# KadAMRN/Data_Free_Quantization

Hardware: AMD Instinct MI355X
Metric: weight-GB/s quantized (per-ch INT8 DFQ sweep) + top-1 delta, MobileNetV2 (higher is better)
Workload: dtype f32

## Files before the change

### data_free_quantization_amd/_lib.py

```python
from __future__ import annotations

import ctypes as C
import os
from pathlib import Path
from typing import Optional

import torch

PKG = Path(__file__).resolve().parent
LIB_PATH = PKG / "libdfq_hip.so"

DFQ_TENSOR_ASYM, DFQ_TENSOR_SYM, DFQ_CHANNEL_ASYM, DFQ_CHANNEL_SYM = 0, 1, 2, 3
DFQ_CLIP, DFQ_GIVEN_RANGE, DFQ_SCALE_F32, DFQ_PACK_INT4, DFQ_DEVICE_RANGE = 0x1, 0x2, 0x4, 0x8, 0x10
DFQ_OK, DFQ_ERR_INVALID, DFQ_ERR_HIP, DFQ_ERR_UNSUPPORTED = 0, -1, -2, -3
DFQ_ERR_NOMEM, DFQ_ERR_SHAPE, DFQ_ERR_WORKSPACE = -4, -5, -6

EXPORTS = [
    "dfq_abi_version", "dfq_preload", "dfq_error_string", "dfq_last_hip_error",
    "dfq_quantize_ws_bytes", "dfq_quantize_tensor", "dfq_chunk_range", "dfq_range", "dfq_fake_quant_given",
    "dfq_fake_quant_tensor",
    "dfq_act_observe",
    "dfq_sweep_plan_create", "dfq_sweep_plan_ws_bytes", "dfq_sweep_plan_create_ws", "dfq_sweep_plan_execute",
    "dfq_sweep_plan_stats", "dfq_sweep_plan_destroy",
    "dfq_bn_fold", "dfq_bn_fold_ws_bytes", "dfq_bn_fold_batch", "dfq_clamp", "dfq_clamp_batch",
    "dfq_cle_ws_bytes", "dfq_cle_relation",
    "dfq_diff_plan_create", "dfq_diff_plan_snapshot", "dfq_diff_plan_execute", "dfq_diff_plan_destroy",
    "dfq_cle_plan_ws_bytes", "dfq_cle_plan_create", "dfq_cle_plan_run", "dfq_cle_plan_launch", "dfq_cle_plan_join",
    "dfq_cle_plan_info", "dfq_cle_plan_set_timing", "dfq_cle_plan_stats", "dfq_cle_plan_destroy",
    "dfq_bias_absorb", "dfq_bias_absorb_ws_bytes", "dfq_bias_absorb_batch", "dfq_bc_expect", "dfq_bc_apply", "dfq_bc_propagate", "dfq_bc_chain",
    "dfq_act_moments", "dfq_act_minmax", "dfq_act_affine",
    "dfq_pair_stats_ws_bytes", "dfq_pair_stats_batch",
    "dfq_clip_search_ws_bytes", "dfq_clip_search_batch",
    "dfq_mx_quantize_ws_bytes", "dfq_mx_quantize_batch", "dfq_mx_quantize_search_batch", "dfq_mx_gemm",
    "dfq_mx_linear", "dfq_mx_conv2d",
    "dfq_int_gemm", "dfq_int_linear", "dfq_int_conv2d", "dfq_int_dwconv2d",
]
DIAG_EXPORTS = ["dfq_probe_stream", "dfq_probe_lds", "dfq_debug_timeline", "dfq_debug_ablate",
                "dfq_diag_cle_check_structure"]
DIAG_LIB_PATH = PKG / "libdfq_diag.so"


class TensorDesc(C.Structure):
    _fields_ = [
        ("src", C.c_void_p), ("dst", C.c_void_p), ("codes", C.c_void_p), ("scale", C.c_void_p),
        ("zero", C.c_void_p), ("esum", C.c_void_p), ("rows", C.c_int64), ("row_len", C.c_int64),
        ("khw", C.c_int32), ("bits", C.c_int32), ("mode", C.c_int32), ("flags", C.c_int32),
        ("clip_lo", C.c_float), ("clip_hi", C.c_float), ("given_min", C.c_double), ("given_max", C.c_double),
        ("range_enc", C.c_void_p),
    ]


class SweepStats(C.Structure):
    _fields_ = [
        ("n_tensors", C.c_int64), ("n_elems", C.c_int64), ("n_tasks_reduce", C.c_int64),
        ("n_tasks_main", C.c_int64), ("algo_bytes", C.c_int64), ("launches", C.c_int32),
        ("grid_blocks", C.c_int32), ("variant", C.c_int32), ("reserved", C.c_int32),
    ]


class BnFoldDesc(C.Structure):
    _fields_ = [
        ("w", C.c_void_p), ("bias", C.c_void_p), ("bn_w", C.c_void_p), ("bn_b", C.c_void_p),
        ("bn_mean", C.c_void_p), ("bn_var", C.c_void_p), ("fake_w", C.c_void_p), ("fake_b", C.c_void_p),
        ("eps", C.c_float), ("flags", C.c_int32), ("rows", C.c_int64), ("row_len", C.c_int64),
        ("range_enc", C.c_void_p),
    ]


class CleRel(C.Structure):
    _fields_ = [
        ("w1", C.c_void_p), ("w2", C.c_void_p), ("b1", C.c_void_p), ("bn_w", C.c_void_p), ("bn_b", C.c_void_p),
        ("s_acc", C.c_void_p), ("c1", C.c_int64), ("len1", C.c_int64), ("o2", C.c_int64), ("i2", C.c_int64),
        ("khw2", C.c_int64), ("s_acc_init", C.c_int32), ("reserved", C.c_int32),
    ]


class AbsorbDesc(C.Structure):
    _fields_ = [
        ("w2", C.c_void_p), ("b1", C.c_void_p), ("b2", C.c_void_p), ("bn_w", C.c_void_p), ("bn_b", C.c_void_p),
        ("c1", C.c_int64), ("o2", C.c_int64), ("i2", C.c_int64), ("khw2", C.c_int64),
    ]


class BcOp(C.Structure):
    _fields_ = [
        ("kind", C.c_int32), ("flag", C.c_int32), ("a", C.c_void_p), ("b", C.c_void_p), ("out", C.c_void_p),
        ("out2", C.c_void_p), ("n", C.c_int64), ("i2", C.c_int64), ("f", C.c_int64),
    ]


class PairDesc(C.Structure):
    _fields_ = [
        ("x", C.c_void_p), ("y", C.c_void_p), ("rows_out", C.c_void_p), ("total_out", C.c_void_p),
        ("rows", C.c_int64), ("row_len", C.c_int64),
    ]


class ClipSearchDesc(C.Structure):
    _fields_ = [
        ("w", C.c_void_p), ("rows", C.c_int64), ("row_len", C.c_int64), ("bits", C.c_int32), ("mode", C.c_int32),
        ("candidates", C.c_int32), ("flags", C.c_int32), ("min_frac", C.c_float), ("reserved", C.c_int32),
        ("choice", C.c_void_p), ("range", C.c_void_p), ("noise", C.c_void_p), ("range_enc", C.c_void_p),
    ]


class MxDesc(C.Structure):
    _fields_ = [
        ("src", C.c_void_p), ("dst", C.c_void_p), ("codes", C.c_void_p), ("scales", C.c_void_p), ("esum", C.c_void_p),
        ("rows", C.c_int64), ("row_len", C.c_int64), ("khw", C.c_int32), ("format", C.c_int32), ("flags", C.c_int32),
        ("reserved", C.c_int32),
    ]


class MxGemmDesc(C.Structure):
    _fields_ = [
        ("a_codes", C.c_void_p), ("a_scales", C.c_void_p), ("b_codes", C.c_void_p), ("b_scales", C.c_void_p),
        ("bias", C.c_void_p), ("out", C.c_void_p), ("ldo", C.c_int64), ("M", C.c_int64), ("N", C.c_int64),
        ("K", C.c_int64), ("a_format", C.c_int32), ("b_format", C.c_int32), ("flags", C.c_int32),
        ("reserved", C.c_int32),
    ]


class MxLinearDesc(C.Structure):
    _fields_ = [
        ("x", C.c_void_p), ("b_codes", C.c_void_p), ("b_scales", C.c_void_p), ("bias", C.c_void_p), ("out", C.c_void_p),
        ("ldx", C.c_int64), ("ldo", C.c_int64), ("M", C.c_int64), ("N", C.c_int64), ("K", C.c_int64),
        ("x_format", C.c_int32), ("b_format", C.c_int32), ("flags", C.c_int32), ("reserved", C.c_int32),
    ]


class MxConv2dDesc(C.Structure):
    _fields_ = [
        ("x", C.c_void_p), ("b_codes", C.c_void_p), ("b_scales", C.c_void_p), ("bias", C.c_void_p), ("out", C.c_void_p),
        ("B", C.c_int64), ("C", C.c_int64), ("H", C.c_int64), ("W", C.c_int64), ("N", C.c_int64), ("KH", C.c_int64),
        ("KW", C.c_int64), ("stride_h", C.c_int64), ("stride_w", C.c_int64), ("pad_h", C.c_int64), ("pad_w", C.c_int64),
        ("dil_h", C.c_int64), ("dil_w", C.c_int64),
        ("x_format", C.c_int32), ("b_format", C.c_int32), ("flags", C.c_int32), ("reserved", C.c_int32),
    ]


class IntGemmDesc(C.Structure):
    _fields_ = [
        ("a_codes", C.c_void_p), ("a_scale", C.c_void_p), ("a_zero", C.c_void_p), ("b_codes", C.c_void_p),
        ("b_scale", C.c_void_p), ("b_zero", C.c_void_p), ("bias", C.c_void_p), ("out", C.c_void_p),
        ("ldo", C.c_int64), ("M", C.c_int64), ("N", C.c_int64), ("K", C.c_int64),
        ("a_signed", C.c_int32), ("b_signed", C.c_int32), ("flags", C.c_int32), ("reserved", C.c_int32),
    ]


class IntLinearDesc(C.Structure):
    _fields_ = [
        ("x", C.c_void_p), ("min_dev", C.c_void_p), ("max_dev", C.c_void_p), ("b_codes", C.c_void_p),
        ("b_scale", C.c_void_p), ("b_zero", C.c_void_p), ("bias", C.c_void_p), ("out", C.c_void_p),
        ("given_min", C.c_double), ("given_max", C.c_double),
        ("ldx", C.c_int64), ("ldo", C.c_int64), ("M", C.c_int64), ("N", C.c_int64), ("K", C.c_int64),
        ("x_bits", C.c_int32), ("x_symmetric", C.c_int32), ("b_signed", C.c_int32), ("flags", C.c_int32),
        ("reserved", C.c_int32), ("reserved2", C.c_int32),
    ]


class IntConv2dDesc(C.Structure):
    _fields_ = [
        ("x", C.c_void_p), ("min_dev", C.c_void_p), ("max_dev", C.c_void_p), ("b_codes", C.c_void_p),
        ("b_scale", C.c_void_p), ("b_zero", C.c_void_p), ("bias", C.c_void_p), ("out", C.c_void_p),
        ("given_min", C.c_double), ("given_max", C.c_double),
        ("B", C.c_int64), ("C", C.c_int64), ("H", C.c_int64), ("W", C.c_int64), ("N", C.c_int64), ("KH", C.c_int64),
        ("KW", C.c_int64), ("stride_h", C.c_int64), ("stride_w", C.c_int64), ("pad_h", C.c_int64), ("pad_w", C.c_int64),
        ("dil_h", C.c_int64), ("dil_w", C.c_int64),
        ("x_bits", C.c_int32), ("x_symmetric", C.c_int32), ("b_signed", C.c_int32), ("flags", C.c_int32),
        ("reserved", C.c_int32), ("reserved2", C.c_int32),
    ]


class IntDwConv2dDesc(C.Structure):
    _fields_ = [(("mult", t) if f == "N" else (f, t)) for f, t in IntConv2dDesc._fields_]


DFQ_BC_OP_EXPECT, DFQ_BC_OP_APPLY, DFQ_BC_OP_PROPAGATE, DFQ_BC_OP_COPY = 0, 1, 2, 3
DFQ_BC_APPLY_VEC_SCRATCH = 1
DFQ_BN_FOLD_ZERO_BIAS = 1
DFQ_PAIR_PIECE_ELEMS = 8192
DFQ_CLIP_PIECE_ELEMS, DFQ_CLIP_MAX_CANDIDATES, DFQ_CLIP_SEARCH_DRY = 4096, 64, 1
DFQ_MX_BLOCK = 32
DFQ_MX_FP4_E2M1, DFQ_MX_FP8_E4M3 = 0, 1
DFQ_MX_FP6_E2M3, DFQ_MX_FP6_E3M2 = 0x23, 0x32
DFQ_MX_TASK_ELEMS, DFQ_MX_ESUM_TASK_ELEMS = 4096, 2048
DFQ_INT_B_PACK4, DFQ_INT_B_PER_ROW, DFQ_INT_MAX_K = 0x1, 0x2, 32768
DFQ_INT_DW_MAX_TAPS, DFQ_INT_DW_TILE_H, DFQ_INT_DW_TILE_W, DFQ_INT_DW_LDS_BYTES = 64, 32, 64, 16384

_LIB: Optional[C.CDLL] = None


class DFQLibraryError(RuntimeError):
    pass


def load(path: Optional[os.PathLike] = None) -> C.CDLL:
    global _LIB
    if _LIB is not None and path is None:
        return _LIB
    by_env = path is None and os.environ.get("DFQ_LIB") == "diag"
    if by_env:
        path = DIAG_LIB_PATH
    p = Path(path) if path else LIB_PATH
    if not p.exists():
        raise DFQLibraryError(
            f"{p} is missing: build it with `python -m data_free_quantization_amd.build` "
            "(or __graft_entry__.build()); there is no CPU fallback")
    L = C.CDLL(str(p))
    P, I32, I64, F32, F64, SZ = C.c_void_p, C.c_int32, C.c_int64, C.c_float, C.c_double, C.c_size_t
    sig = {
        "dfq_abi_version": ([], C.c_int),
        "dfq_preload": ([], C.c_int),
        "dfq_error_string": ([C.c_int], C.c_char_p),
        "dfq_last_hip_error": ([], C.c_char_p),
        "dfq_quantize_ws_bytes": ([C.POINTER(TensorDesc), C.POINTER(SZ)], C.c_int),
        "dfq_quantize_tensor": ([C.POINTER(TensorDesc), P, SZ, P], C.c_int),
        "dfq_chunk_range": ([P, I64, I64, P, P, P], C.c_int),
        "dfq_range": ([P, I64, P, P], C.c_int),
        "dfq_act_observe": ([P, I64, I64, P, P, P, I32, I32, F64, P, P], C.c_int),
        "dfq_fake_quant_given": ([P, P, I64, I32, I32, I32, P, P, P, F64, F64, P], C.c_int),
        "dfq_fake_quant_tensor": ([P, P, I64, I32, I32, I32, P, P], C.c_int),
        "dfq_sweep_plan_create": ([C.POINTER(TensorDesc), I32, C.POINTER(P)], C.c_int),
        "dfq_sweep_plan_ws_bytes": ([C.POINTER(TensorDesc), I32], C.c_int64),
        "dfq_sweep_plan_create_ws": ([C.POINTER(TensorDesc), I32, P, I64, P, C.POINTER(P)], C.c_int),
        "dfq_sweep_plan_execute": ([P, P], C.c_int),
        "dfq_sweep_plan_stats": ([P, C.POINTER(SweepStats)], C.c_int),
        "dfq_sweep_plan_destroy": ([P], C.c_int),
        "dfq_bn_fold": ([P, P, P, P, P, P, P, P, F32, I64, I64, P], C.c_int),
        "dfq_clamp": ([P, I64, F32, F32, P], C.c_int),
        "dfq_clamp_batch": ([C.POINTER(P), C.POINTER(I64), I32, F32, F32, P], C.c_int),
        "dfq_bn_fold_ws_bytes": ([C.POINTER(BnFoldDesc), I32], C.c_int64),
        "dfq_bn_fold_batch": ([C.POINTER(BnFoldDesc), I32, P, I64, P], C.c_int),
        "dfq_cle_ws_bytes": ([I64], SZ),
        "dfq_cle_relation": ([P, P, P, P, P, I64, I64, I64, I64, I64, F64, F64, I32, F32, P, P, I32, P, SZ, P],
                             C.c_int),
        "dfq_diff_plan_create": ([C.POINTER(P), C.POINTER(P), C.POINTER(I64), I32, C.POINTER(P)], C.c_int),
        "dfq_diff_plan_snapshot": ([P, P], C.c_int),
        "dfq_diff_plan_execute": ([P, C.POINTER(F64), P], C.c_int),
        "dfq_diff_plan_destroy": ([P], C.c_int),
        "dfq_cle_plan_ws_bytes": ([C.POINTER(I64), I32], C.c_int64),
        "dfq_cle_plan_create": ([C.POINTER(CleRel), I32, C.POINTER(P), C.POINTER(I64), I32, F64, F64, I32, F32, I32,
                                 P, I64, C.POINTER(P)], C.c_int),
        "dfq_cle_plan_run": ([P, F64, I32, I32, C.POINTER(I32), C.POINTER(F64), P], C.c_int),
        "dfq_cle_plan_launch": ([P, F64, I32, I32, P], C.c_int),
        "dfq_cle_plan_join": ([P, C.POINTER(I32), C.POINTER(F64)], C.c_int),
        "dfq_cle_plan_info": ([P, C.POINTER(I32), C.POINTER(I32), C.POINTER(I32)], C.c_int),
        "dfq_cle_plan_destroy": ([P], C.c_int),
        "dfq_cle_plan_set_timing": ([P, I32], C.c_int),
        "dfq_cle_plan_stats": ([P, C.POINTER(I64), C.POINTER(F64), C.POINTER(I32)], C.c_int),
        "dfq_bias_absorb": ([P, P, P, P, P, I64, I64, I64, I64, F32, P], C.c_int),
        "dfq_bias_absorb_ws_bytes": ([C.POINTER(AbsorbDesc), I32], C.c_int64),
        "dfq_bias_absorb_batch": ([C.POINTER(AbsorbDesc), I32, F32, P, I64, C.POINTER(I32), P], C.c_int),
        "dfq_bc_expect": ([P, P, I64, I32, I32, P, P], C.c_int),
        "dfq_bc_apply": ([P, I64, I64, P, I64, P, P, C.POINTER(I64), P], C.c_int),
        "dfq_bc_propagate": ([P, I64, P, I64, I32, P], C.c_int),
        "dfq_bc_chain": ([C.POINTER(BcOp), I32, C.POINTER(I32), P], C.c_int),
        "dfq_act_moments": ([P, P, I64, I32, I32, F32, I32, P, P, P], C.c_int),
        "dfq_act_minmax": ([P, P, I64, I32, F32, F32, P, P], C.c_int),
        "dfq_act_affine": ([P, P, P, I64, I64, I64, I64, P, P], C.c_int),
        "dfq_pair_stats_ws_bytes": ([C.POINTER(PairDesc), I32], C.c_int64),
        "dfq_pair_stats_batch": ([C.POINTER(PairDesc), I32, P, I64, P], C.c_int),
        "dfq_clip_search_ws_bytes": ([C.POINTER(ClipSearchDesc), I32], C.c_int64),
        "dfq_clip_search_batch": ([C.POINTER(ClipSearchDesc), I32, P, I64, P], C.c_int),
        "dfq_mx_quantize_ws_bytes": ([C.POINTER(MxDesc), I32], C.c_int64),
        "dfq_mx_quantize_batch": ([C.POINTER(MxDesc), I32, P, I64, P], C.c_int),
        "dfq_mx_quantize_search_batch": ([C.POINTER(MxDesc), I32, P, I64, P], C.c_int),
        "dfq_mx_gemm": ([C.POINTER(MxGemmDesc), P], C.c_int),
        "dfq_mx_linear": ([C.POINTER(MxLinearDesc), P], C.c_int),
        "dfq_mx_conv2d": ([C.POINTER(MxConv2dDesc), P], C.c_int),
        "dfq_int_gemm": ([C.POINTER(IntGemmDesc), P], C.c_int),
        "dfq_int_linear": ([C.POINTER(IntLinearDesc), P], C.c_int),
        "dfq_int_conv2d": ([C.POINTER(IntConv2dDesc), P], C.c_int),
        "dfq_int_dwconv2d": ([C.POINTER(IntDwConv2dDesc), P], C.c_int),
    }
    diag = {
        "dfq_probe_stream": ([P, P, P, P, I64, I32, P], C.c_int),
        "dfq_debug_timeline": ([P, I64], C.c_int),
        "dfq_debug_ablate": ([C.c_uint32], C.c_int),
        "dfq_probe_lds": ([P, P, P, P, I64, I32, I32, P], C.c_int),
        "dfq_diag_cle_check_structure": ([C.POINTER(CleRel), I32, C.POINTER(P), C.POINTER(I64), I32, I32,
                                          C.POINTER(I64), C.c_char_p, I32], C.c_int),
    }
    for name, (args, res) in sig.items():
        fn = getattr(L, name)
        fn.argtypes = args
        fn.restype = res
    for name, (args, res) in diag.items():
        if hasattr(L, name):
            fn = getattr(L, name)
            fn.argtypes = args
            fn.restype = res
    if L.dfq_abi_version() != 1:
        raise DFQLibraryError("libdfq_hip.so ABI version mismatch")
    if path is None or by_env:
        _LIB = L
    return L


_PRELOADED = False


def preload() -> C.CDLL:
    global _PRELOADED
    L = load()
    if not _PRELOADED:
        check(L.dfq_preload(), "dfq_preload")
        _PRELOADED = True
    return L


_DIAG: Optional[C.CDLL] = None


def load_diag() -> C.CDLL:
    global _DIAG
    if _DIAG is None:
        _DIAG = load(DIAG_LIB_PATH)
    return _DIAG


def check(rc: int, what: str, shape_error=RuntimeError):
    if rc == DFQ_OK:
        return
    L = load()
    msg = f"{what}: {L.dfq_error_string(rc).decode()}"
    if rc == DFQ_ERR_HIP:
        msg += f" ({L.dfq_last_hip_error().decode()})"
    if rc == DFQ_ERR_SHAPE:
        raise shape_error(msg)
    if rc == DFQ_ERR_UNSUPPORTED:
        raise NotImplementedError(msg)
    raise DFQLibraryError(msg)


_F32 = torch.float32


def require_device(*tensors: Optional[torch.Tensor]):
    for t in tensors:
        if t is None or (t.is_cuda and t.dtype is _F32 and t.is_contiguous()):
            continue
        if not t.is_cuda:
            raise RuntimeError(
                "data_free_quantization_amd runs the DFQ weight path on a ROCm GPU only; "
                f"got a tensor on {t.device} (move the model with .cuda() first)")
        if t.dtype != torch.float32:
            raise TypeError(f"expected float32 tensors, got {t.dtype}")
        raise ValueError("expected contiguous tensors")


def ptr(t: Optional[torch.Tensor]):
    return None if t is None else C.c_void_p(t.data_ptr())


WEIGHT_GENERATION = 0


def weights_changed() -> None:
    global WEIGHT_GENERATION
    WEIGHT_GENERATION += 1


REF_THREADS = int(os.environ.get("DFQ_REF_THREADS", "8"))


_RAW_STREAM = getattr(torch._C, "_cuda_getCurrentRawStream", None)


def raw_stream(device: torch.device) -> C.c_void_p:
    idx = device.index if device.index is not None else torch.cuda.current_device()
    if _RAW_STREAM is not None:
        return C.c_void_p(_RAW_STREAM(idx))
    return C.c_void_p(torch.cuda.current_stream(device).cuda_stream)


def stream_of(t: torch.Tensor):
    return raw_stream(t.device)
```

### data_free_quantization_amd/csrc/dfq_cle.hip

```cpp
#include "dfq_cle_kernels.h"

#include <algorithm>
#include <chrono>
#include <cstdio>
#include <cstdlib>
#include <cstring>
#include <condition_variable>
#include <functional>
#include <memory>
#include <mutex>
#include <thread>
#include <type_traits>
#include <new>
#include <vector>

using namespace dfq;

constexpr int32_t kCleHistCap = 1025;

struct CleTables {
    CleRel* rels = nullptr;
    CleTask *rtasks = nullptr, *atasks = nullptr;
    CleLayer* layers = nullptr;
    CleChunk* chunks = nullptr;
    CleUnit* units = nullptr;
    int64_t* b1off = nullptr;
    float* part = nullptr;
    float* b1 = nullptr;
    float* tail = nullptr;
    uint32_t* rng = nullptr;
    double* means = nullptr;
    CleState* state = nullptr;
    double* hist = nullptr;
    uint32_t* cnt = nullptr;
    float* vsave = nullptr;
    int32_t* vtag = nullptr;
    int64_t host_bytes = 0, total = 0;
    void bind(char* base, const CleStructure& S, int32_t slots) {
        constexpr bool kHost = true, kDevice = false;
        int64_t off = 0;
        auto table = [&](auto*& ptr, int64_t count, bool host_built) {
            using T = std::remove_reference_t<decltype(*ptr)>;
            ptr = base ? reinterpret_cast<T*>(base + off) : nullptr;
            off += round256((int64_t)sizeof(T) * std::max<int64_t>(count, 1));
            if (host_built) host_bytes = off;
        };
        const int64_t nl = (int64_t)S.layers.size(), nch = (int64_t)S.chunks.size();
        table(rels, (int64_t)S.R.size(), kHost);
        table(rtasks, (int64_t)S.rt.size(), kHost);
        table(atasks, (int64_t)S.at.size(), kHost);
        table(layers, nl, kHost);
        table(chunks, nch, kHost);
        table(units, (int64_t)S.units.size(), kHost);
        table(b1off, (int64_t)S.b1off.size(), kHost);
        table(part, (int64_t)(slots + 2) * nl, kHost);
        table(b1, 32 * S.nb1_total, kDevice);
        table(tail, kCleTailWords * nch, kDevice);
        table(rng, 4 * S.M, kDevice);
        table(means, nl, kDevice);
        table(state, 1, kDevice);
        table(hist, kCleHistCap, kDevice);
        table(cnt, nch + 1, kDevice);
        table(vsave, S.lagged ? 2 * S.M : 0, kDevice);
        table(vtag, S.lagged ? (int64_t)S.at.size() : 0, kDevice);
        if (!S.lagged) vsave = nullptr, vtag = nullptr;
        total = off;
    }
};

struct dfq_cle_plan {
    std::shared_ptr<const CleStructure> S;
    CleTables t;
    int32_t slots = 8;
    double* d_hist = nullptr;
    uint32_t* d_flag = nullptr;
    uint64_t* d_sig = nullptr;
    uint64_t gen = 0;
    double smin = 1e-8, smax = 1e8;
    int32_t is_signed = 0;
    float eps = 0.f;
    void* d_tables = nullptr;
    bool pooled = false;
    void* d_snap_owned = nullptr;
    int dev = 0;
    struct CleAsync* async = nullptr;
    bool abandoned = false;
    bool timed = false;
    float loop_ms = -1.f;
    int32_t launched = 0;
    int32_t nl() const { return (int32_t)S->layers.size(); }
    int64_t nchunks() const { return (int64_t)S->chunks.size(); }
    int64_t nunits() const { return (int64_t)S->units.size(); }
};

static bool cle_timing() {
    static const bool on = ab_env("DFQ_CLE_TIMING") != nullptr;
    return on;
}

struct CleDeviceCtx {
    std::mutex mu;
    hipStream_t st = nullptr;
    CleState* h_state = nullptr;
    uint32_t* h_flag = nullptr;
    uint32_t* d_flag = nullptr;
    char* d_pool = nullptr;
    size_t pool_cap = 0;
    char* h_pool = nullptr;
    size_t hpool_cap = 0;
    bool pool_busy = false;
    uint64_t pool_struct = 0;
    hipEvent_t pool_ev = nullptr;
    double* d_hist = nullptr;
    int64_t hist_cap = 0;
    double* h_hist = nullptr;
    int64_t h_hist_cap = 0;
    void* sig = nullptr;
    int sig_state = 0;
    uint64_t gen = 0;
    struct dfq_cle_plan* pending = nullptr;
    hipEvent_t in_ev = nullptr;
    struct CleWorker* worker = nullptr;
};
static CleDeviceCtx& cle_device_ctx(int dev) {
    static CleDeviceCtx ctx[64];
    return ctx[dev & 63];
}
static std::unique_lock<std::mutex> cle_ctx_acquire(CleDeviceCtx& ctx, bool join_pending);
static hipError_t cle_ctx_ready(CleDeviceCtx& ctx) {
    hipError_t e = hipSuccess;
    if (!ctx.st) {
        int least = 0, greatest = 0;
        e = hipDeviceGetStreamPriorityRange(&least, &greatest);
        if (e == hipSuccess) e = hipStreamCreateWithPriority(&ctx.st, hipStreamNonBlocking, greatest);
    }
    if (e == hipSuccess && !ctx.h_state) e = hipHostMalloc(&ctx.h_state, sizeof(CleState));
    if (e == hipSuccess && !ctx.h_flag) {
        e = hipHostMalloc(&ctx.h_flag, 64, hipHostMallocMapped | hipHostMallocCoherent);
        if (e == hipSuccess) e = hipHostGetDevicePointer(reinterpret_cast<void**>(&ctx.d_flag), ctx.h_flag, 0);
    }
    if (e == hipSuccess && !ctx.pool_ev) e = hipEventCreateWithFlags(&ctx.pool_ev, hipEventDisableTiming);
    if (e == hipSuccess && !ctx.in_ev) e = hipEventCreateWithFlags(&ctx.in_ev, hipEventDisableTiming);
    return e;
}

template <class T, class N>
static hipError_t cle_grow(T*& buf, N& have, N need, N cap, bool pinned) {
    if (have >= need) return hipSuccess;
    (void)(pinned ? hipHostFree(buf) : hipFree(buf));
    buf = nullptr;
    have = 0;
    const hipError_t e = pinned ? hipHostMalloc(&buf, sizeof(T) * cap, hipHostMallocDefault) : hipMalloc(&buf, sizeof(T) * cap);
    if (e == hipSuccess) have = cap;
    return e;
}
static hipError_t cle_pool_reserve(CleDeviceCtx& ctx, size_t dev_bytes, size_t host_bytes, bool headroom) {
    const auto cap = [&](size_t n) { return headroom ? n + n / 2 : n; };
    if (ctx.pool_cap < dev_bytes) ctx.pool_struct = 0;
    hipError_t e = cle_grow(ctx.d_pool, ctx.pool_cap, dev_bytes, cap(dev_bytes), false);
    if (e == hipSuccess) e = cle_grow(ctx.h_pool, ctx.hpool_cap, host_bytes, cap(host_bytes), true);
    return e;
}

static void cle_plan_free(dfq_cle_plan* p) {
    const double t0 = now_us();
    if (p->pooled) {
        CleDeviceCtx& ctx = cle_device_ctx(p->dev);
        const std::unique_lock<std::mutex> lock = cle_ctx_acquire(ctx, false);
        ctx.pool_busy = false;
    } else {
        (void)hipFree(p->d_tables);
    }
    (void)hipFree(p->d_snap_owned);
    if (cle_timing()) fprintf(stderr, "DFQ_CLE_TIMING free: %.1f us\n", now_us() - t0);
    delete p;
}

static int64_t snap_bytes(int64_t n) { return round256(n * (int64_t)sizeof(float)); }

extern "C" int64_t dfq_cle_plan_ws_bytes(const int64_t* target_n, int32_t n_targets) {
    if (n_targets < 0 || (n_targets > 0 && !target_n)) return -1;
    int64_t b = 0;
    for (int32_t l = 0; l < n_targets; ++l) {
        if (target_n[l] < 0) return -1;
        b += snap_bytes(target_n[l]);
    }
    return b;
}

extern "C" int dfq_cle_plan_create(const dfq_cle_rel* rels, int32_t n_rel, float* const* targets,
                                   const int64_t* target_n, int32_t n_targets, double s_min, double s_max,
                                   int32_t is_signed, float eps, int32_t ref_threads, void* ws, int64_t ws_bytes,
                                   dfq_cle_plan** out) {
    if (!out || n_rel < 0 || n_targets < 0 || (n_rel > 0 && !rels) || (n_targets > 0 && (!targets || !target_n)))
        return DFQ_ERR_INVALID;
    const double tc0 = now_us();
    const int64_t need_ws = dfq_cle_plan_ws_bytes(target_n, n_targets);
    if (need_ws < 0) return DFQ_ERR_INVALID;
    if (ws && (ws_bytes < need_ws || reinterpret_cast<uintptr_t>(ws) % 256 != 0)) return DFQ_ERR_INVALID;
    *out = nullptr;
    std::vector<CleRel> R;
    int64_t M = 0;
    if (const int rc = cle_rels_from_desc(rels, n_rel, R, M); rc != DFQ_OK) return rc;
    const double tp1 = now_us();
    bool cached = false;
    int rc = DFQ_OK;
    const std::shared_ptr<const CleStructure> S =
        cle_structure_cached(R, M, targets, target_n, n_targets, ref_threads, rc, cached);
    if (!S) return rc;
    const double tp5 = now_us();
    std::vector<CleRel> Rb = S->R;
    for (int32_t r = 0; r < n_rel; ++r) {
        Rb[r].w1 = R[r].w1; Rb[r].w2 = R[r].w2; Rb[r].b1 = R[r].b1;
        Rb[r].bnw = R[r].bnw; Rb[r].bnb = R[r].bnb; Rb[r].sacc = R[r].sacc;
    }
    dfq_cle_plan* p = new (std::nothrow) dfq_cle_plan();
    if (!p) return DFQ_ERR_NOMEM;
    p->S = S;
    std::vector<CleLayer> layers = S->layers;
    {
        char* snap_base = static_cast<char*>(ws);
        if (!snap_base && need_ws > 0) {
            hipError_t e = hipMalloc(&p->d_snap_owned, need_ws);
            if (e != hipSuccess) { set_last_hip_error(e); cle_plan_free(p); return DFQ_ERR_HIP; }
            snap_base = static_cast<char*>(p->d_snap_owned);
        }
        int64_t snap_off = 0;
        for (int32_t l = 0; l < n_targets; ++l) {
            layers[l].w = targets[l];
            layers[l].snap = reinterpret_cast<float*>(snap_base + snap_off);
            snap_off += snap_bytes(target_n[l]);
        }
    }
    if (cle_timing() && !cached) {
        fprintf(stderr, "DFQ_CLE_TIMING plan: steps %d nlaunch %d lagged %d stop %d; offsets (units/ranges):", S->steps,
                S->nlaunch, (int)S->lagged, S->stop_off);
        for (int32_t k = 0; k < 2 * S->nlaunch; ++k)
            fprintf(stderr, " %d:%lld/%lld", k, (long long)(S->uoffs[k + 1] - S->uoffs[k]),
                    (long long)(S->roffs[k + 1] - S->roffs[k]));
        fprintf(stderr, "; rescale tasks per step:");
        for (int32_t k = 0; k < S->steps; ++k) fprintf(stderr, " %lld", (long long)(S->astep[k + 1] - S->astep[k]));
        fprintf(stderr, "\n");
    }
    (void)hipGetDevice(&p->dev);
    p->smin = s_min; p->smax = s_max; p->is_signed = is_signed; p->eps = eps;
    p->slots = std::max<int32_t>(ref_threads, 1);
    hipError_t e;
    auto fail = [&](hipError_t err) { set_last_hip_error(err); cle_plan_free(p); return DFQ_ERR_HIP; };
    CleTables& T = p->t;
    T.bind(nullptr, *S, p->slots);
    const double tm0 = now_us();
    char* base = nullptr;
    char* hblob = nullptr;
    CleDeviceCtx& ctx = cle_device_ctx(p->dev);
    e = hipSuccess;
    {
        const std::unique_lock<std::mutex> lock = cle_ctx_acquire(ctx, false);
        if (!ctx.pool_busy && (e = cle_ctx_ready(ctx)) == hipSuccess &&
            (e = hipEventSynchronize(ctx.pool_ev)) == hipSuccess &&
            (e = cle_pool_reserve(ctx, (size_t)T.total, (size_t)T.host_bytes, true)) == hipSuccess) {
            ctx.pool_busy = true;
            p->pooled = true;
            base = ctx.d_pool;
            hblob = ctx.h_pool;
        }
        if (e != hipSuccess) return fail(e);
    }
    std::vector<char> blob;
    const bool resident = p->pooled && ctx.pool_struct == S->id;
    if (!p->pooled) {
        if ((e = hipMalloc(&p->d_tables, T.total)) != hipSuccess) return fail(e);
        base = static_cast<char*>(p->d_tables);
        blob.assign(T.host_bytes, 0);
        hblob = blob.data();
    } else if (!resident) {
        std::memset(hblob, 0, T.host_bytes);
    }
    T.bind(base, *S, p->slots);
    const double tm1 = now_us();
    auto mirror = [&](const auto* d) { return hblob + (reinterpret_cast<const char*>(d) - base); };
    auto put = [&](const auto* d, const auto& v) {
        if (!v.empty()) std::memcpy(mirror(d), v.data(), sizeof(v[0]) * v.size());
    };
    put(T.rels, Rb);
    put(T.layers, layers);
    if (!resident) {
        put(T.rtasks, S->rt); put(T.atasks, S->at); put(T.chunks, S->chunks); put(T.units, S->units); put(T.b1off, S->b1off);
        float* lm = reinterpret_cast<float*>(mirror(T.part)) + (int64_t)p->slots * n_targets;
        for (int64_t l = 0; l < n_targets; ++l) {
            lm[2 * l] = (float)layers[l].n;
            lm[2 * l + 1] = layers[l].nt == 1 ? 1.f : 0.f;
        }
    }
    if (p->pooled) {
        if (resident) {
            const size_t nr = sizeof(CleRel) * Rb.size(), nly = sizeof(CleLayer) * layers.size();
            if (nr && (e = hipMemcpyAsync(T.rels, mirror(T.rels), nr, hipMemcpyHostToDevice, ctx.st)) != hipSuccess)
                return fail(e);
            if (nly && (e = hipMemcpyAsync(T.layers, mirror(T.layers), nly, hipMemcpyHostToDevice, ctx.st)) != hipSuccess)
                return fail(e);
        } else if ((e = hipMemcpyAsync(base, hblob, T.host_bytes, hipMemcpyHostToDevice, ctx.st)) != hipSuccess) {
            return fail(e);
        }
        if ((e = hipEventRecord(ctx.pool_ev, ctx.st)) != hipSuccess) return fail(e);
        ctx.pool_struct = S->id;
    } else if ((e = hipMemcpy(base, hblob, T.host_bytes, hipMemcpyHostToDevice)) != hipSuccess) {
        return fail(e);
    }
    if (cle_timing())
        fprintf(stderr, "DFQ_CLE_TIMING create: plan %.1f us (relations %.1f, structure %s %.1f: chains %.1f, tasks %.1f, "
                "chunks %.1f, placement %.1f), tables %lld B %.1f us, copy %lld B %.1f us\n", tm0 - tc0, tp1 - tc0,
                cached ? "cached" : "built", tp5 - tp1, S->t_chains, S->t_tasks, S->t_chunks, S->t_place,
                (long long)T.total, tm1 - tm0, (long long)T.host_bytes, now_us() - tm1);
    *out = p;
    return DFQ_OK;
}

static int cle_enqueue_iteration(dfq_cle_plan* p, hipStream_t s, int32_t g, int32_t max_iters) {
    const int64_t kStepGrid = [] {
        const char* e = ab_env("DFQ_CLE_STEP_GRID");
        return e && *e ? std::max<int64_t>(1, atoll(e)) : int64_t(2048);
    }();
    const int64_t kTileGrid = [] {
        const char* e = ab_env("DFQ_CLE_TILE_GRID");
        return e && *e ? std::max<int64_t>(1, atoll(e)) : int64_t(4096);
    }();
    const CleStructure& S = *p->S;
    const CleTables& T = p->t;
    CleFin F{T.cnt, T.part, T.means, p->d_hist, p->nchunks(), S.nbig, p->slots, p->nl(), 0, p->d_flag,
             S.stop_off < 0 ? 1 : 0};
    const int32_t NL = S.nlaunch;
    const bool run_g = g < max_iters, prev = g >= 1;
    for (int32_t k = 0; k < NL; ++k) {
        const bool step = k < S.steps;
        const int64_t a0 = step ? S.astep[k] : 0, a1 = step ? S.astep[k + 1] : 0;
        if (step && run_g && !S.fused && S.rstep[k + 1] > S.rstep[k]) {
            hipLaunchKernelGGL(cle_loop_range_kernel, dim3((int)std::min<int64_t>(S.rstep[k + 1] - S.rstep[k], kStepGrid)),
                               dim3(kThreads), 0, s, T.rels, T.rtasks, S.rstep[k], S.rstep[k + 1], T.rng, S.M, T.state, 0);
            DFQ_LAUNCH_CHECK();
        }
        const int64_t nab = run_g ? std::min<int64_t>(a1 - a0, kStepGrid) : 0;
        const int64_t uo = S.uoffs[k], nuo = run_g ? S.uoffs[k + 1] - uo : 0;
        const int64_t up = S.uoffs[NL + k], nup = prev ? S.uoffs[NL + k + 1] - up : 0;
        const int64_t ro = S.roffs[k], nro_t = (g + 1 < max_iters) ? S.roffs[k + 1] - ro : 0;
        const int64_t rp = S.roffs[NL + k], nrp_t = (prev && run_g) ? S.roffs[NL + k + 1] - rp : 0;
        int64_t nto = std::min<int64_t>(nuo, kTileGrid);
        const int64_t ntp = std::min<int64_t>(nup, kTileGrid);
        F.last = (k == S.steps) ? 1 : 0;
        if (F.last && run_g && S.nbig == 0) nto = std::max<int64_t>(nto, 1);
        const int64_t nro = std::min<int64_t>(nro_t, kStepGrid), nrp = std::min<int64_t>(nrp_t, kStepGrid);
        int32_t stop_it = -1;
        if (S.stop_off == k && run_g) stop_it = g;
        else if (S.stop_off == NL + k && prev) stop_it = g - 1;
        const int64_t nblk = nab + (stop_it >= 0 ? cle_stop_blocks(p->nchunks()) : 0) + nto + ntp + nro + nrp;
        if (nblk == 0) continue;
        auto kern = (step && S.step_pos[k]) ? cle_loop_step_kernel<true> : cle_loop_step_kernel<false>;
        hipLaunchKernelGGL(kern, dim3((int)nblk), dim3(kThreads), 0, s, T.rels, T.atasks, a0, a1, nab, T.rng,
                           S.M, p->is_signed, p->eps, p->smin, p->smax, T.layers, T.chunks, T.b1off,
                           T.units, uo, nuo, nto, up, nup, ntp, T.b1, T.tail, T.rtasks, ro, nro_t, nro, rp,
                           nrp_t, nrp, F, T.state, g, T.vsave, T.vtag, stop_it);
        DFQ_LAUNCH_CHECK();
    }
    return DFQ_OK;
}

constexpr int32_t kCleAhead = 1;
constexpr double kClePollQuietUs = 1000.0;
static constexpr int kCleGateSeconds = 120;
static constexpr int kCleJoinSeconds = kCleGateSeconds + 30;
static constexpr double kCleLaunchDeadlineUs = 0.5e6 * kCleGateSeconds;
static hipError_t cle_hist_ready(CleDeviceCtx& ctx, int32_t max_iters) {
    const int64_t n = (int64_t)max_iters + 1;
    hipError_t e = cle_grow(ctx.h_hist, ctx.h_hist_cap, n, n, true);
    if (e == hipSuccess && n > kCleHistCap) e = cle_grow(ctx.d_hist, ctx.hist_cap, n, n, false);
    return e;
}

static hipError_t cle_copy_back(void* dst, const void* src, size_t bytes, hipStream_t s) {
    hipError_t e = hipMemcpyAsync(dst, src, bytes, hipMemcpyDeviceToHost, s);
    return e == hipSuccess ? hipStreamSynchronize(s) : e;
}

#ifdef DFQ_DIAGNOSTICS
#include "dfq_cle_timeline.h"
#else
struct CleTimeline {
    int begin(const dfq_cle_plan*, hipStream_t) { return DFQ_OK; }
    int report(const dfq_cle_plan*, hipStream_t) { return DFQ_OK; }
};
#endif

struct CleRun {
    double threshold;
    int32_t count, max_iters;
    double deadline_us;
    bool idle = false;
    double t_drive = 0;
    int32_t launched = 0;
    bool deadline_hit = false;
    hipEvent_t tev[2] = {nullptr, nullptr};
};

static int cle_run_setup(dfq_cle_plan* p, CleDeviceCtx& ctx, CleRun& run) {
    DFQ_HIP_CHECK(cle_ctx_ready(ctx));
    *ctx.h_flag = 0;
    p->d_flag = ctx.d_flag;
    hipStream_t s = ctx.st;
    const CleStructure& S = *p->S;
    const CleTables& T = p->t;
    p->d_hist = T.hist;
    DFQ_HIP_CHECK(cle_hist_ready(ctx, run.max_iters));
    if (run.max_iters + 1 > kCleHistCap) p->d_hist = ctx.d_hist;
    CleState init{};
    init.diff = 1e8;
    init.thr = run.threshold;
    init.count = run.count;
    init.max_iters = run.max_iters;
    init.done = !((init.diff > run.threshold) && (0 < run.count)) || run.max_iters == 0;
    run.idle = init.done != 0;
    {
        const int64_t npart = (int64_t)p->slots * std::max(p->nl(), 1), ncnt = p->nchunks() + 1;
        const int64_t nvtag = T.vtag ? (int64_t)S.at.size() : 0;
        const int64_t words = std::max({4 * S.M, npart, ncnt, nvtag});
        const int64_t grid = std::min<int64_t>(std::max<int64_t>({p->nunits(), ceil_div(words, (int64_t)kThreads), 1}), 4096);
        hipLaunchKernelGGL(cle_loop_init_kernel, dim3((int)grid), dim3(kThreads), 0, s, T.layers, T.chunks,
                           p->nchunks(), T.units, p->nunits(), T.rng, S.M, T.part, npart, T.cnt, ncnt,
                           T.vtag, nvtag, T.state, init);
        DFQ_LAUNCH_CHECK();
    }
    if (S.fused && S.rstep[1] > S.rstep[0]) {
        hipLaunchKernelGGL(cle_loop_range_kernel, dim3((int)std::min<int64_t>(S.rstep[1] - S.rstep[0], 2048)),
                           dim3(kThreads), 0, s, T.rels, T.rtasks, S.rstep[0], S.rstep[1], T.rng, S.M, T.state, 0);
        DFQ_LAUNCH_CHECK();
    }
    return DFQ_OK;
}

static int cle_run_drive(dfq_cle_plan* p, CleDeviceCtx& ctx, CleRun& run) {
    hipStream_t s = ctx.st;
    const int32_t max_iters = run.max_iters;
    run.t_drive = now_us();
    p->loop_ms = -1.f;
    if (p->timed) {
        DFQ_HIP_CHECK(hipEventCreate(&run.tev[0]));
        DFQ_HIP_CHECK(hipEventCreate(&run.tev[1]));
        DFQ_HIP_CHECK(hipEventRecord(run.tev[0], s));
    }
    if (run.idle) return DFQ_OK;
    const char* pd = ab_env("DFQ_CLE_TEST_POLL_DELAY_US");
    const int poll_delay_us = pd ? atoi(pd) : 0;
    const double quiet_us = pd ? 0.0 : kClePollQuietUs;
    uint32_t last_f = ~0u;
    double t_moved = run.t_drive;
    for (;;) {
        const uint32_t f = __atomic_load_n(ctx.h_flag, __ATOMIC_ACQUIRE);
        if (f & 1u) break;
        const int32_t ran = (int32_t)(f >> 1);
        if (run.launched <= max_iters && !run.deadline_hit && run.launched - ran <= kCleAhead) {
            const int rc = cle_enqueue_iteration(p, s, run.launched, max_iters);
            if (rc != DFQ_OK) return rc;
            ++run.launched;
            continue;
        }
        if (poll_delay_us > 0) std::this_thread::sleep_for(std::chrono::microseconds(poll_delay_us));
        const double t = now_us();
        if (f != last_f) {
            last_f = f;
            t_moved = t;
        } else if (t - t_moved >= quiet_us) {
            const hipError_t q = hipStreamQuery(s);
            if (q != hipErrorNotReady) {
                if (q != hipSuccess) break;
                const uint32_t f2 = __atomic_load_n(ctx.h_flag, __ATOMIC_ACQUIRE);
                if ((f2 & 1u) || run.launched > max_iters || run.deadline_hit || (int32_t)(f2 >> 1) + 1 < run.launched)
                    break;
            }
            t_moved = t;
        }
        if (run.deadline_us > 0 && t - run.t_drive > run.deadline_us) run.deadline_hit = true;
        __builtin_ia32_pause();
    }
    return DFQ_OK;
}

static int cle_run_drain(dfq_cle_plan* p, CleDeviceCtx& ctx, CleRun& run, CleTimeline& timeline, int32_t* iterations,
                         std::vector<double>* hist) {
    hipStream_t s = ctx.st;
    const CleTables& T = p->t;
    if (!run.idle && p->S->lagged) {
        hipLaunchKernelGGL(cle_loop_rollback_kernel, dim3(1024), dim3(kThreads), 0, s, T.layers, p->nl(), T.rels,
                           T.atasks, (int64_t)p->S->at.size(), T.vsave, T.vtag, T.state);
        DFQ_LAUNCH_CHECK();
    }
    if (run.tev[1]) DFQ_HIP_CHECK(hipEventRecord(run.tev[1], s));
    if (p->d_sig) DFQ_HIP_CHECK(hipStreamWriteValue64(s, p->d_sig, p->gen, 0));
    DFQ_HIP_CHECK(hipMemcpyAsync(ctx.h_state, T.state, sizeof(CleState), hipMemcpyDeviceToHost, s));
    const int32_t hn = std::min(run.launched, run.max_iters);
    if (hist && hn > 0) DFQ_HIP_CHECK(hipMemcpyAsync(ctx.h_hist, p->d_hist, sizeof(double) * hn, hipMemcpyDeviceToHost, s));
    DFQ_HIP_CHECK(hipStreamSynchronize(s));
    p->launched = run.launched;
    if (run.tev[0]) {
        float ms = -1.f;
        if (hipEventElapsedTime(&ms, run.tev[0], run.tev[1]) == hipSuccess) p->loop_ms = ms;
        (void)hipEventDestroy(run.tev[0]);
        (void)hipEventDestroy(run.tev[1]);
    }
    if (cle_timing())
        fprintf(stderr, "DFQ_CLE_TIMING run: loop %.1f us (%d iterations launched)\n", now_us() - run.t_drive, run.launched);
    if (const int rc = timeline.report(p, s); rc != DFQ_OK) return rc;
    const CleState fin = *ctx.h_state;
    if (fin.error) {
        set_last_hip_error(hipErrorLaunchTimeOut);
        return DFQ_ERR_HIP;
    }
    if (!fin.done) {
        set_last_hip_error_text(run.deadline_hit ? "the launched CLE loop reached its time limit before converging"
                                                 : "the CLE loop stopped before its stop rule said done");
        return DFQ_ERR_HIP;
    }
    if (ab_env("DFQ_CLE_DEBUG")) {
        std::vector<float> part((size_t)p->slots * std::max(p->nl(), 1));
        DFQ_HIP_CHECK(cle_copy_back(part.data(), T.part, sizeof(float) * part.size(), s));
        for (int32_t l = 0; l < p->nl(); ++l) {
            fprintf(stderr, "DFQ_CLE_DEBUG layer %d:", l);
            for (int t = 0; t < p->slots; ++t) fprintf(stderr, " %.9g", part[(size_t)p->slots * l + t]);
            fprintf(stderr, "\n");
        }
    }
    if (iterations) *iterations = fin.iters;
    if (hist) {
        hist->assign((size_t)std::max(fin.iters, 0), 0.0);
        if (fin.iters > 0) std::memcpy(hist->data(), ctx.h_hist, sizeof(double) * std::min(fin.iters, hn));
    }
    return DFQ_OK;
}

static int cle_run_locked(dfq_cle_plan* p, CleDeviceCtx& ctx, double threshold, int32_t count, int32_t max_iters,
                          int32_t* iterations, std::vector<double>* hist, double deadline_us = -1.0) {
    CleRun run{threshold, count, max_iters, deadline_us};
    CleTimeline timeline;
    int rc = cle_run_setup(p, ctx, run);
    if (rc == DFQ_OK) rc = timeline.begin(p, ctx.st);
    if (rc == DFQ_OK) rc = cle_run_drive(p, ctx, run);
    if (rc == DFQ_OK) rc = cle_run_drain(p, ctx, run, timeline, iterations, hist);
    return rc;
}


struct CleAsync {
    std::mutex m;
    std::condition_variable cv;
    bool done = false;
    int rc = DFQ_OK;
    int32_t iters = 0;
    std::vector<double> hist;
    char err[128] = {0};
};

struct CleWorker {
    std::mutex m;
    std::condition_variable cv;
    std::function<void()> job;
    bool has_job = false;
};
static void cle_worker_loop(CleWorker* w) {
    for (;;) {
        std::function<void()> j;
        {
            std::unique_lock<std::mutex> l(w->m);
            w->cv.wait(l, [w] { return w->has_job; });
            j = std::move(w->job);
            w->has_job = false;
        }
        j();
    }
}
static void cle_worker_ready(CleDeviceCtx& ctx) {
    if (ctx.worker) return;
    CleWorker* w = new CleWorker();
    std::thread(cle_worker_loop, w).detach();
    ctx.worker = w;
}

static hipError_t cle_signal_ready(CleDeviceCtx& ctx) {
    if (ctx.sig) return hipSuccess;
    if (ctx.sig_state < 0) return hipErrorNotSupported;
    hipError_t e = hipSuccess;
    void* sig = nullptr;
    if ((e = hipExtMallocWithFlags(&sig, sizeof(uint64_t), hipMallocSignalMemory)) != hipSuccess) {
        ctx.sig_state = -1;
        return e;
    }
    if ((e = hipStreamWriteValue64(ctx.st, sig, 0, 0)) != hipSuccess || (e = hipStreamSynchronize(ctx.st)) != hipSuccess) {
        (void)hipFree(sig);
        ctx.sig_state = -1;
        return e;
    }
    ctx.sig = sig;
    ctx.gen = 0;
    return hipSuccess;
}

static bool cle_async_join(dfq_cle_plan* p, double seconds = -1.0) {
    if (!p || !p->async) return true;
    CleAsync* a = p->async;
    std::unique_lock<std::mutex> l(a->m);
    if (seconds < 0) {
        a->cv.wait(l, [a] { return a->done; });
        return true;
    }
    return a->cv.wait_for(l, std::chrono::duration<double>(seconds), [a] { return a->done; });
}

static std::unique_lock<std::mutex> cle_ctx_acquire(CleDeviceCtx& ctx, bool join_pending) {
    std::unique_lock<std::mutex> lock(ctx.mu);
    while (dfq_cle_plan* q = join_pending ? ctx.pending : nullptr) {
        lock.unlock();
        cle_async_join(q);
        lock.lock();
        if (ctx.pending == q) ctx.pending = nullptr;
    }
    return lock;
}
static void cle_pending_clear(CleDeviceCtx& ctx, dfq_cle_plan* p) {
    const std::unique_lock<std::mutex> lock = cle_ctx_acquire(ctx, false);
    if (ctx.pending == p) ctx.pending = nullptr;
}

extern "C" int dfq_cle_plan_run(dfq_cle_plan* p, double threshold, int32_t count, int32_t max_iters,
                                int32_t* iterations, double* diffs, void* stream) {
    if (!p || max_iters < 0 || p->async) return DFQ_ERR_INVALID;
    const double ts0 = now_us();
    DFQ_HIP_CHECK(hipStreamSynchronize(static_cast<hipStream_t>(stream)));
    const double ts1 = now_us();
    int dev = 0;
    DFQ_HIP_CHECK(hipGetDevice(&dev));
    CleDeviceCtx& ctx = cle_device_ctx(dev);
    const std::unique_lock<std::mutex> lock = cle_ctx_acquire(ctx, true);
    if (cle_timing()) fprintf(stderr, "DFQ_CLE_TIMING run: caller sync %.1f us, context %.1f us\n", ts1 - ts0,
                              now_us() - ts1);
    std::vector<double> h;
    const int rc = cle_run_locked(p, ctx, threshold, count, max_iters, iterations, diffs ? &h : nullptr);
    if (rc == DFQ_OK && diffs && !h.empty()) std::memcpy(diffs, h.data(), sizeof(double) * h.size());
    return rc;
}

extern "C" int dfq_cle_plan_launch(dfq_cle_plan* p, double threshold, int32_t count, int32_t max_iters,
                                   void* stream) {
    if (!p || max_iters < 0 || p->async) return DFQ_ERR_INVALID;
    if (ab_env("DFQ_CLE_TL")) return DFQ_ERR_UNSUPPORTED;
    hipStream_t caller = static_cast<hipStream_t>(stream);
    CleDeviceCtx& ctx = cle_device_ctx(p->dev);
    const double tl0 = now_us();
    std::unique_ptr<CleAsync> rec(new (std::nothrow) CleAsync());
    uint64_t gen = 0;
    {
        const std::unique_lock<std::mutex> lock = cle_ctx_acquire(ctx, true);
        DFQ_HIP_CHECK(hipSetDevice(p->dev));
        DFQ_HIP_CHECK(cle_ctx_ready(ctx));
        const hipError_t es = cle_signal_ready(ctx);
        if (es == hipErrorNotSupported) return DFQ_ERR_UNSUPPORTED;
        DFQ_HIP_CHECK(es);
        DFQ_HIP_CHECK(cle_hist_ready(ctx, max_iters));
        DFQ_HIP_CHECK(hipEventRecord(ctx.in_ev, caller));
        DFQ_HIP_CHECK(hipStreamWaitEvent(ctx.st, ctx.in_ev, 0));
        gen = ctx.gen + 1;
        hipLaunchKernelGGL(cle_caller_gate_kernel, dim3(1), dim3(64), 0, caller,
                           static_cast<const uint64_t*>(ctx.sig), gen, (uint64_t)kCleGateSeconds * 100000000ull);
        DFQ_LAUNCH_CHECK();
        ctx.gen = gen;
        if (rec) p->async = rec.get(), ctx.pending = p;
    }
    if (cle_timing()) fprintf(stderr, "DFQ_CLE_TIMING launch: gate and order %.1f us\n", now_us() - tl0);
    CleAsync* a = rec.release();
    const double t_launch = now_us();
    auto body = [p, &ctx, threshold, count, max_iters, gen, t_launch](CleAsync* a) {
        std::lock_guard<std::mutex> lock(ctx.mu);
        int rc = DFQ_OK;
        if (hipSetDevice(p->dev) != hipSuccess) {
            rc = DFQ_ERR_HIP;
        } else {
            rc = cle_run_locked(p, ctx, threshold, count, max_iters, &a->iters, &a->hist, kCleLaunchDeadlineUs);
        }
        if (rc == DFQ_ERR_HIP) copy_error_text(a->err, sizeof(a->err), dfq_last_hip_error());
        if (const char* d = ab_env("DFQ_CLE_TEST_RELEASE_DELAY_MS"))
            std::this_thread::sleep_for(std::chrono::milliseconds(atoi(d)));
        hipError_t e = hipStreamWriteValue64(ctx.st, ctx.sig, gen, 0);
        if (e == hipSuccess) e = hipStreamSynchronize(ctx.st);
        if (e != hipSuccess) {
            fprintf(stderr, "dfq_cle_plan_launch: releasing the caller's stream failed (%s)\n", hipGetErrorString(e));
            if (rc == DFQ_OK) rc = DFQ_ERR_HIP;
        }
        if (rc == DFQ_OK && now_us() - t_launch > 0.9e6 * kCleGateSeconds) {
            set_last_hip_error(hipErrorLaunchTimeOut);
            copy_error_text(a->err, sizeof(a->err), "CLE loop outlived the caller's stream gate");
            rc = DFQ_ERR_HIP;
        }
        {
            std::lock_guard<std::mutex> l(a->m);
            a->rc = rc;
            a->done = true;
        }
        a->cv.notify_all();
    };
    if (!a) {
        CleAsync tmp;
        body(&tmp);
        return tmp.rc;
    }
    p->d_sig = static_cast<uint64_t*>(ctx.sig);
    if (ab_env("DFQ_CLE_HOST_RELEASE")) p->d_sig = nullptr;
    p->gen = gen;
    bool posted = false;
    try {
        const std::unique_lock<std::mutex> lock = cle_ctx_acquire(ctx, false);
        cle_worker_ready(ctx);
        {
            std::lock_guard<std::mutex> l(ctx.worker->m);
            ctx.worker->job = [body, a] { body(a); };
            ctx.worker->has_job = true;
        }
        ctx.worker->cv.notify_one();
        posted = true;
    } catch (...) {}
    if (!posted) body(a);
    if (cle_timing()) fprintf(stderr, "DFQ_CLE_TIMING launch: total %.1f us\n", now_us() - tl0);
    return DFQ_OK;
}

extern "C" int dfq_cle_plan_join(dfq_cle_plan* p, int32_t* iterations, double* diffs) {
    if (!p || !p->async) return DFQ_ERR_INVALID;
    if (p->abandoned) return DFQ_ERR_HIP;
    double limit = kCleJoinSeconds;
    if (const char* j = ab_env("DFQ_CLE_TEST_JOIN_LIMIT_MS")) limit = atoi(j) * 1e-3;
    if (!cle_async_join(p, limit)) {
        p->abandoned = true;
        set_last_hip_error_text("the launched CLE loop did not finish in time; the caller's stream stays held");
        return DFQ_ERR_HIP;
    }
    cle_pending_clear(cle_device_ctx(p->dev), p);
    const CleAsync& a = *p->async;
    if (a.rc == DFQ_ERR_HIP && a.err[0]) set_last_hip_error_text(a.err);
    if (a.rc != DFQ_OK) return a.rc;
    if (iterations) *iterations = a.iters;
    if (diffs && !a.hist.empty()) std::memcpy(diffs, a.hist.data(), sizeof(double) * a.hist.size());
    return DFQ_OK;
}

extern "C" int dfq_cle_plan_info(const dfq_cle_plan* p, int32_t* chains, int32_t* steps, int32_t* launches) {
    if (!p) return DFQ_ERR_INVALID;
    if (chains) *chains = p->S->chains;
    if (steps) *steps = p->S->steps;
    if (launches) *launches = p->S->fused ? p->S->nlaunch : 2 * p->S->steps + 1;
    return DFQ_OK;
}

extern "C" int dfq_cle_plan_set_timing(dfq_cle_plan* p, int32_t on) {
    if (!p || p->async) return DFQ_ERR_INVALID;
    p->timed = on != 0;
    return DFQ_OK;
}

extern "C" int dfq_cle_plan_stats(const dfq_cle_plan* p, int64_t* bytes, double* loop_ms, int32_t* launched) {
    if (!p) return DFQ_ERR_INVALID;
    if (bytes) {
        bytes[0] = p->S->bytes_rescale;
        bytes[1] = p->S->bytes_metric;
        bytes[2] = p->S->bytes_range;
    }
    if (loop_ms) *loop_ms = p->loop_ms;
    if (launched) *launched = p->launched;
    return DFQ_OK;
}

extern "C" int dfq_cle_plan_destroy(dfq_cle_plan* p) {
    if (!p) return DFQ_OK;
    if (p->abandoned) return DFQ_OK;
    if (p->async) {
        cle_async_join(p);
        cle_pending_clear(cle_device_ctx(p->dev), p);
        delete p->async;
        p->async = nullptr;
    }
    cle_plan_free(p);
    return DFQ_OK;
}

namespace dfq {
constexpr size_t kClePreloadPool = size_t(4) << 20, kClePreloadHostPool = size_t(2) << 20;
constexpr int32_t kClePreloadHistIters = 100000;
hipError_t preload_cle() {
    int dev = 0;
    hipError_t e0 = hipGetDevice(&dev);
    if (e0 != hipSuccess) return e0;
    {
        CleDeviceCtx& ctx = cle_device_ctx(dev);
        const std::unique_lock<std::mutex> lock = cle_ctx_acquire(ctx, false);
        if ((e0 = cle_ctx_ready(ctx)) != hipSuccess) return e0;
        if (!ctx.pool_busy && (e0 = cle_pool_reserve(ctx, kClePreloadPool, kClePreloadHostPool, false)) != hipSuccess)
            return e0;
        if ((e0 = cle_hist_ready(ctx, kClePreloadHistIters)) != hipSuccess) return e0;
        (void)cle_signal_ready(ctx);
        try { cle_worker_ready(ctx); } catch (...) {}
    }
    hipFuncAttributes a;
    hipError_t e = hipFuncGetAttributes(&a, reinterpret_cast<const void*>(cle_loop_step_kernel<true>));
    if (e == hipSuccess) e = hipFuncGetAttributes(&a, reinterpret_cast<const void*>(cle_loop_step_kernel<false>));
    return e;
}
}
```

### data_free_quantization_amd/csrc/dfq_cle_kernels.h

```cpp
#pragma once
#include "dfq_cle_common.h"
namespace dfq {

struct CleState {
    double diff;
    double thr;
    int32_t iter_count;
    int32_t iters;
    int32_t done;
    int32_t count;
    int32_t max_iters;
    int32_t error;
};

constexpr int kCleW1RowsPerTask = 4;
constexpr int kCleW2ChansPerTask = 4;

__device__ __forceinline__ float group_min(float v, int g) {
    for (int off = g >> 1; off >= 1; off >>= 1) v = fminf(v, __shfl_xor(v, off, 64));
    return v;
}
__device__ __forceinline__ float group_max(float v, int g) {
    for (int off = g >> 1; off >= 1; off >>= 1) v = fmaxf(v, __shfl_xor(v, off, 64));
    return v;
}
template <class F>
__device__ __forceinline__ void for_short_rows(int64_t a, int64_t b, int64_t len, F&& f) {
    const int lane = threadIdx.x & 63, wv = threadIdx.x >> 6;
    const int G = row_group_lanes(len), rpw = 64 / G;
    const int sub = lane / G, sl = lane % G;
    for (int64_t base = a + (int64_t)wv * rpw; base < b; base += (int64_t)(kThreads / 64) * rpw) {
        const int64_t c = base + sub;
        f(c, c < b, sl, G);
    }
}
__device__ __forceinline__ void wave_range(const float* __restrict__ p_, int64_t n, bool vec, int lane, float& vmin,
                                           float& vmax) {
    const DFQ_GLOBAL float* __restrict__ p = (const DFQ_GLOBAL float*)p_;
    vmin = INFINITY;
    vmax = -INFINITY;
    if (vec) {
        const DFQ_GLOBAL f32x4* p4 = (const DFQ_GLOBAL f32x4*)p;
        const int64_t n4 = n >> 2;
        for (int64_t i = lane; i < n4; i += 4 * 64) {
            f32x4 v[4];
#pragma unroll
            for (int u = 0; u < 4; ++u)
                if (i + 64 * u < n4) v[u] = p4[i + 64 * u];
#pragma unroll
            for (int u = 0; u < 4; ++u)
                if (i + 64 * u < n4) {
                    vmin = fminf(vmin, fminf(fminf(v[u].x, v[u].y), fminf(v[u].z, v[u].w)));
                    vmax = fmaxf(vmax, fmaxf(fmaxf(v[u].x, v[u].y), fmaxf(v[u].z, v[u].w)));
                }
        }
    } else {
        for (int64_t i = lane; i < n; i += 4 * 64) {
            float v[4];
#pragma unroll
            for (int u = 0; u < 4; ++u)
                if (i + 64 * u < n) v[u] = p[i + 64 * u];
#pragma unroll
            for (int u = 0; u < 4; ++u)
                if (i + 64 * u < n) {
                    vmin = fminf(vmin, v[u]);
                    vmax = fmaxf(vmax, v[u]);
                }
        }
    }
    cle_wave_minmax(vmin, vmax);
}

template <class F>
__device__ __forceinline__ void wave_scale(float* __restrict__ p_, int64_t n, bool vec, int lane, F&& factor) {
    DFQ_GLOBAL float* __restrict__ p = (DFQ_GLOBAL float*)p_;
    float f = 0.f;
    bool have = false;
    if (vec) {
        DFQ_GLOBAL f32x4* p4 = (DFQ_GLOBAL f32x4*)p;
        const int64_t n4 = n >> 2;
        for (int64_t i = lane; i < n4; i += 4 * 64) {
            f32x4 v[4];
#pragma unroll
            for (int u = 0; u < 4; ++u)
                if (i + 64 * u < n4) v[u] = p4[i + 64 * u];
            if (!have) {
                f = factor();
                have = true;
            }
#pragma unroll
            for (int u = 0; u < 4; ++u)
                if (i + 64 * u < n4) {
                    v[u].x = v[u].x * f;
                    v[u].y = v[u].y * f;
                    v[u].z = v[u].z * f;
                    v[u].w = v[u].w * f;
                    p4[i + 64 * u] = v[u];
                }
        }
    } else {
        for (int64_t i = lane; i < n; i += 4 * 64) {
            float v[4];
#pragma unroll
            for (int u = 0; u < 4; ++u)
                if (i + 64 * u < n) v[u] = p[i + 64 * u];
            if (!have) {
                f = factor();
                have = true;
            }
#pragma unroll
            for (int u = 0; u < 4; ++u)
                if (i + 64 * u < n) p[i + 64 * u] = v[u] * f;
        }
    }
}

template <class F>
__device__ __forceinline__ void wave_scale_mm(float* __restrict__ p_, int64_t n, bool vec, int lane, float& vmin,
                                              float& vmax, F&& factor) {
    DFQ_GLOBAL float* __restrict__ p = (DFQ_GLOBAL float*)p_;
    vmin = INFINITY;
    vmax = -INFINITY;
    float f = 0.f;
    bool have = false;
    if (vec) {
        DFQ_GLOBAL f32x4* p4 = (DFQ_GLOBAL f32x4*)p;
        const int64_t n4 = n >> 2;
        for (int64_t i = lane; i < n4; i += 4 * 64) {
            f32x4 v[4];
#pragma unroll
            for (int u = 0; u < 4; ++u)
                if (i + 64 * u < n4) v[u] = p4[i + 64 * u];
            if (!have) {
                f = factor();
                have = true;
            }
#pragma unroll
            for (int u = 0; u < 4; ++u)
                if (i + 64 * u < n4) {
                    v[u].x = v[u].x * f;
                    v[u].y = v[u].y * f;
                    v[u].z = v[u].z * f;
                    v[u].w = v[u].w * f;
                    p4[i + 64 * u] = v[u];
                    vmin = fminf(vmin, fminf(fminf(v[u].x, v[u].y), fminf(v[u].z, v[u].w)));
                    vmax = fmaxf(vmax, fmaxf(fmaxf(v[u].x, v[u].y), fmaxf(v[u].z, v[u].w)));
                }
        }
    } else {
        for (int64_t i = lane; i < n; i += 4 * 64) {
            float v[4];
#pragma unroll
            for (int u = 0; u < 4; ++u)
                if (i + 64 * u < n) v[u] = p[i + 64 * u];
            if (!have) {
                f = factor();
                have = true;
            }
#pragma unroll
            for (int u = 0; u < 4; ++u)
                if (i + 64 * u < n) {
                    const float y = v[u] * f;
                    p[i + 64 * u] = y;
                    vmin = fminf(vmin, y);
                    vmax = fmaxf(vmax, y);
                }
        }
    }
    cle_wave_minmax(vmin, vmax);
}

template <class F>
__device__ __forceinline__ void wave_scale_range(float* __restrict__ p_, int64_t n, int lane, float& vmin, float& vmax,
                                                 F&& factor) {
    DFQ_GLOBAL float* __restrict__ p = (DFQ_GLOBAL float*)p_;
    vmin = INFINITY;
    vmax = -INFINITY;
    float f = 0.f;
    bool have = false;
    for (int64_t i = lane; i < n; i += 64) {
        const float x = p[i];
        if (!have) {
            f = factor();
            have = true;
        }
        const float y = x * f;
        p[i] = y;
        vmin = fminf(vmin, y);
        vmax = fmaxf(vmax, y);
    }
    cle_wave_minmax(vmin, vmax);
}

__device__ __forceinline__ bool tile_by_position(const CleRel& R, const CleTask& tk) {
    return R.khw2 > 1 && R.khw2 <= kTileMaxKhw && (tk.a / R.o2g) == ((tk.b - 1) / R.o2g);
}

__device__ void tile_range_by_position(const CleRel& R, const CleTask& tk, uint32_t* __restrict__ mn,
                                       uint32_t* __restrict__ mx, float* __restrict__ tl) {
    const int t = threadIdx.x;
    const int khw = (int)R.khw2;
    const int64_t rowlen = R.i2 * R.khw2;
    const int ncol = (int)(tk.c1 - tk.c0);
    const int npos = ncol * khw;
    const DFQ_GLOBAL float* base = (const DFQ_GLOBAL float*)(R.w2 + tk.c0 * R.khw2);
    float vmn[kTileMaxKhw], vmx[kTileMaxKhw];
#pragma unroll
    for (int m = 0; m < kTileMaxKhw; ++m) {
        vmn[m] = INFINITY;
        vmx[m] = -INFINITY;
    }
    for (int64_t o = tk.a; o < tk.b; ++o) {
        const DFQ_GLOBAL float* rp = base + o * rowlen;
        float v[kTileMaxKhw];
#pragma unroll
        for (int m = 0; m < kTileMaxKhw; ++m)
            if (m < khw && t + kThreads * m < npos) v[m] = rp[t + kThreads * m];
#pragma unroll
        for (int m = 0; m < kTileMaxKhw; ++m)
            if (m < khw && t + kThreads * m < npos) {
                vmn[m] = fminf(vmn[m], v[m]);
                vmx[m] = fmaxf(vmx[m], v[m]);
            }
    }
#pragma unroll
    for (int m = 0; m < kTileMaxKhw; ++m)
        if (m < khw && t + kThreads * m < npos) {
            tl[t + kThreads * m] = vmn[m];
            tl[kThreads * kTileMaxKhw + t + kThreads * m] = vmx[m];
        }
    __syncthreads();
    if (t < ncol) {
        float a = INFINITY, b = -INFINITY;
        for (int k = 0; k < khw; ++k) {
            a = fminf(a, tl[t * khw + k]);
            b = fmaxf(b, tl[kThreads * kTileMaxKhw + t * khw + k]);
        }
        const int64_t c = R.c1 + (tk.a / R.o2g) * R.i2 + tk.c0 + t;
        atomicMin(&mn[c], enc_ord(a));
        atomicMax(&mx[c], enc_ord(b));
    }
    __syncthreads();
}

__device__ __forceinline__ void cle_range_body(const CleRel* __restrict__ rels, const CleTask* __restrict__ tasks,
                                               int64_t t0, int64_t t1, uint32_t* __restrict__ rng, int64_t M, int par,
                                               int64_t blk, int64_t nblk, float* tl) {
    uint32_t* mins = rng + (int64_t)par * 2 * M;
    uint32_t* maxs = mins + M;
    uint32_t* omins = rng + (int64_t)(par ^ 1) * 2 * M;
    uint32_t* omaxs = omins + M;
    const int lane = threadIdx.x & 63;
    const int wv = threadIdx.x >> 6;
    for (int64_t t = t0 + blk; t < t1; t += nblk) {
        const CleTask tk = tasks[t];
        const CleRel& R = rels[tk.rel];
        uint32_t* mn = mins + R.moff;
        uint32_t* mx = maxs + R.moff;
        if (tk.kind == kRangeW1 && R.len1 < 64) {
            for_short_rows(tk.a, tk.b, R.len1, [&](int64_t c, bool act, int sl, int G) {
                float vmin = INFINITY, vmax = -INFINITY;
                if (act)
                    for (int64_t i = sl; i < R.len1; i += G) {
                        const float x = ((DFQ_GLOBAL float*)R.w1)[c * R.len1 + i];
                        vmin = fminf(vmin, x);
                        vmax = fmaxf(vmax, x);
                    }
                vmin = group_min(vmin, G);
                vmax = group_max(vmax, G);
                if (act && sl == 0) {
                    mn[c] = enc_ord(vmin);
                    mx[c] = enc_ord(vmax);
                }
            });
        } else if (tk.kind == kRangeW2Contig && R.o2g * R.khw2 < 64) {
            const int64_t seg = R.o2g * R.khw2;
            for_short_rows(tk.a, tk.b, seg, [&](int64_t c, bool act, int sl, int G) {
                float vmin = INFINITY, vmax = -INFINITY;
                if (act)
                    for (int64_t i = sl; i < seg; i += G) {
                        const float x = ((DFQ_GLOBAL float*)R.w2)[c * seg + i];
                        vmin = fminf(vmin, x);
                        vmax = fmaxf(vmax, x);
                    }
                vmin = group_min(vmin, G);
                vmax = group_max(vmax, G);
                if (act && sl == 0) {
                    mn[R.c1 + c] = enc_ord(vmin);
                    mx[R.c1 + c] = enc_ord(vmax);
                }
            });
        } else if (tk.kind == kRangeW1) {
            for (int64_t c = tk.a + wv; c < tk.b; c += kThreads / 64) {
                float vmin, vmax;
                wave_range(R.w1 + c * R.len1, R.len1, R.vec1, lane, vmin, vmax);
                if (lane == 0) {
                    mn[c] = enc_ord(vmin);
                    mx[c] = enc_ord(vmax);
                }
            }
        } else if (tk.kind == kRangeW2Contig) {
            const int64_t seg = R.o2g * R.khw2;
            for (int64_t c = tk.a + wv; c < tk.b; c += kThreads / 64) {
                float vmin, vmax;
                wave_range(R.w2 + c * seg, seg, R.vec2, lane, vmin, vmax);
                if (lane == 0) {
                    mn[R.c1 + c] = enc_ord(vmin);
                    mx[R.c1 + c] = enc_ord(vmax);
                }
            }
        } else if (tk.kind == kRangeW2Tile) {
            if (tile_by_position(R, tk)) {
                tile_range_by_position(R, tk, mn, mx, tl);
                continue;
            }
            const int64_t rowlen = R.i2 * R.khw2;
            const bool one_group = (tk.a / R.o2g) == ((tk.b - 1) / R.o2g);
            for (int64_t i = tk.c0 + threadIdx.x; i < tk.c1; i += kThreads) {
                float vmin = INFINITY, vmax = -INFINITY;
                if (one_group && R.khw2 == 1) {
                    float v[kColTileRows];
#pragma unroll
                    for (int j = 0; j < kColTileRows; ++j)
                        if (tk.a + j < tk.b) v[j] = ((DFQ_GLOBAL float*)R.w2)[(tk.a + j) * rowlen + i];
#pragma unroll
                    for (int j = 0; j < kColTileRows; ++j)
                        if (tk.a + j < tk.b) {
                            vmin = fminf(vmin, v[j]);
                            vmax = fmaxf(vmax, v[j]);
                        }
                    const int64_t c = R.c1 + (tk.a / R.o2g) * R.i2 + i;
                    atomicMin(&mn[c], enc_ord(vmin));
                    atomicMax(&mx[c], enc_ord(vmax));
                    continue;
                }
                int64_t g_prev = -1;
                for (int64_t o = tk.a; o < tk.b; ++o) {
                    const int64_t g = o / R.o2g;
                    if (g != g_prev && g_prev >= 0) {
                        atomicMin(&mn[R.c1 + g_prev * R.i2 + i], enc_ord(vmin));
                        atomicMax(&mx[R.c1 + g_prev * R.i2 + i], enc_ord(vmax));
                        vmin = INFINITY;
                        vmax = -INFINITY;
                    }
                    g_prev = g;
                    const DFQ_GLOBAL float* p = (const DFQ_GLOBAL float*)(R.w2 + o * rowlen + i * R.khw2);
                    for (int64_t k = 0; k < R.khw2; ++k) {
                        vmin = fminf(vmin, p[k]);
                        vmax = fmaxf(vmax, p[k]);
                    }
                }
                if (g_prev >= 0) {
                    atomicMin(&mn[R.c1 + g_prev * R.i2 + i], enc_ord(vmin));
                    atomicMax(&mx[R.c1 + g_prev * R.i2 + i], enc_ord(vmax));
                }
            }
        } else {
            const int64_t off = R.moff + (tk.kind == kRangeReset ? R.c1 : 0);
            for (int64_t c = tk.a + threadIdx.x; c < tk.b; c += kThreads) {
                omins[off + c] = 0xFFFFFFFFu;
                omaxs[off + c] = 0u;
            }
        }
    }
}

__global__ void __launch_bounds__(kThreads)
cle_loop_range_kernel(const CleRel* __restrict__ rels, const CleTask* __restrict__ tasks, int64_t t0, int64_t t1,
                      uint32_t* __restrict__ rng, int64_t M, const CleState* __restrict__ st, int next) {
    __shared__ float tl[2 * kThreads * kTileMaxKhw];
    if (st->done) return;
    cle_range_body(rels, tasks, t0, t1, rng, M, (st->iters + next) & 1, blockIdx.x, gridDim.x, tl);
}

__device__ __forceinline__ CleScale cle_rel_scale(const CleRel* __restrict__ rels, const CleRel& R,
                                                  const uint32_t* __restrict__ mins, const uint32_t* __restrict__ maxs,
                                                  int64_t c, int is_signed, float eps, double smin, double smax) {
    if (R.dw_prev < 0) return cle_scale(mins + R.moff, maxs + R.moff, R.c1, c, is_signed, eps, smin, smax);
    const CleRel& Q = rels[R.dw_prev];
    const CleScale q = cle_scale(mins + Q.moff, maxs + Q.moff, Q.c1, c, is_signed, eps, smin, smax);
    const float mn1 = dec_ord(mins[Q.moff + Q.c1 + c]) * q.inv;
    const float mx1 = dec_ord(maxs[Q.moff + Q.c1 + c]) * q.inv;
    return cle_scale_from(mn1, mx1, dec_ord(mins[R.moff + R.c1 + c]), dec_ord(maxs[R.moff + R.c1 + c]), is_signed, eps,
                          smin, smax);
}

struct CleApplyLds {
    float red[2][kThreads / 64][kColTileRows];
    float inv_s[kThreads];
    float inv_pos[kThreads * kTileMaxKhw];
    float rows[kColTileRows * kThreads];
};

#ifdef DFQ_DIAGNOSTICS
__device__ uint64_t* g_cle_tl = nullptr;
__device__ uint64_t* g_cle_tl2 = nullptr;
__device__ int64_t g_cle_tl2_a0 = -1;
constexpr int kCleTl2Fin = 8192;
#endif

template <bool POS = true>
__device__ __forceinline__ void cle_apply_body(const CleRel* __restrict__ rels, const CleTask* __restrict__ tasks,
                                               int64_t t0, int64_t t1, uint32_t* __restrict__ rng, int64_t M,
                                               int par, bool first_iter, int is_signed, float eps, double smin,
                                               double smax, int64_t blk, int64_t nblk, CleApplyLds& A,
                                               float* __restrict__ vsave = nullptr, int32_t* __restrict__ vtag = nullptr,
                                               int32_t iter = 0) {
    auto& red = A.red;
    float* rows = A.rows;
    float* inv_s = A.inv_s;
    float* inv_pos = A.inv_pos;
    uint32_t* mins = rng + (int64_t)par * 2 * M;
    uint32_t* maxs = mins + M;
    uint32_t* nmins = rng + (int64_t)(par ^ 1) * 2 * M;
    uint32_t* nmaxs = nmins + M;
    const int lane = threadIdx.x & 63;
    const int wv = threadIdx.x >> 6;
    for (int64_t t = t0 + blk; t < t1; t += nblk) {
#ifdef DFQ_DIAGNOSTICS
        const bool tl_on = g_cle_tl != nullptr;
        const uint64_t tl_start = tl_on ? __builtin_amdgcn_s_memrealtime() : 0;
        uint64_t tl_sub = 0;
#define DFQ_CLE_TL_MARK(k) \
        if (tl_on) tl_sub |= (1ull << 63) | (((__builtin_amdgcn_s_memrealtime() - tl_start) & 0xffffull) << (16 * (k)));
#else
#define DFQ_CLE_TL_MARK(k)
#endif
        const CleTask tk = tasks[t];
        const CleRel& R = rels[tk.rel];
        const uint32_t* mn = mins + R.moff;
        const uint32_t* mx = maxs + R.moff;
        if (tk.kind == kApplyW1 && R.len1 < 64) {
            for_short_rows(tk.a, tk.b, R.len1, [&](int64_t c, bool act, int sl, int G) {
                float y0 = INFINITY, y1 = -INFINITY;
                if (act && sl < R.len1) {
                    DFQ_GLOBAL float* p = (DFQ_GLOBAL float*)(R.w1 + c * R.len1 + sl);
                    const float x = *p;
                    const float y = x * cle_rel_scale(rels, R, mins, maxs, c, is_signed, eps, smin, smax).s;
                    *p = y;
                    y0 = y1 = y;
                }
                if (R.w1_self) {
                    y0 = group_min(y0, G);
                    y1 = group_max(y1, G);
                    if (act && sl == 0) {
                        nmins[R.moff + c] = enc_ord(y0);
                        nmaxs[R.moff + c] = enc_ord(y1);
                    }
                }
            });
        } else if (tk.kind == kApplyDwBoth && R.o2g * R.khw2 < 64) {
            const CleRel& N = rels[tk.c0];
            const int64_t seg = R.o2g * R.khw2;
            for_short_rows(tk.a, tk.b, seg, [&](int64_t c, bool act, int sl, int G) {
                float z0 = INFINITY, z1 = -INFINITY;
                if (act && sl < seg) {
                    DFQ_GLOBAL float* p = (DFQ_GLOBAL float*)(R.w2 + c * seg + sl);
                    const float x = *p;
                    const float inv = cle_rel_scale(rels, R, mins, maxs, c, is_signed, eps, smin, smax).inv;
                    const float sn = cle_rel_scale(rels, N, mins, maxs, c, is_signed, eps, smin, smax).s;
                    const float y = x * inv;
                    const float z = y * sn;
                    *p = z;
                    z0 = z1 = z;
                }
                if (R.w2_self) {
                    z0 = group_min(z0, G);
                    z1 = group_max(z1, G);
                    if (act && sl == 0) {
                        nmins[R.moff + R.c1 + c] = enc_ord(z0);
                        nmaxs[R.moff + R.c1 + c] = enc_ord(z1);
                    }
                }
            });
        } else if (tk.kind == kApplyW2Contig && R.o2g * R.khw2 < 64) {
            const int64_t seg = R.o2g * R.khw2;
            const bool fuse = R.fuse_next >= 0;
            for_short_rows(tk.a, tk.b, seg, [&](int64_t c, bool act, int sl, int G) {
                float vmin = INFINITY, vmax = -INFINITY;
                if (act && sl < seg) {
                    DFQ_GLOBAL float* p = (DFQ_GLOBAL float*)(R.w2 + c * seg + sl);
                    const float x = *p;
                    const float y = x * cle_rel_scale(rels, R, mins, maxs, c, is_signed, eps, smin, smax).inv;
                    *p = y;
                    vmin = vmax = y;
                }
                if (fuse) {
                    vmin = group_min(vmin, G);
                    vmax = group_max(vmax, G);
                    if (act && sl == 0) {
                        const int64_t off = rels[R.fuse_next].moff;
                        mins[off + c] = enc_ord(vmin);
                        maxs[off + c] = enc_ord(vmax);
                    }
                }
            });
        } else if (tk.kind == kApplyW1) {
            for (int64_t c = tk.a + wv; c < tk.b; c += kThreads / 64) {
                auto sc = [&] { return cle_rel_scale(rels, R, mins, maxs, c, is_signed, eps, smin, smax).s; };
                if (R.w1_self) {
                    float y0, y1;
                    wave_scale_mm(R.w1 + c * R.len1, R.len1, R.vec1, lane, y0, y1, sc);
                    if (lane == 0) {
                        nmins[R.moff + c] = enc_ord(y0);
                        nmaxs[R.moff + c] = enc_ord(y1);
                    }
                } else {
                    wave_scale(R.w1 + c * R.len1, R.len1, R.vec1, lane, sc);
                }
            }
        } else if (tk.kind == kApplyDwBoth) {
            const CleRel& N = rels[tk.c0];
            const int64_t seg = R.o2g * R.khw2;
            for (int64_t c = tk.a + wv; c < tk.b; c += kThreads / 64) {
                const float inv = cle_rel_scale(rels, R, mins, maxs, c, is_signed, eps, smin, smax).inv;
                const float sn = cle_rel_scale(rels, N, mins, maxs, c, is_signed, eps, smin, smax).s;
                DFQ_GLOBAL float* p = (DFQ_GLOBAL float*)(R.w2 + c * seg);
                float z0 = INFINITY, z1 = -INFINITY;
                for (int64_t i = lane; i < seg; i += 64) {
                    const float y = p[i] * inv;
                    const float z = y * sn;
                    p[i] = z;
                    z0 = fminf(z0, z);
                    z1 = fmaxf(z1, z);
                }
                if (R.w2_self) {
                    cle_wave_minmax(z0, z1);
                    if (lane == 0) {
                        nmins[R.moff + R.c1 + c] = enc_ord(z0);
                        nmaxs[R.moff + R.c1 + c] = enc_ord(z1);
                    }
                }
            }
        } else if (tk.kind == kApplyW2Contig) {
            const int64_t seg = R.o2g * R.khw2;
            for (int64_t c = tk.a + wv; c < tk.b; c += kThreads / 64) {
                auto inv = [&] { return cle_rel_scale(rels, R, mins, maxs, c, is_signed, eps, smin, smax).inv; };
                if (R.fuse_next >= 0) {
                    float vmin, vmax;
                    wave_scale_range(R.w2 + c * seg, seg, lane, vmin, vmax, inv);
                    if (lane == 0) {
                        const int64_t off = rels[R.fuse_next].moff;
                        mins[off + c] = enc_ord(vmin);
                        maxs[off + c] = enc_ord(vmax);
                    }
                } else {
                    wave_scale(R.w2 + c * seg, seg, R.vec2, lane, inv);
                }
            }
        } else if (POS && tk.kind == kApplyW2Tile && tile_by_position(R, tk) && tk.b - tk.a <= kPosTileMaxRows) {
            const int t = threadIdx.x;
            const int khw = (int)R.khw2;
            const int64_t rowlen = R.i2 * R.khw2;
            const int ncol = (int)(tk.c1 - tk.c0);
            const int npos = ncol * khw;
            DFQ_GLOBAL float* base = (DFQ_GLOBAL float*)(R.w2 + tk.c0 * R.khw2);
            const bool fuse = R.fuse_next >= 0;
            if (t < ncol)
                inv_s[t] = cle_rel_scale(rels, R, mins, maxs, (tk.a / R.o2g) * R.i2 + tk.c0 + t, is_signed, eps, smin, smax).inv;
            __syncthreads();
            DFQ_CLE_TL_MARK(0)
            for (int q = t; q < npos; q += kThreads) inv_pos[q] = inv_s[q / khw];
            __syncthreads();
            DFQ_CLE_TL_MARK(1)
            float v[kPosTileMaxRows][kTileMaxKhw];
#pragma unroll
            for (int r = 0; r < kPosTileMaxRows; ++r) {
                const DFQ_GLOBAL float* rb = base + (tk.a + r) * rowlen;
#pragma unroll
                for (int m = 0; m < kTileMaxKhw; ++m)
                    if (tk.a + r < tk.b && m < khw && t + kThreads * m < npos) v[r][m] = rb[t + kThreads * m];
            }
#pragma unroll
            for (int r = 0; r < kPosTileMaxRows; ++r) {
                if (tk.a + r >= tk.b) break;
                DFQ_GLOBAL float* rp = base + (tk.a + r) * rowlen;
                float lo = INFINITY, hi = -INFINITY;
#pragma unroll
                for (int m = 0; m < kTileMaxKhw; ++m)
                    if (m < khw && t + kThreads * m < npos) {
                        const float y = v[r][m] * inv_pos[t + kThreads * m];
                        rp[t + kThreads * m] = y;
                        lo = fminf(lo, y);
                        hi = fmaxf(hi, y);
                    }
                if (fuse) {
                    cle_wave_minmax(lo, hi);
                    if (lane == 0) {
                        red[0][wv][r] = lo;
                        red[1][wv][r] = hi;
                    }
                }
            }
            __syncthreads();
            DFQ_CLE_TL_MARK(2)
            if (fuse && t < tk.b - tk.a) {
                float a = red[0][0][t], b = red[1][0][t];
                for (int w = 1; w < kThreads / 64; ++w) {
                    a = fminf(a, red[0][w][t]);
                    b = fmaxf(b, red[1][w][t]);
                }
                const int64_t off = rels[R.fuse_next].moff + tk.a + t;
                atomicMin(&mins[off], enc_ord(a));
                atomicMax(&maxs[off], enc_ord(b));
            }
            __syncthreads();
        } else if (tk.kind == kApplyW2Tile && R.fuse_next >= 0) {
            const int64_t rowlen = R.i2 * R.khw2;
            const int64_t i = tk.c0 + threadIdx.x;
            const bool act = i < tk.c1;
            const bool one_group = (tk.a / R.o2g) == ((tk.b - 1) / R.o2g);
            const int nr = (int)(tk.b - tk.a);
            if (one_group && R.khw2 == 1) {
                float v[kColTileRows];
#pragma unroll
                for (int j = 0; j < kColTileRows; ++j)
                    if (act && j < nr) v[j] = ((DFQ_GLOBAL float*)R.w2)[(tk.a + j) * rowlen + i];
                const float inv =
                    act ? cle_rel_scale(rels, R, mins, maxs, (tk.a / R.o2g) * R.i2 + i, is_signed, eps, smin, smax).inv : 0.f;
#pragma unroll
                for (int j = 0; j < kColTileRows; ++j) {
                    if (j < nr) {
                        float y = __builtin_nanf("");
                        if (act) {
                            y = v[j] * inv;
                            ((DFQ_GLOBAL float*)R.w2)[(tk.a + j) * rowlen + i] = y;
                        }
                        rows[j * kThreads + threadIdx.x] = y;
                    }
                    if (j == 0) {
                        DFQ_CLE_TL_MARK(0)
                    }
                }
                DFQ_CLE_TL_MARK(1)
                block_lds_sync();
                const int r = threadIdx.x >> 4, sg = threadIdx.x & 15;
                float lo = INFINITY, hi = -INFINITY;
                if (r < nr) {
                    const float4* q = reinterpret_cast<const float4*>(rows + r * kThreads + sg * 16);
#pragma unroll
                    for (int u = 0; u < 4; ++u) {
                        const float4 x = q[u];
                        lo = fminf(lo, fminf(fminf(x.x, x.y), fminf(x.z, x.w)));
                        hi = fmaxf(hi, fmaxf(fmaxf(x.x, x.y), fmaxf(x.z, x.w)));
                    }
                }
                lo = fminf(lo, dpp_f(lo, 0xB1));
                hi = fmaxf(hi, dpp_f(hi, 0xB1));
                lo = fminf(lo, dpp_f(lo, 0x4E));
                hi = fmaxf(hi, dpp_f(hi, 0x4E));
                lo = fminf(lo, dpp_f(lo, 0x141));
                hi = fmaxf(hi, dpp_f(hi, 0x141));
                lo = fminf(lo, dpp_f(lo, 0x140));
                hi = fmaxf(hi, dpp_f(hi, 0x140));
                DFQ_CLE_TL_MARK(2)
                if (sg == 0 && r < nr) {
                    const int64_t off = rels[R.fuse_next].moff + tk.a + r;
                    atomicMin(&mins[off], enc_ord(lo));
                    atomicMax(&maxs[off], enc_ord(hi));
                }
            } else {
                int64_t g_prev = -1;
                float inv = 0.f;
                for (int j = 0; j < nr; ++j) {
                    const int64_t o = tk.a + j;
                    float lo = INFINITY, hi = -INFINITY;
                    if (act) {
                        const int64_t g = o / R.o2g;
                        if (g != g_prev) {
                            inv = cle_rel_scale(rels, R, mins, maxs, g * R.i2 + i, is_signed, eps, smin, smax).inv;
                            g_prev = g;
                        }
                        DFQ_GLOBAL float* p = (DFQ_GLOBAL float*)(R.w2 + o * rowlen + i * R.khw2);
                        for (int64_t k = 0; k < R.khw2; ++k) {
                            const float y = p[k] * inv;
                            p[k] = y;
                            lo = fminf(lo, y);
                            hi = fmaxf(hi, y);
                        }
                    }
                    float a = lo, b = hi;
                    cle_wave_minmax(a, b);
                    if (lane == 0) {
                        red[0][wv][j] = a;
                        red[1][wv][j] = b;
                    }
                }
                __syncthreads();
                if (threadIdx.x < tk.b - tk.a) {
                    const int j = threadIdx.x;
                    float a = red[0][0][j], b = red[1][0][j];
                    for (int w = 1; w < kThreads / 64; ++w) {
                        a = fminf(a, red[0][w][j]);
                        b = fmaxf(b, red[1][w][j]);
                    }
                    const int64_t off = rels[R.fuse_next].moff + tk.a + j;
                    atomicMin(&mins[off], enc_ord(a));
                    atomicMax(&maxs[off], enc_ord(b));
                }
            }
            __syncthreads();
        } else if (tk.kind == kApplyW2Tile) {
            const int64_t rowlen = R.i2 * R.khw2;
            const bool one_group = (tk.a / R.o2g) == ((tk.b - 1) / R.o2g);
            for (int64_t i = tk.c0 + threadIdx.x; i < tk.c1; i += kThreads) {
                if (one_group && R.khw2 == 1) {
                    float v[kColTileRows];
#pragma unroll
                    for (int j = 0; j < kColTileRows; ++j)
                        if (tk.a + j < tk.b) v[j] = ((DFQ_GLOBAL float*)R.w2)[(tk.a + j) * rowlen + i];
                    const float inv = cle_rel_scale(rels, R, mins, maxs, (tk.a / R.o2g) * R.i2 + i, is_signed, eps, smin,
                                                smax).inv;
                    ((DFQ_GLOBAL float*)R.w2)[tk.a * rowlen + i] = v[0] * inv;
                    DFQ_CLE_TL_MARK(0)
#pragma unroll
                    for (int j = 1; j < kColTileRows; ++j)
                        if (tk.a + j < tk.b) ((DFQ_GLOBAL float*)R.w2)[(tk.a + j) * rowlen + i] = v[j] * inv;
                    DFQ_CLE_TL_MARK(1)
                    continue;
                }
                int64_t g_prev = -1;
                float inv = 0.f;
                for (int64_t o = tk.a; o < tk.b; ++o) {
                    const int64_t g = o / R.o2g;
                    if (g != g_prev) {
                        inv = cle_rel_scale(rels, R, mins, maxs, g * R.i2 + i, is_signed, eps, smin, smax).inv;
                        g_prev = g;
                    }
                    DFQ_GLOBAL float* p = (DFQ_GLOBAL float*)(R.w2 + o * rowlen + i * R.khw2);
                    for (int64_t k = 0; k < R.khw2; ++k) p[k] = p[k] * inv;
                }
            }
        } else {
            if (vtag && threadIdx.x == 0) vtag[t] = iter;
            for (int64_t c = tk.a + threadIdx.x; c < tk.b; c += kThreads) {
                const CleScale cs = cle_rel_scale(rels, R, mins, maxs, c, is_signed, eps, smin, smax);
                if (vsave) {
                    float* v = vsave + 2 * R.moff;
                    if (R.b1) v[c] = R.b1[c];
                    if (R.bnw) v[R.c1 + c] = R.bnw[c];
                    if (R.bnb) v[2 * R.c1 + c] = R.bnb[c];
                    if (R.sacc) v[3 * R.c1 + c] = R.sacc[c];
                }
                if (R.b1) R.b1[c] = R.b1[c] * cs.s;
                if (R.bnw) R.bnw[c] = R.bnw[c] * cs.s;
                if (R.bnb) R.bnb[c] = R.bnb[c] * cs.s;
                if (R.sacc) R.sacc[c] = (R.sacc_init && first_iter) ? cs.s : R.sacc[c] * cs.s;
            }
        }
#ifdef DFQ_DIAGNOSTICS
        if (tl_on) {
            __syncthreads();
            if (threadIdx.x == 0) {
                uint32_t hw, xcc;
                asm volatile("s_getreg_b32 %0, hwreg(HW_REG_HW_ID)" : "=s"(hw));
                asm volatile("s_getreg_b32 %0, hwreg(HW_REG_XCC_ID)" : "=s"(xcc));
                uint64_t* r = g_cle_tl + 4 * t;
                r[0] = tl_start;
                r[1] = __builtin_amdgcn_s_memrealtime();
                r[2] = tl_sub ? tl_sub : (((uint64_t)xcc << 32) | hw);
                r[3] = (uint64_t)tk.kind | ((uint64_t)tk.rel << 8) | ((uint64_t)(tk.b - tk.a) << 24);
            }
        }
#endif
    }
}


__global__ void __launch_bounds__(kThreads)
cle_loop_init_kernel(const CleLayer* __restrict__ layers, const CleChunk* __restrict__ chunks, int64_t nchunks,
                     const CleUnit* __restrict__ units, int64_t nunits, uint32_t* __restrict__ rng, int64_t M,
                     float* __restrict__ part, int64_t npart, uint32_t* __restrict__ cnt, int64_t ncnt,
                     int32_t* __restrict__ vtag, int64_t nvtag, CleState* __restrict__ st, CleState init) {
    const int64_t gt = (int64_t)blockIdx.x * kThreads + threadIdx.x, gs = (int64_t)gridDim.x * kThreads;
    for (int64_t i = gt; i < 4 * M; i += gs) rng[i] = ((i / M) & 1) ? 0u : 0xFFFFFFFFu;
    for (int64_t i = gt; i < npart; i += gs) part[i] = 0.f;
    for (int64_t i = gt; i < ncnt; i += gs) cnt[i] = 0u;
    for (int64_t i = gt; i < nvtag; i += gs) vtag[i] = -1;
    if (gt == 0) *st = init;
    for (int64_t u = blockIdx.x; u < nunits; u += gridDim.x) {
        const CleUnit un = units[u];
        const CleChunk ch = chunks[un.chunk];
        const CleLayer Ly = layers[ch.layer];
        const int64_t nb1 = (ch.len / 32) / 256;
        const int64_t e0 = (int64_t)un.tile * 8192;
        const int64_t e1 = un.tile < nb1 ? e0 + 8192 : ch.len;
        for (int64_t i = e0 + threadIdx.x; i < e1; i += kThreads) Ly.snap[ch.c0 + i] = Ly.w[ch.c0 + i];
    }
    if (blockIdx.x == 0)
        for (int64_t k = 0; k < nchunks; ++k) {
            const CleChunk ch = chunks[k];
            if (ch.len >= 8) continue;
            const CleLayer Ly = layers[ch.layer];
            for (int64_t i = threadIdx.x; i < ch.len; i += kThreads) Ly.snap[ch.c0 + i] = Ly.w[ch.c0 + i];
        }
}


struct CleNoUnitHook {
    __device__ void operator()(const CleUnit&, const CleChunk&, int64_t) const {}
};

template <class Hook = CleNoUnitHook>
__device__ __forceinline__ void cle_tiles_body(const CleLayer* __restrict__ layers, const CleChunk* __restrict__ chunks,
                                               const int64_t* __restrict__ b1off, const CleUnit* __restrict__ units,
                                               int64_t nunits, float* __restrict__ b1buf, float* __restrict__ tailbuf,
                                               int64_t blk, int64_t nblk, float* d, float* b0, Hook hook = Hook()) {
    const int tid = threadIdx.x;
    for (int64_t u = blk; u < nunits; u += nblk) {
        const CleUnit un = units[u];
        const CleChunk ch = chunks[un.chunk];
        const CleLayer Ly = layers[ch.layer];
        const DFQ_GLOBAL float* __restrict__ w = (const DFQ_GLOBAL float*)(Ly.w + ch.c0);
        DFQ_GLOBAL float* __restrict__ sn = (DFQ_GLOBAL float*)(Ly.snap + ch.c0);
        const int64_t len = ch.len, sz = len / 32, vs = len / 8;
        const int64_t nb1 = sz / 256;
        const bool full = un.tile < nb1;
        const int64_t e0 = (int64_t)un.tile * kCleTile;
        const int64_t cnt = full ? kCleTile : len - e0;
        if (full) {
            float xs[2][16], ys[2][16];
#pragma unroll
            for (int h = 0; h < 2; ++h) {
                const int q = tid + h * kThreads;
                const int64_t base = e0 + 32 * (16 * (q >> 5)) + (q & 31);
#pragma unroll
                for (int j = 0; j < 16; ++j) {
                    xs[h][j] = w[base + 32 * j];
                    ys[h][j] = sn[base + 32 * j];
                }
            }
#pragma unroll
            for (int h = 0; h < 2; ++h) {
                const int q = tid + h * kThreads;
                const int64_t base = e0 + 32 * (16 * (q >> 5)) + (q & 31);
                float a = 0.f;
#pragma unroll
                for (int j = 0; j < 16; ++j) {
                    a += fabsf(xs[h][j] - ys[h][j]);
                    sn[base + 32 * j] = xs[h][j];
                }
                b0[q] = a;
            }
            __syncthreads();
            if (tid < 32) {
                float a = 0.f;
#pragma unroll
                for (int m = 0; m < 16; ++m) a += b0[m * 32 + tid];
                st_coh(b1buf + b1off[un.chunk] + (int64_t)un.tile * 32 + tid, a);
            }
        } else {
            for (int64_t e = tid; e < cnt; e += 8 * kThreads) {
                float x[8], y[8];
#pragma unroll
                for (int u = 0; u < 8; ++u)
                    if (e + u * kThreads < cnt) {
                        x[u] = w[e0 + e + u * kThreads];
                        y[u] = sn[e0 + e + u * kThreads];
                    }
#pragma unroll
                for (int u = 0; u < 8; ++u)
                    if (e + u * kThreads < cnt) {
                        d[e + u * kThreads] = fabsf(x[u] - y[u]);
                        sn[e0 + e + u * kThreads] = x[u];
                    }
            }
            __syncthreads();
            const int64_t ni = sz - nb1 * 256;
            const int64_t rem_b0 = ni / 16, tail0 = ni % 16;
            float* tb = tailbuf + (int64_t)un.chunk * kCleTailWords;
            if (tid < 32) {
                float a1p = 0.f;
                for (int64_t m = 0; m < rem_b0; ++m) {
                    float a = 0.f;
                    for (int j = 0; j < 16; ++j) a += d[32 * (16 * m + j) + tid];
                    a1p += a;
                }
                float a0t = 0.f;
                for (int64_t j = 0; j < tail0; ++j) a0t += d[32 * (16 * rem_b0 + j) + tid];
                float p = a0t;
                p += a1p;
                st_coh(tb + tid, p);
            } else if (tid < 64) {
                const int t = tid - 32;
                const int64_t nv = vs - 4 * sz;
                if (t < 24 && t < nv * 8) st_coh(tb + 32 + t, d[8 * (4 * sz) + t - e0]);
                if (t < 8 && t < len - 8 * vs) st_coh(tb + 56 + t, d[8 * vs + t - e0]);
            }
        }
        __syncthreads();
        hook(un, ch, nb1);
    }
}

constexpr int kCleTilesLds = kCleTile + kCleTailWords + 512;
constexpr int kCleRangeLds = 2 * kThreads * kTileMaxKhw;

template <class LdB1, class LdTb>
__device__ __forceinline__ float cle_chunk_sum_with(const CleChunk& ch, LdB1&& b1, LdTb&& tb, int lane) {
    const int64_t len = ch.len;
    const int64_t sz = len / 32, vs = len / 8;
    const int64_t nb1 = sz / 256, nb2 = nb1 / 16, rem_b1 = nb1 % 16;
    float fa = 0.f;
    float p = 0.f;
    if (lane < 32) {
        float a3 = 0.f;
        for (int64_t r = 0; r < nb2; ++r) {
            float b2 = 0.f;
            for (int q = 0; q < 16; ++q) b2 += b1((r * 16 + q) * 32 + lane);
            a3 += b2;
        }
        float a2p = 0.f;
        for (int64_t q = 0; q < rem_b1; ++q) a2p += b1((nb2 * 16 + q) * 32 + lane);
        p = tb(lane);
        p += a2p;
        p += a3;
    }
    auto ps = [&](int s) { return rl_f(p, s); };
    for (int64_t e = 0; e < len - 8 * vs; ++e) fa += tb(56 + e);
    const int64_t nv = vs - 4 * sz;
    for (int l = 0; l < 8; ++l) {
        float p0 = ps(l);
        for (int64_t v = 0; v < nv; ++v) p0 += tb(32 + v * 8 + l);
        p0 += ps(l + 8);
        p0 += ps(l + 16);
        p0 += ps(l + 24);
        fa += p0;
    }
    return fa;
}

__device__ __forceinline__ float cle_chunk_sum(const CleChunk& ch, const float* b1, const float* tb, int lane) {
    const DFQ_GLOBAL float* g1 = (const DFQ_GLOBAL float*)b1;
    const DFQ_GLOBAL float* gt = (const DFQ_GLOBAL float*)tb;
    return cle_chunk_sum_with(ch, [g1](int64_t i) { return ld_coh(g1 + i); }, [gt](int64_t i) { return ld_coh(gt + i); },
                              lane);
}

__device__ __forceinline__ float cle_tiny_chunk_sum(const CleLayer* __restrict__ layers, const CleChunk& ch) {
    const CleLayer Ly = layers[ch.layer];
    float* w = Ly.w + ch.c0;
    float* sn = Ly.snap + ch.c0;
    return aten_inner_sum([&](int64_t e) {
        const float x = w[e];
        const float dd = fabsf(x - sn[e]);
        sn[e] = x;
        return dd;
    }, ch.len);
}

template <class P>
__device__ __forceinline__ double np_pairwise_leaf(P x, int64_t n) {
    if (n < 8) {
        double res = 0.;
        for (int64_t i = 0; i < n; ++i) res += x[i];
        return res;
    }
    double r[8];
#pragma unroll
    for (int j = 0; j < 8; ++j) r[j] = x[j];
    int64_t i;
    for (i = 8; i < n - (n % 8); i += 8)
#pragma unroll
        for (int j = 0; j < 8; ++j) r[j] += x[i + j];
    double res = ((r[0] + r[1]) + (r[2] + r[3])) + ((r[4] + r[5]) + (r[6] + r[7]));
    for (; i < n; ++i) res += x[i];
    return res;
}

struct NpFrame {
    int64_t o, n;
    int64_t state;
};
constexpr int kNpFrames = 48;
constexpr int kNpStackFloats = kNpFrames * (int)(sizeof(NpFrame) + sizeof(double)) / 4;
template <class P>
__device__ double np_pairwise(P a, int64_t n, float* stack) {
    if (n <= 128) return 0. + np_pairwise_leaf(a, n);
    NpFrame* fr = reinterpret_cast<NpFrame*>(stack);
    double* acc = reinterpret_cast<double*>(fr + kNpFrames);
    int fp = 0, ap = 0;
    fr[fp++] = {0, n, 0};
    while (fp > 0) {
        NpFrame& f = fr[fp - 1];
        if (f.n <= 128) {
            acc[ap++] = np_pairwise_leaf(a + f.o, f.n);
            --fp;
        } else if (f.state == 0) {
            int64_t n2 = f.n / 2;
            n2 -= n2 % 8;
            f.state = 1;
            const NpFrame left{f.o, n2, 0}, right{f.o + n2, f.n - n2, 0};
            fr[fp++] = right;
            fr[fp++] = left;
        } else {
            const double right = acc[--ap];
            const double left = acc[--ap];
            acc[ap++] = left + right;
            --fp;
        }
    }
    return 0. + acc[0];
}

template <bool kLeafOnly = false, bool kCoherent = false>
__device__ __forceinline__ void cle_final_body(const CleLayer* __restrict__ layers, int32_t nl,
                                               const float* __restrict__ part, int32_t S, double* __restrict__ means,
                                               double* __restrict__ hist, CleState* __restrict__ st, double* sm,
                                               float* part_lds = nullptr, float* np_stack = nullptr,
                                               uint32_t* hflag = nullptr) {
#ifdef DFQ_DIAGNOSTICS
    uint64_t* tlm = (kCoherent && threadIdx.x == 0 && g_cle_tl2) ? g_cle_tl2 + 4 * kCleTl2Fin : nullptr;
#endif
    constexpr int kStateWords = (int)(sizeof(CleState) / 4);
    static_assert(sizeof(CleState) % 4 == 0, "CleState: whole 4-B words");
    const int64_t nps = (int64_t)nl * (S + 2);
    DFQ_LDS float* pls = (DFQ_LDS float*)part_lds;
    if (part_lds) {
        for (int64_t i = threadIdx.x; i < nps + kStateWords; i += blockDim.x) {
            const DFQ_GLOBAL float* src = (const DFQ_GLOBAL float*)(i < nps ? part + i
                                                                           : reinterpret_cast<const float*>(st) + (i - nps));
            pls[i] = kCoherent ? ld_coh(src) : *src;
        }
        __syncthreads();
    }
#ifdef DFQ_DIAGNOSTICS
    if (tlm) tlm[2] = __builtin_amdgcn_s_memrealtime();
#endif
    DFQ_LDS double* ms = (DFQ_LDS double*)sm;
    DFQ_GLOBAL double* mg = (DFQ_GLOBAL double*)means;
    const bool m_lds = nl <= 1024;
    double* m = m_lds ? sm : means;
    for (int l = threadIdx.x; l < nl; l += blockDim.x) {
        const float* pl = (part_lds ? part_lds : part) + (int64_t)l * S;
        auto ld = [&](int64_t e) { return (part_lds || !kCoherent) ? pl[e] : ld_coh(pl + e); };
        const float* lm = part_lds ? part_lds + (int64_t)nl * S + 2 * l : nullptr;
        const bool serial = lm ? lm[1] != 0.f : layers[l].nt == 1;
        const float sum = serial ? 0.f + (0.f + ld(0)) : 0.f + aten_inner_sum([&](int64_t e) { return ld(e); }, S);
        m[l] = (double)(sum / (lm ? lm[0] : (float)layers[l].n));
    }
    __syncthreads();
#ifdef DFQ_DIAGNOSTICS
    if (tlm) tlm[3] = __builtin_amdgcn_s_memrealtime();
#endif
    if (threadIdx.x == 0) {
        CleState s0;
        if (part_lds) {
            __builtin_memcpy(&s0, part_lds + nps, sizeof(CleState));
        } else {
            s0 = *st;
        }
        double dt = 0.0;
        if constexpr (kLeafOnly) {
            dt = nl > 0 ? 0. + (m_lds ? np_pairwise_leaf(ms, nl) : np_pairwise_leaf(mg, nl)) : 0.0;
        } else {
            dt = nl > 0 ? (m_lds ? np_pairwise(ms, nl, np_stack) : np_pairwise(mg, nl, np_stack)) : 0.0;
        }
        const int it = s0.iters;
        hist[it] = dt;
        int ic = s0.iter_count;
        double diff = s0.diff;
        if (fabs(diff - dt) > 1e-9) {
            ic = 0;
            diff = dt;
        } else {
            ic += 1;
        }
        const bool cont = (diff > s0.thr) && (ic < s0.count);
        const int done = (!cont || it + 1 >= s0.max_iters) ? 1 : 0;
        st->iters = it + 1;
        st->iter_count = ic;
        st->diff = diff;
        st->done = done;
        if (hflag)
            __hip_atomic_store(hflag, ((uint32_t)(it + 1) << 1) | (uint32_t)done, __ATOMIC_RELAXED,
                               __HIP_MEMORY_SCOPE_SYSTEM);
    }
}

__device__ __forceinline__ bool handoff_arrive(uint32_t* c, uint32_t target) {
    return __hip_atomic_fetch_add(c, 1u, __ATOMIC_RELAXED, __HIP_MEMORY_SCOPE_AGENT) == target;
}

__host__ __device__ inline int64_t cle_stop_blocks(int64_t nchunks) {
    return nchunks > 0 ? (nchunks + kThreads / 64 - 1) / (kThreads / 64) : 1;
}

struct CleFin {
    uint32_t* cnt;
    float* part;
    double* means;
    double* hist;
    int64_t nchunks, nbig;
    int32_t S, nl;
    int32_t last;
    uint32_t* hflag;
    int32_t stop_arrival;
};

static_assert(kCleTilesLds - kCleTile >= kNpStackFloats, "np_pairwise's frame stack after the tile area");
union CleStepLds {
    CleApplyLds apply;
    float tiles[kCleTilesLds > kCleRangeLds ? kCleTilesLds : kCleRangeLds];
};

constexpr bool kCleTilesFirst = true;
#ifdef DFQ_DIAGNOSTICS
__device__ int g_cle_tiles_first = kCleTilesFirst ? 1 : 0;
#endif

template <bool POS>
#ifndef DFQ_CLE_POS_WAVES
#define DFQ_CLE_POS_WAVES 1
#endif
__global__ void __launch_bounds__(kThreads) __attribute__((amdgpu_waves_per_eu(POS ? DFQ_CLE_POS_WAVES : 4)))
cle_loop_step_kernel(const CleRel* __restrict__ rels, const CleTask* __restrict__ atasks, int64_t a0, int64_t a1,
                     int64_t nab, uint32_t* __restrict__ rng, int64_t M, int is_signed, float eps, double smin,
                     double smax, const CleLayer* __restrict__ layers, const CleChunk* __restrict__ chunks,
                     const int64_t* __restrict__ b1off, const CleUnit* __restrict__ units, int64_t uo, int64_t nuo,
                     int64_t nto, int64_t up, int64_t nup, int64_t ntp, float* __restrict__ b1buf,
                     float* __restrict__ tailbuf, const CleTask* __restrict__ rtasks, int64_t ro, int64_t nro_t,
                     int64_t nro, int64_t rp, int64_t nrp_t, int64_t nrp, CleFin F, CleState* __restrict__ st,
                     int32_t g, float* __restrict__ vsave, int32_t* __restrict__ vtag, int32_t stop_it) {
    __shared__ CleStepLds L;
    __shared__ int flag;
    if (st->done) return;
    int64_t blk = blockIdx.x;
#ifdef DFQ_DIAGNOSTICS
    const bool tiles_first = g_cle_tiles_first != 0;
#else
    constexpr bool tiles_first = kCleTilesFirst;
#endif
    const int64_t nstop = stop_it >= 0 ? cle_stop_blocks(F.nchunks) : 0;
    if (tiles_first) {
        const int64_t ns = nab + nstop, ntl = nto + ntp;
        if (blk < ntl) blk += ns;
        else if (blk < ntl + ns) blk -= ntl;
    }
    if (blk < nab) {
        cle_apply_body<POS>(rels, atasks, a0, a1, rng, M, g & 1, g == 0, is_signed, eps, smin, smax, blk, nab, L.apply,
                            vsave, vtag, g);
        return;
    }
    blk -= nab;
#ifdef DFQ_DIAGNOSTICS
    const bool tl2 = g_cle_tl2 != nullptr && blk < kCleTl2Fin && (g_cle_tl2_a0 < 0 || (a0 == g_cle_tl2_a0 && nab > 0));
    const uint64_t tl2_start = tl2 ? __builtin_amdgcn_s_memrealtime() : 0;
    auto tl2_rec = [&](int role) {
        if (tl2 && threadIdx.x == 0) {
            uint64_t* r = g_cle_tl2 + 4 * blk;
            r[0] = tl2_start;
            r[1] = __builtin_amdgcn_s_memrealtime();
            r[2] = (uint64_t)role;
        }
    };
#else
    auto tl2_rec = [](int) {};
#endif
    float* lds = L.tiles;
    auto finish = [&]() {
#ifdef DFQ_DIAGNOSTICS
        const uint64_t tf0 = __builtin_amdgcn_s_memrealtime();
#endif
        if (threadIdx.x == 0 && F.nchunks > F.nbig)
            for (int64_t k = 0; k < F.nchunks; ++k) {
                const CleChunk c2 = chunks[k];
                if (c2.len < 8) st_coh(F.part + (int64_t)c2.layer * F.S + c2.t, 0.f + cle_tiny_chunk_sum(layers, c2));
            }
        asm volatile("s_waitcnt vmcnt(0)" ::: "memory");
        __syncthreads();
        const bool stage_part = (int64_t)F.nl * (F.S + 2) + (int64_t)(sizeof(CleState) / 4) + 2048 <= kCleTile;
        if (F.nl <= 128)
            cle_final_body<true, true>(layers, F.nl, F.part, F.S, F.means, F.hist, st, reinterpret_cast<double*>(lds),
                                       stage_part ? lds + 2048 : nullptr, nullptr, F.hflag);
        else
            cle_final_body<false, true>(layers, F.nl, F.part, F.S, F.means, F.hist, st,
                                        reinterpret_cast<double*>(lds), stage_part ? lds + 2048 : nullptr,
                                        lds + kCleTile, F.hflag);
#ifdef DFQ_DIAGNOSTICS
        if (tl2 && threadIdx.x == 0) {
            uint64_t* r = g_cle_tl2 + 4 * kCleTl2Fin;
            r[0] = tf0;
            r[1] = __builtin_amdgcn_s_memrealtime();
        }
#endif
    };
    if (stop_it >= 0) {
        if (blk < nstop) {
            const int64_t c = blk * (kThreads / 64) + (threadIdx.x >> 6);
            if (c < F.nchunks) {
                const CleChunk ch = chunks[c];
                if (ch.len >= 8) {
                    const float fa = cle_chunk_sum(ch, b1buf + b1off[c], tailbuf + c * kCleTailWords, threadIdx.x & 63);
                    if ((threadIdx.x & 63) == 0) st_coh(F.part + (int64_t)ch.layer * F.S + ch.t, 0.f + fa);
                }
            }
            asm volatile("s_waitcnt vmcnt(0)" ::: "memory");
            __syncthreads();
            if (threadIdx.x == 0)
                flag = handoff_arrive(F.cnt + F.nchunks, ((uint32_t)stop_it + 1u) * (uint32_t)nstop - 1u);
            __syncthreads();
            if (flag) finish();
            return;
        }
        blk -= nstop;
    }
    const int64_t ntiles = nto + ntp;
    if (blk >= ntiles) {
        blk -= ntiles;
        const bool own = blk < nro;
        const int64_t b = own ? blk : blk - nro;
        cle_range_body(rels, rtasks, own ? ro : rp, (own ? ro : rp) + (own ? nro_t : nrp_t), rng, M,
                       own ? (g + 1) & 1 : g & 1, b, own ? nro : nrp, L.tiles);
        tl2_rec(2);
        return;
    }
    const bool own = blk < nto;
    const int32_t it = own ? g : g - 1;
    const int64_t tb = own ? blk : blk - nto;
    const int64_t tnb = own ? nto : ntp;
    const uint32_t round = (uint32_t)it + 1u;
    auto arrive = [&](uint32_t* c, uint32_t members) -> bool {
        asm volatile("s_waitcnt vmcnt(0)" ::: "memory");
        __syncthreads();
        if (threadIdx.x == 0) flag = handoff_arrive(c, round * members - 1u);
        __syncthreads();
        return flag != 0;
    };
    if (F.nbig == 0) {
        if (own && tb == 0 && F.last) finish();
        return;
    }
    const uint32_t fin_members = (uint32_t)F.nbig;
    auto hook = [&](const CleUnit& un, const CleChunk& ch, int64_t nb1) {
        if (!arrive(F.cnt + un.chunk, (uint32_t)(nb1 + 1))) return;
        {
            const float* gb1 = b1buf + b1off[un.chunk];
            const float* gtb = tailbuf + (int64_t)un.chunk * kCleTailWords;
            const int64_t nw = 32 * nb1;
            const bool staged = nw + kCleTailWords <= kCleTile;
            if (staged) {
                DFQ_LDS float* ll = (DFQ_LDS float*)lds;
                const DFQ_GLOBAL float* g1 = (const DFQ_GLOBAL float*)gb1;
                for (int64_t i = threadIdx.x; i < nw; i += kThreads) ll[i] = ld_coh(g1 + i);
                if (threadIdx.x < kCleTailWords) ll[nw + threadIdx.x] = ld_coh((const DFQ_GLOBAL float*)gtb + threadIdx.x);
            }
            __syncthreads();
            if (threadIdx.x < 64) {
                const float fa = staged ? cle_chunk_sum_with(ch, [&](int64_t i) { return lds[i]; },
                                                             [&](int64_t i) { return lds[nw + i]; }, threadIdx.x)
                                        : cle_chunk_sum(ch, gb1, gtb, threadIdx.x);
                if (threadIdx.x == 0) st_coh(F.part + (int64_t)ch.layer * F.S + ch.t, 0.f + fa);
            }
        }
        if (F.stop_arrival && arrive(F.cnt + F.nchunks, fin_members)) finish();
    };
    if (F.stop_arrival)
        cle_tiles_body<decltype(hook)>(layers, chunks, b1off, units + (own ? uo : up), own ? nuo : nup, b1buf, tailbuf,
                                       tb, tnb, lds, lds + kCleTile + kCleTailWords, hook);
    else
        cle_tiles_body(layers, chunks, b1off, units + (own ? uo : up), own ? nuo : nup, b1buf, tailbuf, tb, tnb, lds,
                       lds + kCleTile + kCleTailWords);
#ifdef DFQ_DIAGNOSTICS
    if (tl2) {
        const CleUnit un0 = units[(own ? uo : up) + tb];
        tl2_rec(un0.tile >= (chunks[un0.chunk].len / 32) / 256 ? 3 : 1);
    }
#else
    tl2_rec(1);
#endif
}

__global__ void __launch_bounds__(kThreads)
cle_loop_rollback_kernel(const CleLayer* __restrict__ layers, int32_t nl, const CleRel* __restrict__ rels,
                         const CleTask* __restrict__ atasks, int64_t n_at, const float* __restrict__ vsave,
                         const int32_t* __restrict__ vtag, const CleState* __restrict__ st) {
    const int32_t A = st->iters;
    const int64_t gt = (int64_t)blockIdx.x * kThreads + threadIdx.x, gs = (int64_t)gridDim.x * kThreads;
    for (int32_t l = 0; l < nl; ++l) {
        const CleLayer Ly = layers[l];
        for (int64_t i = gt; i < Ly.n; i += gs) Ly.w[i] = Ly.snap[i];
    }
    for (int64_t t = blockIdx.x; t < n_at; t += gridDim.x) {
        const CleTask tk = atasks[t];
        if (tk.kind != kApplyChannels || vtag[t] != A) continue;
        const CleRel& R = rels[tk.rel];
        const float* v = vsave + 2 * R.moff;
        for (int64_t c = tk.a + threadIdx.x; c < tk.b; c += kThreads) {
            if (R.b1) R.b1[c] = v[c];
            if (R.bnw) R.bnw[c] = v[R.c1 + c];
            if (R.bnb) R.bnb[c] = v[2 * R.c1 + c];
            if (R.sacc) R.sacc[c] = v[3 * R.c1 + c];
        }
    }
}


__global__ void __launch_bounds__(64) cle_caller_gate_kernel(const uint64_t* sig, uint64_t gen, uint64_t limit) {
    if (threadIdx.x != 0) return;
    const uint64_t t0 = __builtin_amdgcn_s_memrealtime();
    while (__hip_atomic_load(sig, __ATOMIC_RELAXED, __HIP_MEMORY_SCOPE_SYSTEM) < gen) {
        if (__builtin_amdgcn_s_memrealtime() - t0 > limit) __builtin_trap();
        __builtin_amdgcn_s_sleep(32);
    }
    __atomic_thread_fence(__ATOMIC_ACQUIRE);
}
}
```

### data_free_quantization_amd/csrc/dfq_cle_plan.cpp

```cpp
#include "dfq_cle_plan.h"

#include <algorithm>
#include <atomic>
#include <climits>
#include <cstdio>
#include <cstring>
#include <list>
#include <mutex>
#include <numeric>
#include <utility>

namespace dfq {

CleSwitches CleSwitches::from_env() {
    CleSwitches sw;
    auto rows = [](const char* name, int64_t dflt) {
        const char* e = ab_env(name);
        return e && *e ? std::max<int64_t>(1, atoll(e)) : dflt;
    };
    if (const char* e = ab_env("DFQ_CLE_FUSED")) sw.fused = e[0] != '0';
    sw.w1_mult = rows("DFQ_CLE_W1_ROWS", 0);
    sw.dw_mult = rows("DFQ_CLE_DW_ROWS", kCleDwRowsMult);
    if (const char* e = ab_env("DFQ_CLE_LAG")) sw.lag = e[0] != '0';
    if (const char* e = ab_env("DFQ_CLE_STOP")) sw.stop_arrival = e[0] == 'a';
    if (const char* e = ab_env("DFQ_CLE_BAND")) sw.band = atoi(e);
    return sw;
}
void CleSwitches::append_to(std::vector<int64_t>& key) const {
    key.insert(key.end(), {(int64_t)fused, w1_mult, dw_mult, (int64_t)lag, (int64_t)stop_arrival, (int64_t)band});
}

int cle_rels_from_desc(const dfq_cle_rel* rels, int32_t n_rel, std::vector<CleRel>& R, int64_t& M) {
    R.assign(n_rel, CleRel{});
    M = 0;
    for (int32_t r = 0; r < n_rel; ++r) {
        const dfq_cle_rel& d = rels[r];
        if (!d.w1 || !d.w2 || !d.b1 || d.c1 <= 0 || d.len1 <= 0 || d.o2 <= 0 || d.i2 <= 0 || d.khw2 <= 0)
            return DFQ_ERR_INVALID;
        int64_t groups = 1;
        if (d.c1 != d.i2) {
            groups = d.c1 / d.i2;
            if (groups <= 0 || groups * d.i2 != d.c1) return DFQ_ERR_SHAPE;
        }
        if (d.o2 % groups != 0) return DFQ_ERR_SHAPE;
        CleRel c{};
        c.w1 = d.w1; c.w2 = d.w2; c.b1 = d.b1; c.bnw = d.bn_w; c.bnb = d.bn_b; c.sacc = d.s_acc;
        c.c1 = d.c1; c.len1 = d.len1; c.o2 = d.o2; c.i2 = d.i2; c.khw2 = d.khw2; c.o2g = d.o2 / groups;
        c.moff = M;
        c.sacc_init = d.s_acc_init;
        c.vec1 = (d.len1 % 4 == 0 && reinterpret_cast<uintptr_t>(d.w1) % 16 == 0) ? 1 : 0;
        c.vec2 = (d.i2 == 1 && (c.o2g * d.khw2) % 4 == 0 && reinterpret_cast<uintptr_t>(d.w2) % 16 == 0) ? 1 : 0;
        c.fuse_next = -1;
        c.dw_prev = -1;
        c.w1_self = 0;
        c.w2_self = 0;
        M += 2 * d.c1;
        R[r] = c;
    }
    return DFQ_OK;
}

static int64_t cle_apply_elems(const CleTask& tk, const CleRel& q) {
    const int64_t n = tk.b - tk.a;
    switch (tk.kind) {
        case kApplyW1: return n * q.len1;
        case kApplyW2Tile: return n * (tk.c1 - tk.c0) * q.khw2;
        case kApplyChannels: return 0;
        default: return n * q.o2g * q.khw2;
    }
}
static int64_t cle_range_elems(const CleTask& tk, const CleRel& q) {
    const int64_t n = tk.b - tk.a;
    switch (tk.kind) {
        case kRangeW1: return n * q.len1;
        case kRangeW2Contig: return n * q.o2g * q.khw2;
        case kRangeW2Tile: return n * (tk.c1 - tk.c0) * q.khw2;
        default: return 0;
    }
}

struct CleChains {
    int32_t chains = 0, steps = 0;
    bool fused = true;
    std::vector<int32_t> step_of;
    std::vector<int32_t> w1_src;
    std::vector<int32_t> dw_next;
};

static CleChains cle_chains(std::vector<CleRel>& R, const CleSwitches& sw) {
    const int32_t n_rel = (int32_t)R.size();
    CleChains C;
    std::vector<int32_t> parent(n_rel);
    std::iota(parent.begin(), parent.end(), 0);
    auto find = [&](int32_t x) {
        while (parent[x] != x) x = parent[x] = parent[parent[x]];
        return x;
    };
    for (int32_t a = 0; a < n_rel; ++a) {
        const void* pa[5] = {R[a].w1, R[a].w2, R[a].b1, R[a].bnw, R[a].bnb};
        for (int32_t b = 0; b < a; ++b) {
            const void* pb[5] = {R[b].w1, R[b].w2, R[b].b1, R[b].bnw, R[b].bnb};
            bool share = false;
            for (int i = 0; i < 5 && !share; ++i)
                for (int j = 0; j < 5 && !share; ++j) share = pa[i] && pa[i] == pb[j];
            if (share) parent[find(a)] = find(b);
        }
    }
    std::vector<int32_t> comp_len(n_rel, 0);
    C.step_of.resize(n_rel);
    for (int32_t r = 0; r < n_rel; ++r) {
        const int32_t c = find(r);
        if (comp_len[c] == 0) ++C.chains;
        C.step_of[r] = comp_len[c]++;
        C.steps = std::max(C.steps, C.step_of[r] + 1);
    }
    C.w1_src.assign(n_rel, -1);
    C.fused = sw.fused;
    std::vector<std::vector<int32_t>> chain_of(n_rel);
    for (int32_t r = 0; r < n_rel; ++r) chain_of[find(r)].push_back(r);
    for (const auto& L : chain_of) {
        for (size_t j = 0; j < L.size() && C.fused; ++j) {
            const CleRel& cr = R[L[j]];
            for (size_t i = 0; i < j && C.fused; ++i) {
                const CleRel& cq = R[L[i]];
                if (cq.w1 == cr.w2 || cq.w2 == cr.w2) C.fused = false;
                if (cq.w1 == cr.w1 || cq.w2 == cr.w1) {
                    const bool ok = i + 1 == j && cq.w2 == cr.w1 && cq.w1 != cr.w1 && C.w1_src[L[j]] < 0 &&
                                    (cq.i2 > 1 || cq.o2g == 1) && cr.c1 == cq.o2 && cr.len1 == cq.i2 * cq.khw2;
                    if (ok) C.w1_src[L[j]] = L[i];
                    else C.fused = false;
                }
            }
        }
    }
    if (C.fused)
        for (int32_t r = 0; r < n_rel; ++r)
            if (C.w1_src[r] >= 0) R[C.w1_src[r]].fuse_next = r;
    C.dw_next.assign(n_rel, -1);
    if (C.fused) {
        for (int32_t r = 0; r < n_rel; ++r) {
            const int32_t q = C.w1_src[r];
            if (q < 0 || R[q].dw_prev >= 0 || C.dw_next[q] >= 0) continue;
            const CleRel& cq = R[q];
            const CleRel& cr = R[r];
            const bool dw = cq.i2 == 1 && cq.o2g == 1 && cq.o2 == cq.c1 && cr.c1 == cq.o2 && cr.len1 == cq.khw2;
            if (!dw) continue;
            R[r].dw_prev = q;
            R[q].fuse_next = -1;
            C.dw_next[q] = r;
        }
        std::vector<int32_t> cur(n_rel, 0);
        C.steps = 0;
        for (int32_t r = 0; r < n_rel; ++r) {
            const int32_t c = find(r);
            C.step_of[r] = R[r].dw_prev >= 0 ? C.step_of[R[r].dw_prev] : cur[c]++;
            C.steps = std::max(C.steps, C.step_of[r] + 1);
        }
    }
    return C;
}

struct CleTaskTables {
    std::vector<CleTask> rt, at;
    std::vector<int64_t> rstep{0}, astep{0};
    int64_t ri0 = 0, ri1 = 0;
};

static void cle_w2_range_tasks(const CleRel& c, int32_t r, std::vector<CleTask>& out) {
    if (c.i2 == 1) {
        const int64_t k = rows_per_task(c.o2g * c.khw2);
        for (int64_t a = 0; a < c.c1; a += k) out.push_back({r, kRangeW2Contig, a, std::min<int64_t>(a + k, c.c1), 0, 0});
    } else {
        for (int64_t a = 0; a < c.o2; a += kColTileRows)
            for (int64_t i0 = 0; i0 < c.i2; i0 += kThreads)
                out.push_back({r, kRangeW2Tile, a, std::min<int64_t>(a + kColTileRows, c.o2), i0,
                               std::min<int64_t>(i0 + kThreads, c.i2)});
        for (int64_t a = 0; a < c.c1; a += kCleChansPerTask)
            out.push_back({r, kRangeReset, a, std::min<int64_t>(a + kCleChansPerTask, c.c1), 0, 0});
    }
}
static void cle_w1_range_tasks(const CleRel& c, int32_t r, bool produced, std::vector<CleTask>& out) {
    if (c.dw_prev >= 0) return;
    const int32_t kind = produced ? kRangeResetW1 : kRangeW1;
    const int64_t k = produced ? kCleChansPerTask : rows_per_task(c.len1);
    for (int64_t a = 0; a < c.c1; a += k) out.push_back({r, kind, a, std::min<int64_t>(a + k, c.c1), 0, 0});
}
static void cle_apply_tasks(const CleRel& c, int32_t r, int32_t dw_next, const CleSwitches& sw,
                            std::vector<CleTask>& out) {
    if (c.dw_prev < 0) {
        int64_t k = rows_per_task(c.len1);
        k = sw.w1_mult > 0 ? sw.w1_mult * k : (k * c.len1 < kCleW1SmallElems ? 2 * k : k);
        for (int64_t a = 0; a < c.c1; a += k) out.push_back({r, kApplyW1, a, std::min<int64_t>(a + k, c.c1), 0, 0});
    }
    if (dw_next >= 0) {
        for (int64_t a = 0, k = sw.dw_mult * rows_per_task(c.o2g * c.khw2); a < c.c1; a += k)
            out.push_back({r, kApplyDwBoth, a, std::min<int64_t>(a + k, c.c1), dw_next, 0});
    } else if (c.i2 == 1) {
        for (int64_t a = 0, k = rows_per_task(c.o2g * c.khw2); a < c.c1; a += k)
            out.push_back({r, kApplyW2Contig, a, std::min<int64_t>(a + k, c.c1), 0, 0});
    } else {
        const int64_t rows = (c.khw2 > 1 && c.khw2 <= kTileMaxKhw) ? kPosTileMaxRows : kColTileRows;
        for (int64_t a = 0; a < c.o2; a += rows)
            for (int64_t i0 = 0; i0 < c.i2; i0 += kThreads)
                out.push_back({r, kApplyW2Tile, a, std::min<int64_t>(a + rows, c.o2), i0,
                               std::min<int64_t>(i0 + kThreads, c.i2)});
    }
    for (int64_t a = 0; a < c.c1; a += kThreads)
        out.push_back({r, kApplyChannels, a, std::min<int64_t>(a + kThreads, c.c1), 0, 0});
}

static CleTaskTables cle_tasks(std::vector<CleRel>& R, const CleChains& C, const CleSwitches& sw) {
    const int32_t n_rel = (int32_t)R.size();
    CleTaskTables T;
    auto range_tasks = [&](int32_t r) {
        cle_w1_range_tasks(R[r], r, C.fused && C.w1_src[r] >= 0, T.rt);
        cle_w2_range_tasks(R[r], r, T.rt);
    };
    if (C.fused) {
        for (int32_t r = 0; r < n_rel; ++r) range_tasks(r);
        T.rstep.push_back((int64_t)T.rt.size());
        for (int32_t r = 0; r < n_rel; ++r) {
            if (C.w1_src[r] < 0 && R[r].dw_prev < 0) R[r].w1_self = 1;
            if (C.dw_next[r] >= 0) R[r].w2_self = 1;
        }
        T.ri0 = (int64_t)T.rt.size();
        for (int64_t t = T.rstep[0]; t < T.rstep[1]; ++t) {
            const CleTask tk = T.rt[t];
            if (tk.kind == kRangeW1 && R[tk.rel].w1_self) continue;
            if (tk.kind == kRangeW2Contig && R[tk.rel].w2_self) continue;
            T.rt.push_back(tk);
        }
        T.ri1 = (int64_t)T.rt.size();
    }
    for (int32_t k = 0; k < C.steps; ++k) {
        for (int32_t r = 0; r < n_rel; ++r) {
            if (C.step_of[r] != k) continue;
            if (!C.fused) range_tasks(r);
            cle_apply_tasks(R[r], r, C.dw_next[r], sw, T.at);
        }
        auto prio = [](int32_t kind) {
            switch (kind) {
                case kApplyW2Tile: return 0;
                case kApplyChannels: return 1;
                case kApplyDwBoth: return 2;
                case kApplyW1: return 3;
                default: return 4;
            }
        };
        std::stable_sort(T.at.begin() + T.astep.back(), T.at.end(),
                         [&](const CleTask& x, const CleTask& y) { return prio(x.kind) < prio(y.kind); });
        if (!C.fused) T.rstep.push_back((int64_t)T.rt.size());
        T.astep.push_back((int64_t)T.at.size());
    }
    return T;
}

struct CleMetric {
    std::vector<CleLayer> layers;
    std::vector<CleChunk> chunks;
    std::vector<CleUnit> units;
    std::vector<int64_t> b1off;
    int64_t nb1_total = 0;
};

static int cle_metric(float* const* targets, const int64_t* target_n, int32_t n_targets, int32_t ref_threads,
                      CleMetric& X) {
    X.layers.resize(n_targets);
    for (int32_t l = 0; l < n_targets; ++l) {
        const int64_t n = target_n[l];
        if (!targets[l] || n <= 0) return DFQ_ERR_INVALID;
        X.layers[l] = CleLayer{nullptr, nullptr, n, 1};
        int64_t nt = 1;
        if (n >= 32768 && ref_threads > 1) nt = std::min<int64_t>(ref_threads, ceil_div(n, (int64_t)32768));
        X.layers[l].nt = nt;
        const int64_t chunk = ceil_div(n, nt);
        for (int64_t t = 0; t < nt; ++t) {
            const int64_t b = t * chunk;
            if (b >= n) break;
            const int64_t len = std::min<int64_t>(n, b + chunk) - b;
            const int64_t sz = len / 32;
            if (aten_ceil_log2(sz) / 4 > 4) return DFQ_ERR_UNSUPPORTED;
            const int32_t ci = (int32_t)X.chunks.size();
            X.chunks.push_back(CleChunk{l, (int32_t)t, b, len});
            const int64_t nb1 = sz / 256;
            X.b1off.push_back(32 * X.nb1_total);
            X.nb1_total += nb1;
            if (len >= 8)
                for (int64_t g = 0; g <= nb1; ++g) X.units.push_back(CleUnit{ci, (int32_t)g});
        }
    }
    return DFQ_OK;
}

struct ClePlacement {
    std::vector<int32_t> layer_off;
    std::vector<int32_t> rt_off;
    int32_t nlaunch = 0;
    int32_t stop_off = -1;
    bool lagged = false;
};

struct CleSpans {
    std::vector<const float*> w;
    std::vector<std::pair<int32_t, int32_t>> v;
    std::vector<int32_t> rel_t1, rel_t2;
    std::vector<int32_t> lay_t;
    int32_t find(const float* p) const {
        for (size_t i = 0; i < w.size(); ++i)
            if (w[i] == p) return (int32_t)i;
        return -1;
    }
};
static CleSpans cle_spans(const std::vector<CleRel>& R, const CleChains& C, float* const* targets, int32_t n_targets) {
    const int32_t n_rel = (int32_t)R.size();
    CleSpans P;
    P.rel_t1.resize(n_rel);
    P.rel_t2.resize(n_rel);
    for (int32_t r = 0; r < n_rel; ++r)
        for (int side = 0; side < 2; ++side) {
            const float* w = side ? R[r].w2 : R[r].w1;
            int32_t i = P.find(w);
            if (i < 0) {
                i = (int32_t)P.w.size();
                P.w.push_back(w);
                P.v.push_back({C.step_of[r], C.step_of[r]});
            } else {
                P.v[i] = {std::min(P.v[i].first, C.step_of[r]), std::max(P.v[i].second, C.step_of[r])};
            }
            (side ? P.rel_t2 : P.rel_t1)[r] = i;
        }
    P.lay_t.resize(n_targets);
    for (int32_t l = 0; l < n_targets; ++l) P.lay_t[l] = P.find(targets[l]);
    return P;
}

static bool cle_place_lagged(int32_t nl, const std::vector<CleRel>& R, const CleChains& C, const CleTaskTables& T,
                             const CleSpans& P, const int64_t* target_n, int32_t n_targets, const CleSwitches& sw,
                             ClePlacement& out, int32_t& lag_max) {
    auto window = [&](int32_t ti) -> std::pair<int32_t, int32_t> {
        if (ti < 0) return {0, 2 * nl - 1};
        return {P.v[ti].second + 1, std::min(2 * nl - 1, nl + P.v[ti].first - 1)};
    };
    std::vector<double> base_load(nl, 0.0);
    for (int32_t k = 0; k < C.steps && k < nl; ++k)
        for (int64_t t = T.astep[k]; t < T.astep[k + 1]; ++t)
            base_load[k] += 8.0 * (double)cle_apply_elems(T.at[t], R[T.at[t].rel]);
    const int64_t nr = T.ri1 - T.ri0;
    std::vector<std::pair<int32_t, int32_t>> rwin((size_t)nr);
    std::vector<double> rbytes((size_t)nr);
    for (int64_t x = 0; x < nr; ++x) {
        const CleTask& tk = T.rt[T.ri0 + x];
        std::pair<int32_t, int32_t> w;
        switch (tk.kind) {
            case kRangeW1: w = window(P.rel_t1[tk.rel]); break;
            case kRangeW2Contig:
            case kRangeW2Tile: w = window(P.rel_t2[tk.rel]); break;
            case kRangeReset:
                w = {C.step_of[tk.rel] + 1, std::min(2 * nl - 1, nl + P.v[P.rel_t2[tk.rel]].second)};
                break;
            default:
                w = {C.step_of[tk.rel] + 1, 2 * nl - 1};
        }
        if (w.first > w.second) return false;
        rwin[x] = w;
        rbytes[x] = tk.kind >= kRangeReset ? 64.0 : 4.0 * (double)cle_range_elems(tk, R[tk.rel]);
    }
    int32_t maxlo = 0, minhi = 2 * nl - 1;
    std::vector<std::pair<int32_t, int32_t>> lwin(n_targets);
    for (int32_t l = 0; l < n_targets; ++l) {
        lwin[l] = window(P.lay_t[l]);
        if (lwin[l].first > lwin[l].second) return false;
        maxlo = std::max(maxlo, lwin[l].first);
        minhi = std::min(minhi, lwin[l].second);
    }
    const int32_t bw = sw.stop_arrival ? nl : nl - 1;
    if (bw < 1) return false;
    const int32_t b_lo = std::max(0, maxlo - bw + 1), b_hi = std::min(minhi, 2 * nl - 1 - bw);
    if (b_lo > b_hi) return false;
    std::vector<int32_t> lord(n_targets);
    std::iota(lord.begin(), lord.end(), 0);
    std::sort(lord.begin(), lord.end(),
              [&](int32_t x, int32_t y) { return target_n[x] != target_n[y] ? target_n[x] > target_n[y] : x < y; });
    std::vector<int64_t> rord((size_t)nr);
    std::iota(rord.begin(), rord.end(), 0);
    std::sort(rord.begin(), rord.end(),
              [&](int64_t x, int64_t y) { return rbytes[x] != rbytes[y] ? rbytes[x] > rbytes[y] : x < y; });
    double best = 1e300;
    std::vector<int32_t> roff((size_t)nr), loff(n_targets);
    for (int32_t B0 = b_lo; B0 <= b_hi; ++B0) {
        if (sw.band >= 0 && B0 != sw.band && sw.band >= b_lo && sw.band <= b_hi) continue;
        std::vector<double> load = base_load;
        auto pick = [&](int32_t lo, int32_t hi, double bytes) {
            int32_t bo = lo;
            for (int32_t o = lo; o <= hi; ++o)
                if (load[o % nl] < load[bo % nl]) bo = o;
            load[bo % nl] += bytes;
            return bo;
        };
        for (int64_t x : rord) roff[x] = pick(rwin[x].first, rwin[x].second, rbytes[x]);
        int32_t maxoff = 0;
        for (int32_t l : lord) {
            loff[l] = pick(std::max(lwin[l].first, B0), std::min(lwin[l].second, B0 + bw - 1), 12.0 * target_n[l]);
            maxoff = std::max(maxoff, loff[l]);
        }
        if (!sw.stop_arrival && maxoff + 1 > 2 * nl - 1) continue;
        double cost = *std::max_element(load.begin(), load.end());
        if (cost < best) {
            best = cost;
            out.layer_off = loff;
            out.rt_off = roff;
            out.stop_off = sw.stop_arrival ? -1 : maxoff + 1;
            lag_max = maxoff;
        }
    }
    return best < 1e300;
}

static ClePlacement cle_place(const std::vector<CleRel>& R, const CleChains& C, const CleTaskTables& T,
                              const CleMetric& X, float* const* targets, const int64_t* target_n, int32_t n_targets,
                              const CleSwitches& sw) {
    const bool tiny = std::any_of(X.chunks.begin(), X.chunks.end(), [](const CleChunk& c) { return c.len < 8; });
    const bool have_tiles = std::any_of(X.chunks.begin(), X.chunks.end(), [](const CleChunk& c) { return c.len >= 8; });
    const bool lag_ok = C.fused && !tiny && have_tiles && C.steps > 0 && sw.lag;
    ClePlacement P;
    int32_t lag_max = -1;
    if (lag_ok &&
        cle_place_lagged(C.steps, R, C, T, cle_spans(R, C, targets, n_targets), target_n, n_targets, sw, P, lag_max) &&
        (sw.stop_arrival ? lag_max >= C.steps : P.stop_off >= C.steps)) {
        P.nlaunch = C.steps;
        P.lagged = true;
    } else {
        P.nlaunch = C.steps + 1;
        P.stop_off = -1;
        P.layer_off.assign(n_targets, C.steps);
        P.rt_off.assign((size_t)(T.ri1 - T.ri0), C.steps);
    }
    return P;
}

static void cle_bucket(const ClePlacement& P, bool fused, CleTaskTables& T, CleMetric& X, std::vector<int64_t>& uoffs,
                       std::vector<int64_t>& roffs) {
    const int32_t nb = 2 * P.nlaunch;
    uoffs.assign(nb + 1, 0);
    roffs.assign(nb + 1, 0);
    std::vector<std::vector<CleUnit>> ub(nb);
    for (const CleUnit& u : X.units) ub[P.layer_off[X.chunks[u.chunk].layer]].push_back(u);
    X.units.clear();
    for (int32_t k = 0; k < nb; ++k) {
        uoffs[k] = (int64_t)X.units.size();
        X.units.insert(X.units.end(), ub[k].begin(), ub[k].end());
    }
    uoffs[nb] = (int64_t)X.units.size();
    if (!fused) return;
    std::vector<std::vector<CleTask>> rb(nb);
    for (int64_t t = T.ri0; t < T.ri1; ++t) rb[P.rt_off[t - T.ri0]].push_back(T.rt[t]);
    T.rt.resize(T.ri0);
    for (int32_t k = 0; k < nb; ++k) {
        roffs[k] = (int64_t)T.rt.size();
        T.rt.insert(T.rt.end(), rb[k].begin(), rb[k].end());
    }
    roffs[nb] = T.ri1 = (int64_t)T.rt.size();
}

static void cle_bytes(CleStructure& S) {
    for (const CleTask& tk : S.at) {
        const CleRel& q = S.R[tk.rel];
        if (tk.kind == kApplyChannels)
            S.bytes_rescale += 8 * (tk.b - tk.a) * ((q.b1 ? 1 : 0) + (q.bnw ? 1 : 0) + (q.bnb ? 1 : 0) + (q.sacc ? 1 : 0));
        else
            S.bytes_rescale += 8 * cle_apply_elems(tk, q);
    }
    for (const CleLayer& l : S.layers) S.bytes_metric += 12 * l.n;
    const int64_t r0 = S.fused ? S.ri0 : 0, r1 = S.fused ? S.ri1 : (int64_t)S.rt.size();
    for (int64_t t = r0; t < r1; ++t) S.bytes_range += 4 * cle_range_elems(S.rt[t], S.R[S.rt[t].rel]);
}

static std::atomic<uint64_t> g_struct_ids{0};

int cle_build_structure(std::vector<CleRel> R, int64_t M, float* const* targets, const int64_t* target_n,
                        int32_t n_targets, int32_t ref_threads, const CleSwitches& sw, CleStructure& S) {
    const double tp1 = now_us();
    const CleChains C = cle_chains(R, sw);
    const double tp2 = now_us();
    CleTaskTables T = cle_tasks(R, C, sw);
    const double tp3 = now_us();
    CleMetric X;
    if (const int rc = cle_metric(targets, target_n, n_targets, ref_threads, X); rc != DFQ_OK) return rc;
    const double tp4 = now_us();
    const ClePlacement P = cle_place(R, C, T, X, targets, target_n, n_targets, sw);
    cle_bucket(P, C.fused, T, X, S.uoffs, S.roffs);
    S.R = std::move(R);
    S.M = M;
    S.chains = C.chains;
    S.steps = C.steps;
    S.fused = C.fused;
    S.rt = std::move(T.rt);
    S.at = std::move(T.at);
    S.rstep = std::move(T.rstep);
    S.astep = std::move(T.astep);
    S.ri0 = T.ri0;
    S.ri1 = T.ri1;
    S.layers = std::move(X.layers);
    S.chunks = std::move(X.chunks);
    S.units = std::move(X.units);
    S.b1off = std::move(X.b1off);
    S.nb1_total = X.nb1_total;
    S.nlaunch = P.nlaunch;
    S.stop_off = P.stop_off;
    S.lagged = P.lagged;
    S.step_pos.assign(std::max<int32_t>(S.steps, 1), 0);
    for (int32_t k = 0; k < S.steps; ++k)
        for (int64_t t = S.astep[k]; t < S.astep[k + 1]; ++t)
            if (S.at[t].kind == kApplyW2Tile && S.R[S.at[t].rel].khw2 > 1) S.step_pos[k] = 1;
    for (const CleChunk& c : S.chunks) S.nbig += c.len >= 8 ? 1 : 0;
    S.id = ++g_struct_ids;
    cle_bytes(S);
    const double tp5 = now_us();
    S.t_chains = tp2 - tp1;
    S.t_tasks = tp3 - tp2;
    S.t_chunks = tp4 - tp3;
    S.t_place = tp5 - tp4;
    return DFQ_OK;
}

static std::vector<int64_t> cle_structure_key(const std::vector<CleRel>& R, int64_t M, float* const* targets,
                                              const int64_t* target_n, int32_t n_targets, int32_t ref_threads,
                                              const CleSwitches& sw) {
    std::vector<std::pair<uintptr_t, int32_t>> ps;
    ps.reserve(5 * R.size() + n_targets);
    for (const CleRel& c : R)
        for (const void* q : {(const void*)c.w1, (const void*)c.w2, (const void*)c.b1, (const void*)c.bnw,
                              (const void*)c.bnb})
            ps.push_back({reinterpret_cast<uintptr_t>(q), (int32_t)ps.size()});
    for (int32_t l = 0; l < n_targets; ++l) ps.push_back({reinterpret_cast<uintptr_t>(targets[l]), (int32_t)ps.size()});
    std::vector<int32_t> id(ps.size());
    std::vector<std::pair<uintptr_t, int32_t>> srt = ps;
    std::sort(srt.begin(), srt.end());
    for (size_t i = 0; i < srt.size();) {
        size_t j = i;
        while (j < srt.size() && srt[j].first == srt[i].first) ++j;
        for (size_t k = i; k < j; ++k) id[srt[k].second] = srt[i].first ? srt[i].second : -1;
        i = j;
    }
    std::vector<int64_t> key;
    key.reserve(16 * R.size() + 2 * n_targets + 16);
    key.push_back((int64_t)R.size());
    key.push_back(M);
    key.push_back(n_targets);
    key.push_back(ref_threads);
    sw.append_to(key);
    size_t q = 0;
    for (const CleRel& c : R) {
        key.insert(key.end(), {c.c1, c.len1, c.o2, c.i2, c.khw2, (int64_t)c.sacc_init, (int64_t)c.vec1, (int64_t)c.vec2,
                               (int64_t)(c.sacc != nullptr)});
        for (int k = 0; k < 5; ++k) key.push_back(id[q++]);
    }
    for (int32_t l = 0; l < n_targets; ++l) {
        key.push_back(target_n[l]);
        key.push_back(id[q++]);
    }
    return key;
}

std::shared_ptr<const CleStructure> cle_structure_cached(const std::vector<CleRel>& R, int64_t M,
                                                         float* const* targets, const int64_t* target_n,
                                                         int32_t n_targets, int32_t ref_threads, int& rc, bool& cached) {
    static std::mutex mu;
    static std::list<std::pair<std::vector<int64_t>, std::shared_ptr<const CleStructure>>> cache;
    constexpr size_t kCap = 8;
    rc = DFQ_OK;
    cached = false;
    const CleSwitches sw = CleSwitches::from_env();
    const std::vector<int64_t> key = cle_structure_key(R, M, targets, target_n, n_targets, ref_threads, sw);
    {
        std::lock_guard<std::mutex> lock(mu);
        for (auto it = cache.begin(); it != cache.end(); ++it)
            if (it->first == key) {
                cache.splice(cache.begin(), cache, it);
                cached = true;
                return it->second;
            }
    }
    auto built = std::make_shared<CleStructure>();
    rc = cle_build_structure(R, M, targets, target_n, n_targets, ref_threads, sw, *built);
    if (rc != DFQ_OK) return nullptr;
    std::lock_guard<std::mutex> lock(mu);
    cache.emplace_front(key, built);
    if (cache.size() > kCap) cache.pop_back();
    return built;
}

}

#ifdef DFQ_DIAGNOSTICS
#include "dfq_diag.h"
using namespace dfq;

static uint64_t cle_structure_digest(const CleStructure& S) {
    uint64_t h = 0xcbf29ce484222325ull;
    auto put = [&](int64_t v) {
        for (int i = 0; i < 8; ++i) h = (h ^ (((uint64_t)v >> (8 * i)) & 0xff)) * 0x100000001b3ull;
    };
    auto put_all = [&](const std::vector<int64_t>& v) {
        put((int64_t)v.size());
        for (int64_t x : v) put(x);
    };
    auto put_tasks = [&](const std::vector<CleTask>& v) {
        put((int64_t)v.size());
        for (const CleTask& t : v)
            for (int64_t x : {(int64_t)t.rel, (int64_t)t.kind, t.a, t.b, t.c0, t.c1}) put(x);
    };
    for (int64_t x : {S.M, (int64_t)S.chains, (int64_t)S.steps, (int64_t)S.fused, (int64_t)S.lagged, (int64_t)S.nlaunch,
                      (int64_t)S.stop_off, S.ri0, S.ri1, S.nb1_total})
        put(x);
    put((int64_t)S.R.size());
    for (const CleRel& c : S.R)
        for (int64_t x : {c.moff, (int64_t)c.vec1, (int64_t)c.vec2, (int64_t)c.fuse_next, (int64_t)c.dw_prev,
                          (int64_t)c.w1_self, (int64_t)c.w2_self, c.o2g})
            put(x);
    put_tasks(S.at);
    put_tasks(S.rt);
    put_all(S.rstep);
    put_all(S.astep);
    put((int64_t)S.layers.size());
    for (const CleLayer& l : S.layers) put(l.n), put(l.nt);
    put((int64_t)S.chunks.size());
    for (const CleChunk& c : S.chunks) put(c.layer), put(c.t), put(c.c0), put(c.len);
    put((int64_t)S.units.size());
    for (const CleUnit& u : S.units) put(u.chunk), put(u.tile);
    put_all(S.b1off);
    put_all(S.uoffs);
    put_all(S.roffs);
    put(S.bytes_rescale), put(S.bytes_metric), put(S.bytes_range);
    return h;
}

extern "C" int dfq_diag_cle_check_structure(const dfq_cle_rel* rels, int32_t n_rel, float* const* targets,
                                            const int64_t* target_n, int32_t n_targets, int32_t ref_threads,
                                            int64_t* info, char* msg, int32_t msg_cap) {
    auto fail = [&](const char* fmt, long long a, long long b, long long c) {
        if (msg && msg_cap > 0) snprintf(msg, (size_t)msg_cap, fmt, a, b, c);
        return DFQ_ERR_INVALID;
    };
    if (n_rel < 0 || n_targets < 0 || (n_rel > 0 && !rels) || (n_targets > 0 && (!targets || !target_n)))
        return fail("bad arguments %lld %lld %lld", n_rel, n_targets, 0);
    std::vector<CleRel> R0;
    int64_t M = 0;
    if (const int rc = cle_rels_from_desc(rels, n_rel, R0, M); rc != DFQ_OK) return rc;
    CleStructure S;
    if (const int rc = cle_build_structure(R0, M, targets, target_n, n_targets, ref_threads, CleSwitches::from_env(), S);
        rc != DFQ_OK)
        return rc;
    const std::vector<CleRel>& R = S.R;
    const int32_t steps = S.steps, NL = S.nlaunch;
    if (const char* e = getenv("DFQ_CLE_PLACE_DUMP"); e && *e) {
        fprintf(stderr, "DFQ_CLE_PLACE steps %d nlaunch %d lagged %d stop_off %d\n", steps, NL, (int)S.lagged,
                S.stop_off);
        for (int32_t k = 0; k < 2 * NL; ++k) {
            int64_t na = 0;
            double ba = 0;
            if (k < steps)
                for (int64_t t = S.astep[k]; t < S.astep[k + 1]; ++t, ++na)
                    ba += 8.0 * (double)cle_apply_elems(S.at[t], R[S.at[t].rel]);
            double bu = 0;
            for (int64_t u = S.uoffs[k]; u < S.uoffs[k + 1]; ++u) {
                const CleChunk& ch = S.chunks[S.units[u].chunk];
                const int64_t nb1 = ch.len / kCleTile;
                bu += 12.0 * (S.units[u].tile < nb1 ? kCleTile : ch.len - nb1 * kCleTile);
            }
            double br = 0;
            for (int64_t t = S.roffs[k]; t < S.roffs[k + 1]; ++t)
                br += 4.0 * (double)cle_range_elems(S.rt[t], R[S.rt[t].rel]);
            fprintf(stderr, "DFQ_CLE_PLACE offset %d: rescale %lld blocks %.2f MB, tiles %lld blocks %.2f MB, ranges %lld blocks %.2f MB\n",
                    k, (long long)na, ba / 1e6, (long long)(S.uoffs[k + 1] - S.uoffs[k]), bu / 1e6,
                    (long long)(S.roffs[k + 1] - S.roffs[k]), br / 1e6);
        }
    }
    if (info) {
        const int64_t v[8] = {steps, NL, S.lagged ? 1 : 0, S.stop_off, (int64_t)S.at.size(), (int64_t)S.rt.size(),
                              (int64_t)S.units.size(), (int64_t)S.chunks.size()};
        std::memcpy(info, v, sizeof(v));
    }
    for (int32_t r = 0; r < n_rel; ++r) {
        const CleRel& c = R[r];
        if (c.moff < 0 || c.moff + 2 * c.c1 > S.M) return fail("rel %lld: range words [%lld, +2 c1) past M %lld", r, c.moff, S.M);
        if (2 * c.moff + 4 * c.c1 > 2 * S.M) return fail("rel %lld: rollback saves past 2 M (moff %lld, c1 %lld)", r, c.moff, c.c1);
        if (c.fuse_next >= n_rel || c.dw_prev >= n_rel || c.fuse_next < -1 || c.dw_prev < -1)
            return fail("rel %lld: link out of range (fuse_next %lld, dw_prev %lld)", r, c.fuse_next, c.dw_prev);
        if (c.fuse_next >= 0 && R[c.fuse_next].moff + R[c.fuse_next].c1 > S.M)
            return fail("rel %lld: fused W1 words of rel %lld past M %lld", r, c.fuse_next, S.M);
    }
    if ((int32_t)S.astep.size() != steps + 1 || S.astep[0] != 0 || S.astep.back() != (int64_t)S.at.size())
        return fail("astep: %lld entries for %lld steps, last %lld", (long long)S.astep.size(), steps,
                    S.astep.empty() ? -1 : S.astep.back());
    std::vector<int32_t> rel_step(n_rel, -1);
    std::vector<std::pair<const float*, int32_t>> touch;
    if ((int32_t)S.step_pos.size() != std::max<int32_t>(steps, 1) || (steps == 0 && S.step_pos[0] != 0))
        return fail("step_pos: %lld entries for %lld steps (first %lld)", (long long)S.step_pos.size(), steps,
                    S.step_pos.empty() ? -1 : S.step_pos[0]);
    for (int32_t k = 0; k < steps; ++k) {
        if (S.astep[k + 1] < S.astep[k]) return fail("astep not monotone at step %lld: %lld > %lld", k, S.astep[k], S.astep[k + 1]);
        bool pos = false;
        for (int64_t t = S.astep[k]; t < S.astep[k + 1]; ++t) {
            const CleTask& tk = S.at[t];
            if (tk.rel < 0 || tk.rel >= n_rel) return fail("rescale task %lld: relation %lld of %lld", t, tk.rel, n_rel);
            const CleRel& c = R[tk.rel];
            if (tk.a < 0 || tk.a >= tk.b) return fail("rescale task %lld: empty or negative span [%lld, %lld)", t, tk.a, tk.b);
            switch (tk.kind) {
                case kApplyW1:
                    if (tk.b > c.c1) return fail("W1 task %lld: rows to %lld of %lld", t, tk.b, c.c1);
                    touch.push_back({c.w1, k});
                    break;
                case kApplyW2Contig:
                    if (tk.b > c.c1 || c.i2 != 1) return fail("W2 contig task %lld: channels to %lld of %lld", t, tk.b, c.c1);
                    touch.push_back({c.w2, k});
                    break;
                case kApplyDwBoth:
                    if (tk.b > c.c1 || tk.c0 < 0 || tk.c0 >= n_rel || R[tk.c0].w1 != c.w2 || R[tk.c0].dw_prev != tk.rel)
                        return fail("depthwise pair task %lld: partner %lld, channels to %lld", t, tk.c0, tk.b);
                    touch.push_back({c.w2, k});
                    break;
                case kApplyW2Tile:
                    if (tk.b > c.o2 || tk.c0 < 0 || tk.c0 >= tk.c1 || tk.c1 > c.i2)
                        return fail("W2 tile task %lld: rows to %lld, columns to %lld", t, tk.b, tk.c1);
                    touch.push_back({c.w2, k});
                    pos = pos || c.khw2 > 1;
                    break;
                case kApplyChannels:
                    if (tk.b > c.c1) return fail("channel task %lld: channels to %lld of %lld", t, tk.b, c.c1);
                    if (rel_step[tk.rel] >= 0 && rel_step[tk.rel] != k)
                        return fail("relation %lld: channel tasks in steps %lld and %lld", tk.rel, rel_step[tk.rel], k);
                    rel_step[tk.rel] = k;
                    break;
                default:
                    return fail("rescale task %lld: kind %lld", t, tk.kind, 0);
            }
        }
        if ((S.step_pos[k] != 0) != pos)
            return fail("step %lld: step_pos %lld, its tasks say %lld (the wrong step kernel)", k, S.step_pos[k], pos);
    }
    for (int32_t r = 0; r < n_rel; ++r)
        if (rel_step[r] < 0) return fail("relation %lld has no channel task", r, 0, 0);
    const int64_t nrt = (int64_t)S.rt.size();
    if (S.ri0 < 0 || S.ri0 > S.ri1 || S.ri1 > nrt) return fail("range slice [%lld, %lld) of %lld tasks", S.ri0, S.ri1, nrt);
    for (int64_t t = 0; t < nrt; ++t) {
        const CleTask& tk = S.rt[t];
        if (tk.rel < 0 || tk.rel >= n_rel) return fail("range task %lld: relation %lld of %lld", t, tk.rel, n_rel);
        const CleRel& c = R[tk.rel];
        if (tk.a < 0 || tk.a >= tk.b) return fail("range task %lld: span [%lld, %lld)", t, tk.a, tk.b);
        const bool ok = tk.kind == kRangeW2Tile ? (tk.b <= c.o2 && tk.c0 >= 0 && tk.c0 < tk.c1 && tk.c1 <= c.i2)
                                                : (tk.kind >= kRangeW1 && tk.kind <= kRangeResetW1 && tk.b <= c.c1);
        if (!ok) return fail("range task %lld (kind %lld): span to %lld out of the relation's shape", t, tk.kind, tk.b);
    }
    int64_t nb1_seen = 0, nbig_seen = 0;
    for (size_t ci = 0; ci < S.chunks.size(); ++ci) {
        const CleChunk& ch = S.chunks[ci];
        if (ch.layer < 0 || ch.layer >= n_targets) return fail("chunk %lld: layer %lld of %lld", (long long)ci, ch.layer, n_targets);
        if (ch.c0 < 0 || ch.len <= 0 || ch.c0 + ch.len > target_n[ch.layer])
            return fail("chunk %lld: elements [%lld, +%lld) past its layer", (long long)ci, ch.c0, ch.len);
        const int64_t nb1 = ch.len / 32 / 256;
        if (S.b1off[ci] != 32 * nb1_seen) return fail("chunk %lld: level-1 offset %lld, expected %lld", (long long)ci, S.b1off[ci], 32 * nb1_seen);
        nb1_seen += nb1;
        nbig_seen += ch.len >= 8 ? 1 : 0;
    }
    if (nb1_seen != S.nb1_total) return fail("level-1 slots %lld, table %lld", nb1_seen, S.nb1_total, 0);
    if (nbig_seen != S.nbig) return fail("chunks with tiles %lld, nbig %lld", nbig_seen, S.nbig, 0);
    for (size_t u = 0; u < S.units.size(); ++u) {
        const CleUnit& un = S.units[u];
        if (un.chunk < 0 || un.chunk >= (int32_t)S.chunks.size()) return fail("unit %lld: chunk %lld", (long long)u, un.chunk, 0);
        const CleChunk& ch = S.chunks[un.chunk];
        if (ch.len < 8 || un.tile < 0 || un.tile > ch.len / 32 / 256)
            return fail("unit %lld: tile %lld of chunk %lld", (long long)u, un.tile, un.chunk);
        const int64_t nb1 = ch.len / 32 / 256, e0 = (int64_t)un.tile * kCleTile;
        if (un.tile < nb1 ? e0 + kCleTile > ch.len : (ch.len - e0 < 0 || ch.len - e0 > kCleTile + kCleTailWords))
            return fail("unit %lld: tile past chunk %lld (len %lld)", (long long)u, un.chunk, ch.len);
    }
    if ((int32_t)S.uoffs.size() != 2 * NL + 1 || S.uoffs[0] != 0 || S.uoffs.back() != (int64_t)S.units.size())
        return fail("uoffs: %lld entries for %lld launches, last %lld", (long long)S.uoffs.size(), NL, S.uoffs.back());
    for (int32_t k = 0; k < 2 * NL; ++k)
        if (S.uoffs[k + 1] < S.uoffs[k]) return fail("uoffs not monotone at %lld", k, 0, 0);
    if (S.fused) {
        if ((int32_t)S.roffs.size() != 2 * NL + 1 || S.roffs[0] != S.ri0 || S.roffs.back() != S.ri1)
            return fail("roffs: %lld entries, [%lld, %lld)", (long long)S.roffs.size(), S.roffs.empty() ? -1 : S.roffs[0],
                        S.roffs.empty() ? -1 : S.roffs.back());
        for (int32_t k = 0; k < 2 * NL; ++k)
            if (S.roffs[k + 1] < S.roffs[k]) return fail("roffs not monotone at %lld", k, 0, 0);
    } else if ((int32_t)S.rstep.size() != steps + 1 || S.rstep.back() != nrt) {
        return fail("unfused rstep: %lld entries, last %lld of %lld", (long long)S.rstep.size(), S.rstep.back(), nrt);
    }
    if (NL != (S.lagged ? steps : steps + 1)) return fail("nlaunch %lld for %lld steps (lagged %lld)", NL, steps, S.lagged);
    auto span = [&](const float* w, int32_t& first, int32_t& last) {
        first = INT32_MAX;
        last = -1;
        for (const auto& x : touch)
            if (x.first == w) {
                first = std::min(first, x.second);
                last = std::max(last, x.second);
            }
        return last >= 0;
    };
    auto in_window = [&](const float* w, int32_t o) {
        int32_t f, l;
        if (!span(w, f, l)) return o >= 0 && o <= 2 * NL - 1;
        return o >= l + 1 && o <= std::min(2 * NL - 1, NL + f - 1);
    };
    int32_t umin = INT32_MAX, umax = -1;
    for (int32_t k = 0; k < 2 * NL; ++k)
        for (int64_t u = S.uoffs[k]; u < S.uoffs[k + 1]; ++u) {
            const int32_t l = S.chunks[S.units[u].chunk].layer;
            if (!S.lagged && k != steps) return fail("unit %lld of layer %lld at offset %lld outside the tiles-only launch", u, l, k);
            if (!in_window(targets[l], k)) return fail("unit %lld of layer %lld at offset %lld outside its tensor's window", u, l, k);
            umin = std::min(umin, k);
            umax = std::max(umax, k);
        }
    if (S.fused)
        for (int32_t k = 0; k < 2 * NL; ++k)
            for (int64_t t = S.roffs[k]; t < S.roffs[k + 1]; ++t) {
                const CleTask& tk = S.rt[t];
                const CleRel& c = R[tk.rel];
                bool ok = true;
                switch (tk.kind) {
                    case kRangeW1: ok = in_window(c.w1, k); break;
                    case kRangeW2Contig:
                    case kRangeW2Tile: ok = in_window(c.w2, k); break;
                    case kRangeReset: {
                        int32_t f, l;
                        span(c.w2, f, l);
                        ok = k >= rel_step[tk.rel] + 1 && k <= std::min(2 * NL - 1, NL + l);
                        break;
                    }
                    default: ok = k >= rel_step[tk.rel] + 1 && k <= 2 * NL - 1;
                }
                if (!S.lagged && k != steps) ok = false;
                if (!ok) return fail("range task %lld (kind %lld) at offset %lld outside its window", t, tk.kind, k);
            }
    if (S.lagged && S.stop_off >= 0) {
        if (S.stop_off < steps || S.stop_off > 2 * NL - 1) return fail("stop rule at offset %lld of [%lld, %lld]", S.stop_off, steps, 2 * NL - 1);
        if (umax >= 0 && S.stop_off <= umax) return fail("stop rule at offset %lld, not after the last tile offset %lld", S.stop_off, umax, 0);
        if (umax >= 0 && umin + NL <= S.stop_off)
            return fail("the next iteration's first tile (offset %lld + %lld) not after the stop rule at %lld", umin, NL, S.stop_off);
    } else if (!S.lagged && S.stop_off != -1) {
        return fail("unlagged plan with a stop-rule offset %lld", S.stop_off, 0, 0);
    }
    if (msg && msg_cap > 0) snprintf(msg, (size_t)msg_cap, "digest %016llx", (unsigned long long)cle_structure_digest(S));
    return DFQ_OK;
}
#endif
```

### data_free_quantization_amd/csrc/dfq_cle_plan.h

```cpp
#pragma once
#include <stdint.h>
#include <stdlib.h>

#include <chrono>
#include <memory>
#include <vector>

#include "dfq_hip.h"

#ifdef __HIPCC__
#define DFQ_HOST_DEVICE __host__ __device__
#else
#define DFQ_HOST_DEVICE
#endif

namespace dfq {

inline const char* ab_env(const char* name) {
#ifdef DFQ_DIAGNOSTICS
    return getenv(name);
#else
    (void)name;
    return nullptr;
#endif
}
inline double now_us() {
    return std::chrono::duration<double, std::micro>(std::chrono::steady_clock::now().time_since_epoch()).count();
}

DFQ_HOST_DEVICE inline int64_t ceil_div(int64_t a, int64_t b) { return (a + b - 1) / b; }
DFQ_HOST_DEVICE inline int64_t round256(int64_t b) { return ceil_div(b, (int64_t)256) * 256; }
DFQ_HOST_DEVICE inline int aten_ceil_log2(int64_t x) {
    if (x <= 2) return 1;
    int r = 0;
    for (uint64_t v = (uint64_t)(x - 1); v; v >>= 1) ++r;
    return r;
}

constexpr int kWave = 64;
constexpr int kThreads = 256;
constexpr int kColTileRows = 16;

struct CleRel {
    float* w1;
    float* w2;
    float* b1;
    float* bnw;
    float* bnb;
    float* sacc;
    int64_t c1, len1, o2, i2, khw2, o2g;
    int64_t moff;
    int32_t sacc_init;
    int32_t vec1;
    int32_t vec2;
    int32_t fuse_next;
    int32_t dw_prev;
    int32_t w1_self;
    int32_t w2_self;
};

enum : int32_t { kRangeW1 = 0, kRangeW2Contig = 1, kRangeW2Tile = 2, kRangeReset = 3, kRangeResetW1 = 4 };
enum : int32_t { kApplyW1 = 0, kApplyW2Contig = 1, kApplyW2Tile = 2, kApplyChannels = 3, kApplyDwBoth = 4 };

struct CleTask {
    int32_t rel;
    int32_t kind;
    int64_t a, b;
    int64_t c0, c1;
};

struct CleLayer {
    float* w;
    float* snap;
    int64_t n;
    int64_t nt;
};

struct CleChunk {
    int32_t layer;
    int32_t t;
    int64_t c0;
    int64_t len;
};

struct CleUnit {
    int32_t chunk;
    int32_t tile;
};
constexpr int kCleTile = 8192;
constexpr int kCleTailWords = 64;

DFQ_HOST_DEVICE inline int row_group_lanes(int64_t len) {
    if (len >= 64) return 64;
    int g = 1;
    while (g < len) g <<= 1;
    return g;
}
DFQ_HOST_DEVICE inline int64_t rows_per_task(int64_t len) { return 4 * (64 / row_group_lanes(len)); }

constexpr int64_t kCleChansPerTask = 1024;
constexpr int64_t kCleW1SmallElems = 2048, kCleDwRowsMult = 1;

constexpr int kTileMaxKhw = 9;
#ifndef DFQ_CLE_POS_ROWS
#define DFQ_CLE_POS_ROWS 4
#endif
constexpr int kPosTileMaxRows = DFQ_CLE_POS_ROWS;

struct CleSwitches {
    bool fused = true;
    int64_t w1_mult = 0;
    int64_t dw_mult = kCleDwRowsMult;
    bool lag = true;
    bool stop_arrival = false;
    int32_t band = -1;
    static CleSwitches from_env();
    void append_to(std::vector<int64_t>& key) const;
};

struct CleStructure {
    std::vector<CleRel> R;
    int64_t M = 0;
    int32_t chains = 0, steps = 0;
    bool fused = false;
    std::vector<CleTask> rt, at;
    std::vector<int64_t> rstep, astep;
    std::vector<char> step_pos;
    int64_t ri0 = 0, ri1 = 0;
    std::vector<CleLayer> layers;
    std::vector<CleChunk> chunks;
    int64_t nbig = 0;
    std::vector<CleUnit> units;
    std::vector<int64_t> b1off;
    int64_t nb1_total = 0;
    std::vector<int64_t> uoffs, roffs;
    int32_t nlaunch = 0, stop_off = -1;
    bool lagged = false;
    double t_chains = 0, t_tasks = 0, t_chunks = 0, t_place = 0;
    int64_t bytes_rescale = 0, bytes_metric = 0, bytes_range = 0;
    uint64_t id = 0;
};

int cle_rels_from_desc(const dfq_cle_rel* rels, int32_t n_rel, std::vector<CleRel>& R, int64_t& M);
int cle_build_structure(std::vector<CleRel> R, int64_t M, float* const* targets, const int64_t* target_n,
                        int32_t n_targets, int32_t ref_threads, const CleSwitches& sw, CleStructure& S);
std::shared_ptr<const CleStructure> cle_structure_cached(const std::vector<CleRel>& R, int64_t M,
                                                         float* const* targets, const int64_t* target_n,
                                                         int32_t n_targets, int32_t ref_threads, int& rc, bool& cached);

}
```

### include/dfq_diag.h

```cpp
#ifndef DFQ_DIAG_H_
#define DFQ_DIAG_H_

#include "dfq_hip.h"

#ifdef __cplusplus
extern "C" {
#endif
#pragma GCC visibility push(default)

int dfq_probe_stream(const float* x, float* y, void* codes, float* esum, int64_t n, int32_t blocks,
                     void* stream);
int dfq_debug_timeline(void* buf, int64_t cap);
int dfq_debug_ablate(uint32_t flags);
int dfq_probe_lds(const float* x, float* y, void* codes, float* esum, int64_t n, int32_t copy_only,
                  int32_t blocks, void* stream);

int dfq_diag_cle_check_structure(const dfq_cle_rel* rels, int32_t n_rel, float* const* targets,
                                 const int64_t* target_n, int32_t n_targets, int32_t ref_threads, int64_t* info,
                                 char* msg, int32_t msg_cap);

#pragma GCC visibility pop
#ifdef __cplusplus
}
#endif
#endif
```

Measured before the change: 1958.

## Ping-pong CLE weight buffers instead of snapshotting layers before each step

Cross-layer equalization now reads weights from one buffer and writes them to an alternate buffer chosen by iteration parity, using per-relation first-rescale flags and a selection table. This replaces separate snapshot copies and the snapshot init work in the loop init kernel. The change is meant to cut extra weight copy traffic, in exchange for always launching the rollback kernel and more complex buffer bookkeeping, which a new diagnostic checker validates.

```diff
diff --git a/data_free_quantization_amd/_lib.py b/data_free_quantization_amd/_lib.py
--- a/data_free_quantization_amd/_lib.py
+++ b/data_free_quantization_amd/_lib.py
@@ -36,7 +36,7 @@
     "dfq_int_gemm", "dfq_int_linear", "dfq_int_conv2d", "dfq_int_dwconv2d",
 ]
 DIAG_EXPORTS = ["dfq_probe_stream", "dfq_probe_lds", "dfq_debug_timeline", "dfq_debug_ablate",
-                "dfq_diag_cle_check_structure"]
+                "dfq_diag_cle_check_structure", "dfq_diag_cle_check_selection"]
 DIAG_LIB_PATH = PKG / "libdfq_diag.so"
 
 
@@ -281,6 +281,8 @@
         "dfq_probe_lds": ([P, P, P, P, I64, I32, I32, P], C.c_int),
         "dfq_diag_cle_check_structure": ([C.POINTER(CleRel), I32, C.POINTER(P), C.POINTER(I64), I32, I32,
                                           C.POINTER(I64), C.c_char_p, I32], C.c_int),
+        "dfq_diag_cle_check_selection": ([C.POINTER(CleRel), I32, C.POINTER(P), C.POINTER(I64), I32, I32,
+                                          C.POINTER(I32), C.POINTER(I32), C.c_char_p, I32], C.c_int),
     }
     for name, (args, res) in sig.items():
         fn = getattr(L, name)
diff --git a/data_free_quantization_amd/csrc/dfq_cle.hip b/data_free_quantization_amd/csrc/dfq_cle.hip
--- a/data_free_quantization_amd/csrc/dfq_cle.hip
+++ b/data_free_quantization_amd/csrc/dfq_cle.hip
@@ -225,11 +225,20 @@
             if (e != hipSuccess) { set_last_hip_error(e); cle_plan_free(p); return DFQ_ERR_HIP; }
             snap_base = static_cast<char*>(p->d_snap_owned);
         }
+        std::vector<float*> slot(n_targets);
         int64_t snap_off = 0;
         for (int32_t l = 0; l < n_targets; ++l) {
+            slot[l] = reinterpret_cast<float*>(snap_base + snap_off);
+            snap_off += snap_bytes(target_n[l]);
+        }
+        const CleSelect& sel = S->sel;
+        for (int32_t l = 0; l < n_targets; ++l) {
             layers[l].w = targets[l];
-            layers[l].snap = reinterpret_cast<float*>(snap_base + snap_off);
-            snap_off += snap_bytes(target_n[l]);
+            layers[l].snap = sel.lay_alt[l] >= 0 ? slot[sel.lay_alt[l]] : targets[l];
+        }
+        for (int32_t r = 0; r < n_rel; ++r) {
+            Rb[r].w1a = sel.rel_lay1[r] >= 0 ? slot[sel.rel_lay1[r]] : Rb[r].w1;
+            Rb[r].w2a = sel.rel_lay2[r] >= 0 ? slot[sel.rel_lay2[r]] : Rb[r].w2;
         }
     }
     if (cle_timing() && !cached) {
@@ -422,10 +431,9 @@
         const int64_t npart = (int64_t)p->slots * std::max(p->nl(), 1), ncnt = p->nchunks() + 1;
         const int64_t nvtag = T.vtag ? (int64_t)S.at.size() : 0;
         const int64_t words = std::max({4 * S.M, npart, ncnt, nvtag});
-        const int64_t grid = std::min<int64_t>(std::max<int64_t>({p->nunits(), ceil_div(words, (int64_t)kThreads), 1}), 4096);
-        hipLaunchKernelGGL(cle_loop_init_kernel, dim3((int)grid), dim3(kThreads), 0, s, T.layers, T.chunks,
-                           p->nchunks(), T.units, p->nunits(), T.rng, S.M, T.part, npart, T.cnt, ncnt,
-                           T.vtag, nvtag, T.state, init);
+        const int64_t grid = std::min<int64_t>(std::max<int64_t>(ceil_div(words, (int64_t)kThreads), 1), 4096);
+        hipLaunchKernelGGL(cle_loop_init_kernel, dim3((int)grid), dim3(kThreads), 0, s, T.rng, S.M, T.part, npart,
+                           T.cnt, ncnt, T.vtag, nvtag, T.state, init);
         DFQ_LAUNCH_CHECK();
     }
     if (S.fused && S.rstep[1] > S.rstep[0]) {
@@ -487,7 +495,7 @@
                          std::vector<double>* hist) {
     hipStream_t s = ctx.st;
     const CleTables& T = p->t;
-    if (!run.idle && p->S->lagged) {
+    if (!run.idle) {
         hipLaunchKernelGGL(cle_loop_rollback_kernel, dim3(1024), dim3(kThreads), 0, s, T.layers, p->nl(), T.rels,
                            T.atasks, (int64_t)p->S->at.size(), T.vsave, T.vtag, T.state);
         DFQ_LAUNCH_CHECK();
diff --git a/data_free_quantization_amd/csrc/dfq_cle_kernels.h b/data_free_quantization_amd/csrc/dfq_cle_kernels.h
--- a/data_free_quantization_amd/csrc/dfq_cle_kernels.h
+++ b/data_free_quantization_amd/csrc/dfq_cle_kernels.h
@@ -72,18 +72,19 @@
 }
 
 template <class F>
-__device__ __forceinline__ void wave_scale(float* __restrict__ p_, int64_t n, bool vec, int lane, F&& factor) {
-    DFQ_GLOBAL float* __restrict__ p = (DFQ_GLOBAL float*)p_;
+__device__ __forceinline__ void wave_scale(const DFQ_GLOBAL float* s, DFQ_GLOBAL float* p, int64_t n, bool vec,
+                                           int lane, F&& factor) {
     float f = 0.f;
     bool have = false;
     if (vec) {
+        const DFQ_GLOBAL f32x4* s4 = (const DFQ_GLOBAL f32x4*)s;
         DFQ_GLOBAL f32x4* p4 = (DFQ_GLOBAL f32x4*)p;
         const int64_t n4 = n >> 2;
         for (int64_t i = lane; i < n4; i += 4 * 64) {
             f32x4 v[4];
 #pragma unroll
             for (int u = 0; u < 4; ++u)
-                if (i + 64 * u < n4) v[u] = p4[i + 64 * u];
+                if (i + 64 * u < n4) v[u] = s4[i + 64 * u];
             if (!have) {
                 f = factor();
                 have = true;
@@ -103,7 +104,7 @@
             float v[4];
 #pragma unroll
             for (int u = 0; u < 4; ++u)
-                if (i + 64 * u < n) v[u] = p[i + 64 * u];
+                if (i + 64 * u < n) v[u] = s[i + 64 * u];
             if (!have) {
                 f = factor();
                 have = true;
@@ -116,21 +117,21 @@
 }
 
 template <class F>
-__device__ __forceinline__ void wave_scale_mm(float* __restrict__ p_, int64_t n, bool vec, int lane, float& vmin,
-                                              float& vmax, F&& factor) {
-    DFQ_GLOBAL float* __restrict__ p = (DFQ_GLOBAL float*)p_;
+__device__ __forceinline__ void wave_scale_mm(const DFQ_GLOBAL float* s, DFQ_GLOBAL float* p, int64_t n, bool vec,
+                                              int lane, float& vmin, float& vmax, F&& factor) {
     vmin = INFINITY;
     vmax = -INFINITY;
     float f = 0.f;
     bool have = false;
     if (vec) {
+        const DFQ_GLOBAL f32x4* s4 = (const DFQ_GLOBAL f32x4*)s;
         DFQ_GLOBAL f32x4* p4 = (DFQ_GLOBAL f32x4*)p;
         const int64_t n4 = n >> 2;
         for (int64_t i = lane; i < n4; i += 4 * 64) {
             f32x4 v[4];
 #pragma unroll
             for (int u = 0; u < 4; ++u)
-                if (i + 64 * u < n4) v[u] = p4[i + 64 * u];
+                if (i + 64 * u < n4) v[u] = s4[i + 64 * u];
             if (!have) {
                 f = factor();
                 have = true;
@@ -152,7 +153,7 @@
             float v[4];
 #pragma unroll
             for (int u = 0; u < 4; ++u)
-                if (i + 64 * u < n) v[u] = p[i + 64 * u];
+                if (i + 64 * u < n) v[u] = s[i + 64 * u];
             if (!have) {
                 f = factor();
                 have = true;
@@ -171,15 +172,14 @@
 }
 
 template <class F>
-__device__ __forceinline__ void wave_scale_range(float* __restrict__ p_, int64_t n, int lane, float& vmin, float& vmax,
-                                                 F&& factor) {
-    DFQ_GLOBAL float* __restrict__ p = (DFQ_GLOBAL float*)p_;
+__device__ __forceinline__ void wave_scale_range(const DFQ_GLOBAL float* s, DFQ_GLOBAL float* p, int64_t n, int lane,
+                                                 float& vmin, float& vmax, F&& factor) {
     vmin = INFINITY;
     vmax = -INFINITY;
     float f = 0.f;
     bool have = false;
     for (int64_t i = lane; i < n; i += 64) {
-        const float x = p[i];
+        const float x = s[i];
         if (!have) {
             f = factor();
             have = true;
@@ -196,14 +196,23 @@
     return R.khw2 > 1 && R.khw2 <= kTileMaxKhw && (tk.a / R.o2g) == ((tk.b - 1) / R.o2g);
 }
 
-__device__ void tile_range_by_position(const CleRel& R, const CleTask& tk, uint32_t* __restrict__ mn,
+__device__ __forceinline__ float* cle_wr1(const CleRel& R, int par) { return cle_cur(R.w1, R.w1a, par); }
+__device__ __forceinline__ float* cle_wr2(const CleRel& R, int par) { return cle_cur(R.w2, R.w2a, par); }
+__device__ __forceinline__ const float* cle_rd1(const CleRel& R, int par) {
+    return R.first1 ? cle_prev(R.w1, R.w1a, par) : cle_cur(R.w1, R.w1a, par);
+}
+__device__ __forceinline__ const float* cle_rd2(const CleRel& R, int par) {
+    return R.first2 ? cle_prev(R.w2, R.w2a, par) : cle_cur(R.w2, R.w2a, par);
+}
+
+__device__ void tile_range_by_position(const CleRel& R, const float* w2, const CleTask& tk, uint32_t* __restrict__ mn,
                                        uint32_t* __restrict__ mx, float* __restrict__ tl) {
     const int t = threadIdx.x;
     const int khw = (int)R.khw2;
     const int64_t rowlen = R.i2 * R.khw2;
     const int ncol = (int)(tk.c1 - tk.c0);
     const int npos = ncol * khw;
-    const DFQ_GLOBAL float* base = (const DFQ_GLOBAL float*)(R.w2 + tk.c0 * R.khw2);
+    const DFQ_GLOBAL float* base = (const DFQ_GLOBAL float*)(w2 + tk.c0 * R.khw2);
     float vmn[kTileMaxKhw], vmx[kTileMaxKhw];
 #pragma unroll
     for (int m = 0; m < kTileMaxKhw; ++m) {
@@ -257,12 +266,14 @@
         const CleRel& R = rels[tk.rel];
         uint32_t* mn = mins + R.moff;
         uint32_t* mx = maxs + R.moff;
+        const float* w1 = cle_rd1(R, par);
+        const float* w2 = cle_rd2(R, par);
         if (tk.kind == kRangeW1 && R.len1 < 64) {
             for_short_rows(tk.a, tk.b, R.len1, [&](int64_t c, bool act, int sl, int G) {
                 float vmin = INFINITY, vmax = -INFINITY;
                 if (act)
                     for (int64_t i = sl; i < R.len1; i += G) {
-                        const float x = ((DFQ_GLOBAL float*)R.w1)[c * R.len1 + i];
+                        const float x = ((const DFQ_GLOBAL float*)w1)[c * R.len1 + i];
                         vmin = fminf(vmin, x);
                         vmax = fmaxf(vmax, x);
                     }
@@ -279,7 +290,7 @@
                 float vmin = INFINITY, vmax = -INFINITY;
                 if (act)
                     for (int64_t i = sl; i < seg; i += G) {
-                        const float x = ((DFQ_GLOBAL float*)R.w2)[c * seg + i];
+                        const float x = ((const DFQ_GLOBAL float*)w2)[c * seg + i];
                         vmin = fminf(vmin, x);
                         vmax = fmaxf(vmax, x);
                     }
@@ -293,7 +304,7 @@
         } else if (tk.kind == kRangeW1) {
             for (int64_t c = tk.a + wv; c < tk.b; c += kThreads / 64) {
                 float vmin, vmax;
-                wave_range(R.w1 + c * R.len1, R.len1, R.vec1, lane, vmin, vmax);
+                wave_range(w1 + c * R.len1, R.len1, R.vec1, lane, vmin, vmax);
                 if (lane == 0) {
                     mn[c] = enc_ord(vmin);
                     mx[c] = enc_ord(vmax);
@@ -303,7 +314,7 @@
             const int64_t seg = R.o2g * R.khw2;
             for (int64_t c = tk.a + wv; c < tk.b; c += kThreads / 64) {
                 float vmin, vmax;
-                wave_range(R.w2 + c * seg, seg, R.vec2, lane, vmin, vmax);
+                wave_range(w2 + c * seg, seg, R.vec2, lane, vmin, vmax);
                 if (lane == 0) {
                     mn[R.c1 + c] = enc_ord(vmin);
                     mx[R.c1 + c] = enc_ord(vmax);
@@ -311,7 +322,7 @@
             }
         } else if (tk.kind == kRangeW2Tile) {
             if (tile_by_position(R, tk)) {
-                tile_range_by_position(R, tk, mn, mx, tl);
+                tile_range_by_position(R, w2, tk, mn, mx, tl);
                 continue;
             }
             const int64_t rowlen = R.i2 * R.khw2;
@@ -322,7 +333,7 @@
                     float v[kColTileRows];
 #pragma unroll
                     for (int j = 0; j < kColTileRows; ++j)
-                        if (tk.a + j < tk.b) v[j] = ((DFQ_GLOBAL float*)R.w2)[(tk.a + j) * rowlen + i];
+                        if (tk.a + j < tk.b) v[j] = ((const DFQ_GLOBAL float*)w2)[(tk.a + j) * rowlen + i];
 #pragma unroll
                     for (int j = 0; j < kColTileRows; ++j)
                         if (tk.a + j < tk.b) {
@@ -344,7 +355,7 @@
                         vmax = -INFINITY;
                     }
                     g_prev = g;
-                    const DFQ_GLOBAL float* p = (const DFQ_GLOBAL float*)(R.w2 + o * rowlen + i * R.khw2);
+                    const DFQ_GLOBAL float* p = (const DFQ_GLOBAL float*)(w2 + o * rowlen + i * R.khw2);
                     for (int64_t k = 0; k < R.khw2; ++k) {
                         vmin = fminf(vmin, p[k]);
                         vmax = fmaxf(vmax, p[k]);
@@ -430,14 +441,16 @@
         const CleRel& R = rels[tk.rel];
         const uint32_t* mn = mins + R.moff;
         const uint32_t* mx = maxs + R.moff;
+        const bool w1_task = tk.kind == kApplyW1;
+        const DFQ_GLOBAL float* rd = (const DFQ_GLOBAL float*)(w1_task ? cle_rd1(R, par) : cle_rd2(R, par));
+        DFQ_GLOBAL float* wr = (DFQ_GLOBAL float*)(w1_task ? cle_wr1(R, par) : cle_wr2(R, par));
         if (tk.kind == kApplyW1 && R.len1 < 64) {
             for_short_rows(tk.a, tk.b, R.len1, [&](int64_t c, bool act, int sl, int G) {
                 float y0 = INFINITY, y1 = -INFINITY;
                 if (act && sl < R.len1) {
-                    DFQ_GLOBAL float* p = (DFQ_GLOBAL float*)(R.w1 + c * R.len1 + sl);
-                    const float x = *p;
+                    const float x = rd[c * R.len1 + sl];
                     const float y = x * cle_rel_scale(rels, R, mins, maxs, c, is_signed, eps, smin, smax).s;
-                    *p = y;
+                    wr[c * R.len1 + sl] = y;
                     y0 = y1 = y;
                 }
                 if (R.w1_self) {
@@ -455,13 +468,12 @@
             for_short_rows(tk.a, tk.b, seg, [&](int64_t c, bool act, int sl, int G) {
                 float z0 = INFINITY, z1 = -INFINITY;
                 if (act && sl < seg) {
-                    DFQ_GLOBAL float* p = (DFQ_GLOBAL float*)(R.w2 + c * seg + sl);
-                    const float x = *p;
+                    const float x = rd[c * seg + sl];
                     const float inv = cle_rel_scale(rels, R, mins, maxs, c, is_signed, eps, smin, smax).inv;
                     const float sn = cle_rel_scale(rels, N, mins, maxs, c, is_signed, eps, smin, smax).s;
                     const float y = x * inv;
                     const float z = y * sn;
-                    *p = z;
+                    wr[c * seg + sl] = z;
                     z0 = z1 = z;
                 }
                 if (R.w2_self) {
@@ -479,10 +491,9 @@
             for_short_rows(tk.a, tk.b, seg, [&](int64_t c, bool act, int sl, int G) {
                 float vmin = INFINITY, vmax = -INFINITY;
                 if (act && sl < seg) {
-                    DFQ_GLOBAL float* p = (DFQ_GLOBAL float*)(R.w2 + c * seg + sl);
-                    const float x = *p;
+                    const float x = rd[c * seg + sl];
                     const float y = x * cle_rel_scale(rels, R, mins, maxs, c, is_signed, eps, smin, smax).inv;
-                    *p = y;
+                    wr[c * seg + sl] = y;
                     vmin = vmax = y;
                 }
                 if (fuse) {
@@ -500,13 +511,13 @@
                 auto sc = [&] { return cle_rel_scale(rels, R, mins, maxs, c, is_signed, eps, smin, smax).s; };
                 if (R.w1_self) {
                     float y0, y1;
-                    wave_scale_mm(R.w1 + c * R.len1, R.len1, R.vec1, lane, y0, y1, sc);
+                    wave_scale_mm(rd + c * R.len1, wr + c * R.len1, R.len1, R.vec1, lane, y0, y1, sc);
                     if (lane == 0) {
                         nmins[R.moff + c] = enc_ord(y0);
                         nmaxs[R.moff + c] = enc_ord(y1);
                     }
                 } else {
-                    wave_scale(R.w1 + c * R.len1, R.len1, R.vec1, lane, sc);
+                    wave_scale(rd + c * R.len1, wr + c * R.len1, R.len1, R.vec1, lane, sc);
                 }
             }
         } else if (tk.kind == kApplyDwBoth) {
@@ -515,12 +526,11 @@
             for (int64_t c = tk.a + wv; c < tk.b; c += kThreads / 64) {
                 const float inv = cle_rel_scale(rels, R, mins, maxs, c, is_signed, eps, smin, smax).inv;
                 const float sn = cle_rel_scale(rels, N, mins, maxs, c, is_signed, eps, smin, smax).s;
-                DFQ_GLOBAL float* p = (DFQ_GLOBAL float*)(R.w2 + c * seg);
                 float z0 = INFINITY, z1 = -INFINITY;
                 for (int64_t i = lane; i < seg; i += 64) {
-                    const float y = p[i] * inv;
+                    const float y = rd[c * seg + i] * inv;
                     const float z = y * sn;
-                    p[i] = z;
+                    wr[c * seg + i] = z;
                     z0 = fminf(z0, z);
                     z1 = fmaxf(z1, z);
                 }
@@ -538,14 +548,14 @@
                 auto inv = [&] { return cle_rel_scale(rels, R, mins, maxs, c, is_signed, eps, smin, smax).inv; };
                 if (R.fuse_next >= 0) {
                     float vmin, vmax;
-                    wave_scale_range(R.w2 + c * seg, seg, lane, vmin, vmax, inv);
+                    wave_scale_range(rd + c * seg, wr + c * seg, seg, lane, vmin, vmax, inv);
                     if (lane == 0) {
                         const int64_t off = rels[R.fuse_next].moff;
                         mins[off + c] = enc_ord(vmin);
                         maxs[off + c] = enc_ord(vmax);
                     }
                 } else {
-                    wave_scale(R.w2 + c * seg, seg, R.vec2, lane, inv);
+                    wave_scale(rd + c * seg, wr + c * seg, seg, R.vec2, lane, inv);
                 }
             }
         } else if (POS && tk.kind == kApplyW2Tile && tile_by_position(R, tk) && tk.b - tk.a <= kPosTileMaxRows) {
@@ -554,7 +564,8 @@
             const int64_t rowlen = R.i2 * R.khw2;
             const int ncol = (int)(tk.c1 - tk.c0);
             const int npos = ncol * khw;
-            DFQ_GLOBAL float* base = (DFQ_GLOBAL float*)(R.w2 + tk.c0 * R.khw2);
+            const DFQ_GLOBAL float* rbase = rd + tk.c0 * R.khw2;
+            DFQ_GLOBAL float* base = wr + tk.c0 * R.khw2;
             const bool fuse = R.fuse_next >= 0;
             if (t < ncol)
                 inv_s[t] = cle_rel_scale(rels, R, mins, maxs, (tk.a / R.o2g) * R.i2 + tk.c0 + t, is_signed, eps, smin, smax).inv;
@@ -566,7 +577,7 @@
             float v[kPosTileMaxRows][kTileMaxKhw];
 #pragma unroll
             for (int r = 0; r < kPosTileMaxRows; ++r) {
-                const DFQ_GLOBAL float* rb = base + (tk.a + r) * rowlen;
+                const DFQ_GLOBAL float* rb = rbase + (tk.a + r) * rowlen;
 #pragma unroll
                 for (int m = 0; m < kTileMaxKhw; ++m)
                     if (tk.a + r < tk.b && m < khw && t + kThreads * m < npos) v[r][m] = rb[t + kThreads * m];
@@ -615,7 +626,7 @@
                 float v[kColTileRows];
 #pragma unroll
                 for (int j = 0; j < kColTileRows; ++j)
-                    if (act && j < nr) v[j] = ((DFQ_GLOBAL float*)R.w2)[(tk.a + j) * rowlen + i];
+                    if (act && j < nr) v[j] = rd[(tk.a + j) * rowlen + i];
                 const float inv =
                     act ? cle_rel_scale(rels, R, mins, maxs, (tk.a / R.o2g) * R.i2 + i, is_signed, eps, smin, smax).inv : 0.f;
 #pragma unroll
@@ -624,7 +635,7 @@
                         float y = __builtin_nanf("");
                         if (act) {
                             y = v[j] * inv;
-                            ((DFQ_GLOBAL float*)R.w2)[(tk.a + j) * rowlen + i] = y;
+                            wr[(tk.a + j) * rowlen + i] = y;
                         }
                         rows[j * kThreads + threadIdx.x] = y;
                     }
@@ -671,10 +682,10 @@
                             inv = cle_rel_scale(rels, R, mins, maxs, g * R.i2 + i, is_signed, eps, smin, smax).inv;
                             g_prev = g;
                         }
-                        DFQ_GLOBAL float* p = (DFQ_GLOBAL float*)(R.w2 + o * rowlen + i * R.khw2);
+                        const int64_t e = o * rowlen + i * R.khw2;
                         for (int64_t k = 0; k < R.khw2; ++k) {
-                            const float y = p[k] * inv;
-                            p[k] = y;
+                            const float y = rd[e + k] * inv;
+                            wr[e + k] = y;
                             lo = fminf(lo, y);
                             hi = fmaxf(hi, y);
                         }
@@ -708,14 +719,14 @@
                     float v[kColTileRows];
 #pragma unroll
                     for (int j = 0; j < kColTileRows; ++j)
-                        if (tk.a + j < tk.b) v[j] = ((DFQ_GLOBAL float*)R.w2)[(tk.a + j) * rowlen + i];
+                        if (tk.a + j < tk.b) v[j] = rd[(tk.a + j) * rowlen + i];
                     const float inv = cle_rel_scale(rels, R, mins, maxs, (tk.a / R.o2g) * R.i2 + i, is_signed, eps, smin,
                                                 smax).inv;
-                    ((DFQ_GLOBAL float*)R.w2)[tk.a * rowlen + i] = v[0] * inv;
+                    wr[tk.a * rowlen + i] = v[0] * inv;
                     DFQ_CLE_TL_MARK(0)
 #pragma unroll
                     for (int j = 1; j < kColTileRows; ++j)
-                        if (tk.a + j < tk.b) ((DFQ_GLOBAL float*)R.w2)[(tk.a + j) * rowlen + i] = v[j] * inv;
+                        if (tk.a + j < tk.b) wr[(tk.a + j) * rowlen + i] = v[j] * inv;
                     DFQ_CLE_TL_MARK(1)
                     continue;
                 }
@@ -727,8 +738,8 @@
                         inv = cle_rel_scale(rels, R, mins, maxs, g * R.i2 + i, is_signed, eps, smin, smax).inv;
                         g_prev = g;
                     }
-                    DFQ_GLOBAL float* p = (DFQ_GLOBAL float*)(R.w2 + o * rowlen + i * R.khw2);
-                    for (int64_t k = 0; k < R.khw2; ++k) p[k] = p[k] * inv;
+                    const int64_t e = o * rowlen + i * R.khw2;
+                    for (int64_t k = 0; k < R.khw2; ++k) wr[e + k] = rd[e + k] * inv;
                 }
             }
         } else {
@@ -768,34 +779,16 @@
 
 
 __global__ void __launch_bounds__(kThreads)
-cle_loop_init_kernel(const CleLayer* __restrict__ layers, const CleChunk* __restrict__ chunks, int64_t nchunks,
-                     const CleUnit* __restrict__ units, int64_t nunits, uint32_t* __restrict__ rng, int64_t M,
-                     float* __restrict__ part, int64_t npart, uint32_t* __restrict__ cnt, int64_t ncnt,
-                     int32_t* __restrict__ vtag, int64_t nvtag, CleState* __restrict__ st, CleState init) {
+cle_loop_init_kernel(uint32_t* __restrict__ rng, int64_t M, float* __restrict__ part, int64_t npart,
+                     uint32_t* __restrict__ cnt, int64_t ncnt, int32_t* __restrict__ vtag, int64_t nvtag,
+                     CleState* __restrict__ st, CleState init) {
     const int64_t gt = (int64_t)blockIdx.x * kThreads + threadIdx.x, gs = (int64_t)gridDim.x * kThreads;
     for (int64_t i = gt; i < 4 * M; i += gs) rng[i] = ((i / M) & 1) ? 0u : 0xFFFFFFFFu;
     for (int64_t i = gt; i < npart; i += gs) part[i] = 0.f;
     for (int64_t i = gt; i < ncnt; i += gs) cnt[i] = 0u;
     for (int64_t i = gt; i < nvtag; i += gs) vtag[i] = -1;
     if (gt == 0) *st = init;
-    for (int64_t u = blockIdx.x; u < nunits; u += gridDim.x) {
-        const CleUnit un = units[u];
-        const CleChunk ch = chunks[un.chunk];
-        const CleLayer Ly = layers[ch.layer];
-        const int64_t nb1 = (ch.len / 32) / 256;
-        const int64_t e0 = (int64_t)un.tile * 8192;
-        const int64_t e1 = un.tile < nb1 ? e0 + 8192 : ch.len;
-        for (int64_t i = e0 + threadIdx.x; i < e1; i += kThreads) Ly.snap[ch.c0 + i] = Ly.w[ch.c0 + i];
-    }
-    if (blockIdx.x == 0)
-        for (int64_t k = 0; k < nchunks; ++k) {
-            const CleChunk ch = chunks[k];
-            if (ch.len >= 8) continue;
-            const CleLayer Ly = layers[ch.layer];
-            for (int64_t i = threadIdx.x; i < ch.len; i += kThreads) Ly.snap[ch.c0 + i] = Ly.w[ch.c0 + i];
-        }
-}
-
+}
 
 struct CleNoUnitHook {
     __device__ void operator()(const CleUnit&, const CleChunk&, int64_t) const {}
@@ -805,14 +798,15 @@
 __device__ __forceinline__ void cle_tiles_body(const CleLayer* __restrict__ layers, const CleChunk* __restrict__ chunks,
                                                const int64_t* __restrict__ b1off, const CleUnit* __restrict__ units,
                                                int64_t nunits, float* __restrict__ b1buf, float* __restrict__ tailbuf,
-                                               int64_t blk, int64_t nblk, float* d, float* b0, Hook hook = Hook()) {
+                                               int par, int64_t blk, int64_t nblk, float* d, float* b0,
+                                               Hook hook = Hook()) {
     const int tid = threadIdx.x;
     for (int64_t u = blk; u < nunits; u += nblk) {
         const CleUnit un = units[u];
         const CleChunk ch = chunks[un.chunk];
         const CleLayer Ly = layers[ch.layer];
-        const DFQ_GLOBAL float* __restrict__ w = (const DFQ_GLOBAL float*)(Ly.w + ch.c0);
-        DFQ_GLOBAL float* __restrict__ sn = (DFQ_GLOBAL float*)(Ly.snap + ch.c0);
+        const DFQ_GLOBAL float* w = (const DFQ_GLOBAL float*)(cle_cur(Ly.w, Ly.snap, par) + ch.c0);
+        const DFQ_GLOBAL float* sn = (const DFQ_GLOBAL float*)(cle_prev(Ly.w, Ly.snap, par) + ch.c0);
         const int64_t len = ch.len, sz = len / 32, vs = len / 8;
         const int64_t nb1 = sz / 256;
         const bool full = un.tile < nb1;
@@ -833,13 +827,9 @@
 #pragma unroll
             for (int h = 0; h < 2; ++h) {
                 const int q = tid + h * kThreads;
-                const int64_t base = e0 + 32 * (16 * (q >> 5)) + (q & 31);
                 float a = 0.f;
 #pragma unroll
-                for (int j = 0; j < 16; ++j) {
-                    a += fabsf(xs[h][j] - ys[h][j]);
-                    sn[base + 32 * j] = xs[h][j];
-                }
+                for (int j = 0; j < 16; ++j) a += fabsf(xs[h][j] - ys[h][j]);
                 b0[q] = a;
             }
             __syncthreads();
@@ -860,10 +850,7 @@
                     }
 #pragma unroll
                 for (int u = 0; u < 8; ++u)
-                    if (e + u * kThreads < cnt) {
-                        d[e + u * kThreads] = fabsf(x[u] - y[u]);
-                        sn[e0 + e + u * kThreads] = x[u];
-                    }
+                    if (e + u * kThreads < cnt) d[e + u * kThreads] = fabsf(x[u] - y[u]);
             }
             __syncthreads();
             const int64_t ni = sz - nb1 * 256;
@@ -937,16 +924,11 @@
                               lane);
 }
 
-__device__ __forceinline__ float cle_tiny_chunk_sum(const CleLayer* __restrict__ layers, const CleChunk& ch) {
+__device__ __forceinline__ float cle_tiny_chunk_sum(const CleLayer* __restrict__ layers, const CleChunk& ch, int par) {
     const CleLayer Ly = layers[ch.layer];
-    float* w = Ly.w + ch.c0;
-    float* sn = Ly.snap + ch.c0;
-    return aten_inner_sum([&](int64_t e) {
-        const float x = w[e];
-        const float dd = fabsf(x - sn[e]);
-        sn[e] = x;
-        return dd;
-    }, ch.len);
+    const float* w = cle_cur(Ly.w, Ly.snap, par) + ch.c0;
+    const float* sn = cle_prev(Ly.w, Ly.snap, par) + ch.c0;
+    return aten_inner_sum([&](int64_t e) { return fabsf(w[e] - sn[e]); }, ch.len);
 }
 
 template <class P>
@@ -1158,14 +1140,15 @@
     auto tl2_rec = [](int) {};
 #endif
     float* lds = L.tiles;
-    auto finish = [&]() {
+    auto finish = [&](int fin_par) {
 #ifdef DFQ_DIAGNOSTICS
         const uint64_t tf0 = __builtin_amdgcn_s_memrealtime();
 #endif
         if (threadIdx.x == 0 && F.nchunks > F.nbig)
             for (int64_t k = 0; k < F.nchunks; ++k) {
                 const CleChunk c2 = chunks[k];
-                if (c2.len < 8) st_coh(F.part + (int64_t)c2.layer * F.S + c2.t, 0.f + cle_tiny_chunk_sum(layers, c2));
+                if (c2.len < 8)
+                    st_coh(F.part + (int64_t)c2.layer * F.S + c2.t, 0.f + cle_tiny_chunk_sum(layers, c2, fin_par));
             }
         asm volatile("s_waitcnt vmcnt(0)" ::: "memory");
         __syncthreads();
@@ -1200,7 +1183,7 @@
             if (threadIdx.x == 0)
                 flag = handoff_arrive(F.cnt + F.nchunks, ((uint32_t)stop_it + 1u) * (uint32_t)nstop - 1u);
             __syncthreads();
-            if (flag) finish();
+            if (flag) finish(stop_it & 1);
             return;
         }
         blk -= nstop;
@@ -1228,7 +1211,7 @@
         return flag != 0;
     };
     if (F.nbig == 0) {
-        if (own && tb == 0 && F.last) finish();
+        if (own && tb == 0 && F.last) finish(it & 1);
         return;
     }
     const uint32_t fin_members = (uint32_t)F.nbig;
@@ -1253,14 +1236,14 @@
                 if (threadIdx.x == 0) st_coh(F.part + (int64_t)ch.layer * F.S + ch.t, 0.f + fa);
             }
         }
-        if (F.stop_arrival && arrive(F.cnt + F.nchunks, fin_members)) finish();
+        if (F.stop_arrival && arrive(F.cnt + F.nchunks, fin_members)) finish(it & 1);
     };
     if (F.stop_arrival)
         cle_tiles_body<decltype(hook)>(layers, chunks, b1off, units + (own ? uo : up), own ? nuo : nup, b1buf, tailbuf,
-                                       tb, tnb, lds, lds + kCleTile + kCleTailWords, hook);
+                                       it & 1, tb, tnb, lds, lds + kCleTile + kCleTailWords, hook);
     else
-        cle_tiles_body(layers, chunks, b1off, units + (own ? uo : up), own ? nuo : nup, b1buf, tailbuf, tb, tnb, lds,
-                       lds + kCleTile + kCleTailWords);
+        cle_tiles_body(layers, chunks, b1off, units + (own ? uo : up), own ? nuo : nup, b1buf, tailbuf, it & 1, tb, tnb,
+                       lds, lds + kCleTile + kCleTailWords);
 #ifdef DFQ_DIAGNOSTICS
     if (tl2) {
         const CleUnit un0 = units[(own ? uo : up) + tb];
@@ -1277,10 +1260,13 @@
                          const int32_t* __restrict__ vtag, const CleState* __restrict__ st) {
     const int32_t A = st->iters;
     const int64_t gt = (int64_t)blockIdx.x * kThreads + threadIdx.x, gs = (int64_t)gridDim.x * kThreads;
-    for (int32_t l = 0; l < nl; ++l) {
-        const CleLayer Ly = layers[l];
-        for (int64_t i = gt; i < Ly.n; i += gs) Ly.w[i] = Ly.snap[i];
-    }
+    if (A & 1)
+        for (int32_t l = 0; l < nl; ++l) {
+            const CleLayer Ly = layers[l];
+            if (Ly.snap == Ly.w) continue;
+            for (int64_t i = gt; i < Ly.n; i += gs) Ly.w[i] = Ly.snap[i];
+        }
+    if (!vtag) return;
     for (int64_t t = blockIdx.x; t < n_at; t += gridDim.x) {
         const CleTask tk = atasks[t];
         if (tk.kind != kApplyChannels || vtag[t] != A) continue;
diff --git a/data_free_quantization_amd/csrc/dfq_cle_plan.cpp b/data_free_quantization_amd/csrc/dfq_cle_plan.cpp
--- a/data_free_quantization_amd/csrc/dfq_cle_plan.cpp
+++ b/data_free_quantization_amd/csrc/dfq_cle_plan.cpp
@@ -332,6 +332,37 @@
     P.lay_t.resize(n_targets);
     for (int32_t l = 0; l < n_targets; ++l) P.lay_t[l] = P.find(targets[l]);
     return P;
+}
+
+static bool cle_select(std::vector<CleRel>& R, const CleChains& C, const CleSpans& P, int32_t n_targets,
+                       CleSelect& sel) {
+    const int32_t n_rel = (int32_t)R.size();
+    std::vector<int32_t> firsts(P.w.size(), 0);
+    for (int32_t r = 0; r < n_rel; ++r) {
+        R[r].first1 = R[r].first2 = 0;
+        for (int side = 0; side < 2; ++side) {
+            if (side == 0 && R[r].dw_prev >= 0) continue;
+            const int32_t ti = side ? P.rel_t2[r] : P.rel_t1[r];
+            if (C.step_of[r] != P.v[ti].first) continue;
+            (side ? R[r].first2 : R[r].first1) = 1;
+            if (++firsts[ti] > 1) return false;
+        }
+    }
+    std::vector<int32_t> slot(P.w.size(), -1);
+    sel.lay_alt.assign(n_targets, -1);
+    for (int32_t l = 0; l < n_targets; ++l) {
+        const int32_t ti = P.lay_t[l];
+        if (ti < 0) continue;
+        if (slot[ti] < 0) slot[ti] = l;
+        sel.lay_alt[l] = slot[ti];
+    }
+    sel.rel_lay1.resize(n_rel);
+    sel.rel_lay2.resize(n_rel);
+    for (int32_t r = 0; r < n_rel; ++r) {
+        sel.rel_lay1[r] = slot[P.rel_t1[r]];
+        sel.rel_lay2[r] = slot[P.rel_t2[r]];
+    }
+    return true;
 }
 
 static bool cle_place_lagged(int32_t nl, const std::vector<CleRel>& R, const CleChains& C, const CleTaskTables& T,
@@ -481,6 +512,7 @@
                         int32_t n_targets, int32_t ref_threads, const CleSwitches& sw, CleStructure& S) {
     const double tp1 = now_us();
     const CleChains C = cle_chains(R, sw);
+    if (!cle_select(R, C, cle_spans(R, C, targets, n_targets), n_targets, S.sel)) return DFQ_ERR_UNSUPPORTED;
     const double tp2 = now_us();
     CleTaskTables T = cle_tasks(R, C, sw);
     const double tp3 = now_us();
@@ -635,9 +667,9 @@
     return h;
 }
 
-extern "C" int dfq_diag_cle_check_structure(const dfq_cle_rel* rels, int32_t n_rel, float* const* targets,
-                                            const int64_t* target_n, int32_t n_targets, int32_t ref_threads,
-                                            int64_t* info, char* msg, int32_t msg_cap) {
+static int cle_check_structure(const dfq_cle_rel* rels, int32_t n_rel, float* const* targets, const int64_t* target_n,
+                               int32_t n_targets, int32_t ref_threads, int64_t* info, char* msg, int32_t msg_cap,
+                               const int32_t* sel_set, int32_t* sel_get) {
     auto fail = [&](const char* fmt, long long a, long long b, long long c) {
         if (msg && msg_cap > 0) snprintf(msg, (size_t)msg_cap, fmt, a, b, c);
         return DFQ_ERR_INVALID;
@@ -651,6 +683,22 @@
     if (const int rc = cle_build_structure(R0, M, targets, target_n, n_targets, ref_threads, CleSwitches::from_env(), S);
         rc != DFQ_OK)
         return rc;
+    if (sel_get) {
+        for (int32_t r = 0; r < n_rel; ++r) {
+            const int32_t v[4] = {S.R[r].first1, S.R[r].first2, S.sel.rel_lay1[r], S.sel.rel_lay2[r]};
+            std::memcpy(sel_get + 4 * r, v, sizeof(v));
+        }
+        for (int32_t l = 0; l < n_targets; ++l) sel_get[4 * n_rel + l] = S.sel.lay_alt[l];
+    }
+    if (sel_set) {
+        for (int32_t r = 0; r < n_rel; ++r) {
+            S.R[r].first1 = sel_set[4 * r];
+            S.R[r].first2 = sel_set[4 * r + 1];
+            S.sel.rel_lay1[r] = sel_set[4 * r + 2];
+            S.sel.rel_lay2[r] = sel_set[4 * r + 3];
+        }
+        for (int32_t l = 0; l < n_targets; ++l) S.sel.lay_alt[l] = sel_set[4 * n_rel + l];
+    }
     const std::vector<CleRel>& R = S.R;
     const int32_t steps = S.steps, NL = S.nlaunch;
     if (const char* e = getenv("DFQ_CLE_PLACE_DUMP"); e && *e) {
@@ -695,6 +743,7 @@
                     S.astep.empty() ? -1 : S.astep.back());
     std::vector<int32_t> rel_step(n_rel, -1);
     std::vector<std::pair<const float*, int32_t>> touch;
+    std::vector<int32_t> touch_side;
     if ((int32_t)S.step_pos.size() != std::max<int32_t>(steps, 1) || (steps == 0 && S.step_pos[0] != 0))
         return fail("step_pos: %lld entries for %lld steps (first %lld)", (long long)S.step_pos.size(), steps,
                     S.step_pos.empty() ? -1 : S.step_pos[0]);
@@ -710,20 +759,24 @@
                 case kApplyW1:
                     if (tk.b > c.c1) return fail("W1 task %lld: rows to %lld of %lld", t, tk.b, c.c1);
                     touch.push_back({c.w1, k});
+                    touch_side.push_back(2 * tk.rel);
                     break;
                 case kApplyW2Contig:
                     if (tk.b > c.c1 || c.i2 != 1) return fail("W2 contig task %lld: channels to %lld of %lld", t, tk.b, c.c1);
                     touch.push_back({c.w2, k});
+                    touch_side.push_back(2 * tk.rel + 1);
                     break;
                 case kApplyDwBoth:
                     if (tk.b > c.c1 || tk.c0 < 0 || tk.c0 >= n_rel || R[tk.c0].w1 != c.w2 || R[tk.c0].dw_prev != tk.rel)
                         return fail("depthwise pair task %lld: partner %lld, channels to %lld", t, tk.c0, tk.b);
                     touch.push_back({c.w2, k});
+                    touch_side.push_back(2 * tk.rel + 1);
                     break;
                 case kApplyW2Tile:
                     if (tk.b > c.o2 || tk.c0 < 0 || tk.c0 >= tk.c1 || tk.c1 > c.i2)
                         return fail("W2 tile task %lld: rows to %lld, columns to %lld", t, tk.b, tk.c1);
                     touch.push_back({c.w2, k});
+                    touch_side.push_back(2 * tk.rel + 1);
                     pos = pos || c.khw2 > 1;
                     break;
                 case kApplyChannels:
@@ -741,6 +794,54 @@
     }
     for (int32_t r = 0; r < n_rel; ++r)
         if (rel_step[r] < 0) return fail("relation %lld has no channel task", r, 0, 0);
+    if ((int32_t)S.sel.rel_lay1.size() != n_rel || (int32_t)S.sel.rel_lay2.size() != n_rel ||
+        (int32_t)S.sel.lay_alt.size() != n_targets)
+        return fail("selection tables: %lld / %lld relations, %lld targets", (long long)S.sel.rel_lay1.size(),
+                    (long long)S.sel.rel_lay2.size(), (long long)S.sel.lay_alt.size());
+    std::vector<int32_t> use_step(2 * (size_t)n_rel, -1);
+    for (size_t i = 0; i < touch.size(); ++i) {
+        int32_t& u = use_step[touch_side[i]];
+        if (u >= 0 && u != touch[i].second)
+            return fail("relation %lld side %lld: rescale tasks in steps %lld and more", touch_side[i] / 2, touch_side[i] % 2, u);
+        u = touch[i].second;
+    }
+    auto side_w = [&](int32_t x) { return (x & 1) ? R[x / 2].w2 : R[x / 2].w1; };
+    auto first_layer_of = [&](const float* w) {
+        for (int32_t l = 0; l < n_targets; ++l)
+            if (targets[l] == w) return l;
+        return (int32_t)-1;
+    };
+    for (int32_t x = 0; x < 2 * n_rel; ++x) {
+        const float* w = side_w(x);
+        const int32_t first = (x & 1) ? R[x / 2].first2 : R[x / 2].first1;
+        if (first != 0 && first != 1) return fail("relation %lld side %lld: first flag %lld", x / 2, x % 2, first);
+        int32_t fstep = INT32_MAX, nfirst = 0;
+        for (int32_t y = 0; y < 2 * n_rel; ++y) {
+            if (side_w(y) != w || use_step[y] < 0) continue;
+            fstep = std::min(fstep, use_step[y]);
+            nfirst += ((y & 1) ? R[y / 2].first2 : R[y / 2].first1) ? 1 : 0;
+            if (y != x && use_step[y] == use_step[x])
+                return fail("relations %lld and %lld rescale one tensor in the same step %lld", x / 2, y / 2, use_step[x]);
+        }
+        if (use_step[x] < 0) {
+            if (first) return fail("relation %lld side %lld is a first rescale without rescale tasks", x / 2, x % 2, 0);
+        } else {
+            if (nfirst != 1) return fail("relation %lld side %lld: its tensor has %lld first rescales", x / 2, x % 2, nfirst);
+            if ((first != 0) != (use_step[x] == fstep))
+                return fail("relation %lld side %lld: first rescale flag %lld, but the tensor's first step is not its own", x / 2,
+                            x % 2, first);
+        }
+        const int32_t lay = (x & 1) ? S.sel.rel_lay2[x / 2] : S.sel.rel_lay1[x / 2];
+        if (lay != first_layer_of(w))
+            return fail("relation %lld side %lld: second buffer of layer %lld, not its tensor's", x / 2, x % 2, lay);
+    }
+    for (int32_t l = 0; l < n_targets; ++l) {
+        bool rescaled = false;
+        for (int32_t x = 0; x < 2 * n_rel && !rescaled; ++x) rescaled = side_w(x) == targets[l];
+        const int32_t expect = rescaled ? first_layer_of(targets[l]) : -1;
+        if (S.sel.lay_alt[l] != expect)
+            return fail("target %lld: second buffer of layer %lld, expected %lld", l, S.sel.lay_alt[l], expect);
+    }
     const int64_t nrt = (int64_t)S.rt.size();
     if (S.ri0 < 0 || S.ri0 > S.ri1 || S.ri1 > nrt) return fail("range slice [%lld, %lld) of %lld tasks", S.ri0, S.ri1, nrt);
     for (int64_t t = 0; t < nrt; ++t) {
@@ -845,4 +946,17 @@
     if (msg && msg_cap > 0) snprintf(msg, (size_t)msg_cap, "digest %016llx", (unsigned long long)cle_structure_digest(S));
     return DFQ_OK;
 }
+
+extern "C" int dfq_diag_cle_check_structure(const dfq_cle_rel* rels, int32_t n_rel, float* const* targets,
+                                            const int64_t* target_n, int32_t n_targets, int32_t ref_threads,
+                                            int64_t* info, char* msg, int32_t msg_cap) {
+    return cle_check_structure(rels, n_rel, targets, target_n, n_targets, ref_threads, info, msg, msg_cap, nullptr, nullptr);
+}
+
+extern "C" int dfq_diag_cle_check_selection(const dfq_cle_rel* rels, int32_t n_rel, float* const* targets,
+                                            const int64_t* target_n, int32_t n_targets, int32_t ref_threads,
+                                            const int32_t* sel_set, int32_t* sel_get, char* msg, int32_t msg_cap) {
+    return cle_check_structure(rels, n_rel, targets, target_n, n_targets, ref_threads, nullptr, msg, msg_cap, sel_set,
+                               sel_get);
+}
 #endif
diff --git a/data_free_quantization_amd/csrc/dfq_cle_plan.h b/data_free_quantization_amd/csrc/dfq_cle_plan.h
--- a/data_free_quantization_amd/csrc/dfq_cle_plan.h
+++ b/data_free_quantization_amd/csrc/dfq_cle_plan.h
@@ -57,7 +57,15 @@
     int32_t dw_prev;
     int32_t w1_self;
     int32_t w2_self;
+    float* w1a;
+    float* w2a;
+    int32_t first1;
+    int32_t first2;
 };
+template <class T>
+DFQ_HOST_DEVICE inline T* cle_cur(T* w, T* wa, int par) { return par ? w : wa; }
+template <class T>
+DFQ_HOST_DEVICE inline T* cle_prev(T* w, T* wa, int par) { return par ? wa : w; }
 
 enum : int32_t { kRangeW1 = 0, kRangeW2Contig = 1, kRangeW2Tile = 2, kRangeReset = 3, kRangeResetW1 = 4 };
 enum : int32_t { kApplyW1 = 0, kApplyW2Contig = 1, kApplyW2Tile = 2, kApplyChannels = 3, kApplyDwBoth = 4 };
@@ -118,6 +126,11 @@
     void append_to(std::vector<int64_t>& key) const;
 };
 
+struct CleSelect {
+    std::vector<int32_t> rel_lay1, rel_lay2;
+    std::vector<int32_t> lay_alt;
+};
+
 struct CleStructure {
     std::vector<CleRel> R;
     int64_t M = 0;
@@ -138,6 +151,7 @@
     bool lagged = false;
     double t_chains = 0, t_tasks = 0, t_chunks = 0, t_place = 0;
     int64_t bytes_rescale = 0, bytes_metric = 0, bytes_range = 0;
+    CleSelect sel;
     uint64_t id = 0;
 };
 
diff --git a/include/dfq_diag.h b/include/dfq_diag.h
--- a/include/dfq_diag.h
+++ b/include/dfq_diag.h
@@ -18,6 +18,9 @@
 int dfq_diag_cle_check_structure(const dfq_cle_rel* rels, int32_t n_rel, float* const* targets,
                                  const int64_t* target_n, int32_t n_targets, int32_t ref_threads, int64_t* info,
                                  char* msg, int32_t msg_cap);
+int dfq_diag_cle_check_selection(const dfq_cle_rel* rels, int32_t n_rel, float* const* targets,
+                                 const int64_t* target_n, int32_t n_targets, int32_t ref_threads,
+                                 const int32_t* sel_set, int32_t* sel_get, char* msg, int32_t msg_cap);
 
 #pragma GCC visibility pop
 #ifdef __cplusplus
```

New measurement: 1958, median of 2. About the same (-0.0%).
